# unilight/seq2seq-vc

Hardware: AMD Instinct MI355X
Metric: mel-frames/sec (train) (higher is better)
Workload: dtype bf16; 1 GPU; VTN egs/arctic/vc1 (vtn.v1.yaml) training step: fwd+Seq2SeqLoss+bwd+clip+Adam+WarmupLR; batch_per_gpu=32, global_batch=32, T_src=256, T_tgt=256, mel_dim=80, parallelism=dp1, split_backward=False, hip_graph=True, backward_stages=1

## Files before the change

include/s2svc_hip.h:

```cpp
#ifndef S2SVC_HIP_H
#define S2SVC_HIP_H
#include <stdint.h>
#ifdef __cplusplus
extern "C" {
#endif

const char* s2svc_last_error(void);
int s2svc_abi_version(void);
int s2svc_launch_floor(int workgroups, int threads, void* sink_1024_words, void* stream);

int s2svc_event_create(void** out );
int s2svc_event_destroy(void* ev);
int s2svc_event_record(void* ev, void* stream);
int s2svc_stream_wait_event(void* stream, void* ev);

enum { S2SVC_LAYOUT_KC = 0,
       S2SVC_LAYOUT_RC = 1 };
enum { S2SVC_OP_DENSE = 0,
       S2SVC_OP_CONV1D = 1,
       S2SVC_OP_CONV2D_S2 = 2,
       S2SVC_OP_TCONV2D_S2 = 3 };

typedef struct {
  const void* ptr;
  int64_t ld;
  int32_t layout;
  int32_t mode;
  int32_t C;
  int32_t T;
  int32_t pad;
  int32_t T1, F1, T2, F2;
  int64_t bs0, bs1;
  int32_t zero_padded;
  int32_t reserved_;
} s2svc_operand;

typedef struct {
  s2svc_operand A, B;
  void* C;
  int64_t ldc, cbs0, cbs1;
  int32_t c_dtype;
  const float* bias;
  const void* res;
  int64_t ldr, rbs0, rbs1;
  int32_t M, N, K;
  int32_t nb0, nb1;
  int32_t act;
  float alpha;
  int32_t dtype;
  int32_t accumulate;
  int32_t splitk;
  float* ws;
  float* a_rowsum;
  float* a_rowsum_ws;
  int32_t a_rowsum_accumulate;
  int32_t tile_hint;
  const void* emask;
  int64_t ldm;
  float drop_p;
  int32_t emask_mode;
  const uint64_t* seed_base;
  uint64_t seed_off;
  int32_t c_map;
  int32_t cm_T1, cm_F1, cm_Tc, cm_Fc, cm_pt, cm_pf;
  int32_t reserved3_;
  void* c_pre;
} s2svc_gemm_desc;

int s2svc_gemm(const s2svc_gemm_desc* desc , void* stream);
const char* s2svc_gemm_last_route(void);

int s2svc_tconv2d_weights(int O, int C, const float* w, void* out_bf16, void* stream);

int s2svc_gemm_grouped_ok(const s2svc_gemm_desc* desc );
int s2svc_gemm_grouped(const s2svc_gemm_desc* descs , int n, int tile, void* stream);
int s2svc_gemm_grouped_batched(const s2svc_gemm_desc* descs , int n, void* stream);
int s2svc_gemm_wgrad_ok(const s2svc_gemm_desc* desc );
int64_t s2svc_gemm_wgrad_ws_floats(const s2svc_gemm_desc* descs , int n);
int s2svc_gemm_wgrad_grouped(const s2svc_gemm_desc* descs , int n, float* ws, void* stream);
int s2svc_gemm_wgrad_grouped_bg(const s2svc_gemm_desc* descs , int n, float* ws, void* stream, int wgs_cap);
int s2svc_gemm_set_w8(int on, int kt_chunk);

int s2svc_gemm_set_8ph(int mode);

int s2svc_layernorm_fwd(int dtype, int rows, int D, const void* x, const void* res, float drop_p, float hscale,
                        const uint64_t* seed_base, uint64_t seed_off, const float* gamma, const float* beta, float eps,
                        void* y, void* s_out, float* mean, float* rstd, void* stream);
int s2svc_layernorm_bwd(int dtype, int rows, int D, const void* dy, const void* s, const float* mean, const float* rstd,
                        const float* gamma, const void* ds_extra, float drop_p, float hscale, const uint64_t* seed_base,
                        uint64_t seed_off, void* ds, void* dh, void* stream);
int s2svc_colreduce(int dtype, int rows, int D, int mode, const void* dy, const void* x, const float* mean,
                    const float* rstd, float scale, float* out_sum, float* out_dot, int accumulate, float* ws,
                    int ws_chunks, int Tn, const int32_t* vlens , void* stream);
typedef struct {
  const void* dy;
  const void* x;
  const float* mean;
  const float* rstd;
  float* out_sum;
  float* out_dot;
  float* ws;
  int32_t dtype, rows, D, mode, accumulate, ws_chunks;
  float scale;
  int32_t reserved_;
} s2svc_colreduce_item;
int s2svc_colreduce_grouped(const s2svc_colreduce_item* items , int n, void* stream);
int s2svc_layernorm_bwd_pg_chunks(int dtype, int rows, int D, const void* dy, const void* s, const float* gamma, const void* ds_extra,
                                  const void* ds, const void* dh);
int s2svc_layernorm_bwd_pg(int dtype, int rows, int D, const void* dy, const void* s, const float* mean, const float* rstd,
                           const float* gamma, const void* ds_extra, float drop_p, float hscale, const uint64_t* seed_base,
                           uint64_t seed_off, void* ds, void* dh, float* ws, void* stream);
int s2svc_bn_finalize(int C, int n, float eps, float momentum, const float* mean, const float* var, float* rstd,
                      float* run_mean, float* run_var, int64_t* num_batches, int var_is_ex2 ,
                      int Tn, const int32_t* vlens , void* stream);
int s2svc_rstd_from_var(int C, float eps, const float* var, float* rstd, void* stream);
int s2svc_bn_stats(int dtype, int rows, int C, const void* x, float eps, float momentum, float* mean, float* rstd,
                   float* run_mean, float* run_var, int64_t* num_batches, float* ws, int ws_chunks, int Tn, const int32_t* vlens,
                   void* stream);
int s2svc_bn_apply(int dtype, int64_t rows, int C, const void* x, const float* mean, const float* rstd,
                   const float* gamma, const float* beta, int act, float drop_p, const uint64_t* seed_base,
                   uint64_t seed_off, void* y, void* pre_act, int Tn, const int32_t* vlens, void* stream);
int s2svc_bn_bwd(int dtype, int64_t rows, int C, const void* dy, const void* x, const float* mean, const float* rstd,
                 const float* gamma, const float* sum_dy, const float* sum_dy_xhat, int use_batch_stats, void* dx,
                 int Tn, const int32_t* vlens, void* stream);

int s2svc_attn_softmax_fwd(int dtype, int B, int H, int T1, int T2, int ld, const float* scores, const float* bd, int Lp,
                           int ldb, int rel_mode, float scale, const int32_t* klen, int causal, float drop_p,
                           const uint64_t* seed_base, uint64_t seed_off, void* attn, void* pdrop, void* stream);
int s2svc_attn_softmax_bwd(int dtype, int B, int H, int T1, int T2, int ld, const void* attn, const float* dp, const void* dattn,
                           float scale, float drop_p, const uint64_t* seed_base, uint64_t seed_off, void* dscores,
                           void* dbd, int Lp, int ldb, int rel_mode, void* stream);

int s2svc_act_dropout_fwd(int dtype, int64_t n, const void* x, int act, float p, const uint64_t* seed_base,
                          uint64_t seed_off, void* y, void* stream);
int s2svc_act_dropout_bwd(int dtype, int64_t n, const void* dz, const void* saved, int act, float p,
                          const uint64_t* seed_base, uint64_t seed_off, void* dx, void* stream);
int s2svc_posenc_fwd(int dtype, int64_t B, int T, int D, const void* x, float xscale, const float* alpha, const float* pe,
                     float p, const uint64_t* seed_base, uint64_t seed_off, void* y, void* stream);
int s2svc_posenc_bwd(int dtype, int64_t B, int T, int D, const void* dy, float xscale, const float* pe, float p,
                     const uint64_t* seed_base, uint64_t seed_off, void* dx, float* dalpha, float* partials, void* stream);
int s2svc_axpby(int dtype, int64_t n, float a, const void* x, float b, const void* y, void* out, void* stream);
#define S2SVC_SCALAR_TERMS_MAX 8
typedef struct {
  const float* x[S2SVC_SCALAR_TERMS_MAX];
  int32_t n[S2SVC_SCALAR_TERMS_MAX];
  float w[S2SVC_SCALAR_TERMS_MAX];
  int32_t k;
  int32_t reserved_;
} s2svc_scalar_terms;
int s2svc_weighted_sum(const s2svc_scalar_terms* terms , float* out, void* stream);
int s2svc_weighted_sum_bwd(const s2svc_scalar_terms* grads , const float* g, void* stream);
int s2svc_scalars_axpy(const s2svc_scalar_terms* terms , float beta, float* acc, void* stream);
int s2svc_fill_zero(void* p, int64_t nbytes, void* stream);
int s2svc_seed_advance(uint64_t* seed, uint64_t inc, void* stream);
int s2svc_pad_cols(int dtype, int64_t rows, int N, int ldo, const void* in, void* out, void* stream);
int s2svc_decoder_input(int out_dtype, int B, int Tin, int r, int D, int64_t ys_batch_stride, const float* ys, void* out, void* stream);
int s2svc_append_eos(int B, int T, int64_t ldx, const int64_t* xs, const int32_t* lens, int64_t eos, int64_t pad, int64_t* out, void* stream);
int s2svc_copy_rows(int dtype, int64_t rows, int D, int64_t lds, const void* src, void* out, void* stream);
int s2svc_stop_labels(int B, int T, int64_t ld_labels, const float* labels, const int32_t* lens, float* out, void* stream);
int s2svc_add_n(int dtype, int64_t n, int k, const void* x0, const void* x1, const void* x2, const void* x3, void* out, void* stream);
int s2svc_add_head_bias(int dtype, int64_t rows, int D, const void* q, const float* u, const float* v, void* qu, void* qv,
                        void* stream);
int s2svc_add_head_bias_ld(int dtype, int64_t rows, int D, const void* q, int64_t ldq, const float* u, const float* v, void* qu,
                           void* qv, void* stream);
int s2svc_add_rows(int dtype, int64_t rows, int D, const void* a, int64_t lda, const void* b, int64_t ldb, void* out, int64_t ldo,
                   void* stream);
int s2svc_glu_fwd(int dtype, int64_t rows, int C, const void* x, void* y, void* stream);
int s2svc_glu_bwd(int dtype, int64_t rows, int C, const void* x, const void* dy, void* dx, void* stream);
int s2svc_cast(int in_dtype, int out_dtype, int64_t n, const void* x, void* y, void* stream);
int s2svc_gather3(int in_dtype, int out_dtype, int n0, int n1, int n2, int64_t s0, int64_t s1, int64_t s2, int64_t off,
                  const void* in, void* out, void* stream);
typedef struct s2svc_gather3_job {
  const void* in;
  void* out;
  int64_t s0, s1, s2, off;
  int32_t n0, n1, n2;
  int32_t out_dtype;
} s2svc_gather3_job;
int s2svc_gather3_grouped(const s2svc_gather3_job* jobs , int n, void* stream);
enum { S2SVC_DERIVED_GATHER3 = 0, S2SVC_DERIVED_TCONV2D = 1 };
typedef struct s2svc_derived_job {
  const void* in;
  void* out;
  int64_t s0, s1, s2, off;
  int32_t n0, n1, n2;
  int32_t out_dtype;
  int32_t kind;
  int32_t reserved_;
} s2svc_derived_job;
int s2svc_derived_refresh(const s2svc_derived_job* jobs , int n, void* stream);
int s2svc_derived_refresh_plan(const s2svc_derived_job* jobs , int n, int32_t* path , int32_t* units );
int s2svc_permute_inner(int n, int A, int B, const float* src, float* dst, int accumulate, void* stream);
int s2svc_rowscale(int dtype, int64_t rows, int D, const void* x, const float* s, void* out, void* stream);

int s2svc_conv_in1_fwd(int dtype, int B, int Tn, int Fn, int O, const void* x, const float* w, const float* bias, void* y,
                       void* stream);
int s2svc_conv_in1_wgrad(int dtype, int B, int Tn, int Fn, int O, const void* x, const void* dy, const void* y, float* dw,
                         float* db, int accumulate, float* partial, int max_chunks, void* stream);
int s2svc_col2im_s2(int dtype, int B, int T1, int F1, int C, int T2, int F2, const void* dcols, void* dx, void* stream);
int s2svc_interp_nearest(int dtype, int B, int Tin, int Tout, int C, const void* x, void* y, const int32_t* ext_in,
                         const int32_t* ext_out, void* stream);
int s2svc_interp_nearest_bwd(int dtype, int B, int Tin, int Tout, int C, const void* dy, void* dx, const int32_t* ext_in,
                             const int32_t* ext_out, void* stream);
int s2svc_interp_nearest_rows(int dtype, int B, int Tin, int Tout, int C, const void* x, void* y, const int32_t* lens_in,
                              const int32_t* lens_out, void* stream);
int s2svc_dwconv(int dtype, int B, int Tn, int C, int ks, int dil, const void* x, const float* w, const float* bias,
                 void* y, int flip, void* stream);
int s2svc_dwconv_add(int dtype, int B, int Tn, int C, int ks, int dil, const void* x, const float* w, const float* bias,
                     const void* add, void* y, int flip, void* stream);
int s2svc_dwconv_wgrad(int dtype, int B, int Tn, int C, int ks, int dil, const void* x, const void* dy, float* dw,
                       int accumulate, float* ws, int ws_chunks, void* stream);

int s2svc_convmod_supported(int C, int ks);
int s2svc_convmod_fwd(int B, int Tn, int C, int ks, const void* y2, const float* w, const float* bias, void* z, float eps,
                      float momentum, float* mean, float* rstd, float* run_mean, float* run_var, int64_t* num_batches, float* ws,
                      const int32_t* vlens, void* stream);
int s2svc_bn_swish_apply(int64_t rows, int C, const void* z, const float* mean, const float* rstd, const float* gamma,
                         const float* beta, void* out, int Tn, const int32_t* vlens, void* stream);
int s2svc_convmod_bwd(int B, int Tn, int C, int ks, const void* da, const void* z, const void* y2, const float* w, const float* mean,
                      const float* rstd, const float* gamma, const float* beta, void* dy2, float* sdy, float* sdyx,
                      float* dgamma_acc, float* dbeta_acc, float* ws_stats, float* ws_w, const int32_t* vlens, void* stream);
int s2svc_convmod_wgrad_final(int C, int ks, int chunks, const float* ws_w, float* dw, float* db, int accumulate, void* stream);

int s2svc_convmod_infer_supported(int C, int ks);
int s2svc_convmod_infer(int dtype, int B, int Tn, int C, int ks, const void* y2, const float* w, const float* bias, const float* run_mean,
                        const float* run_var, const float* gamma, const float* beta, float eps, void* out, const int32_t* vlens,
                        void* stream);

int s2svc_bn_stats_vec(int rows, int C, const void* x, float eps, float momentum, float* mean, float* rstd, float* run_mean,
                       float* run_var, int64_t* num_batches, float* ws, int Tn, const int32_t* vlens, void* stream);
int s2svc_bn_act_apply_vec(int rows, int C, const void* x, const float* mean, const float* rstd, const float* gamma, const float* beta,
                           int act, float drop_p, const uint64_t* seed_base, uint64_t seed_off, void* y, void* pre_act, int Tn,
                           const int32_t* vlens, void* stream);
int s2svc_bn_act_bwd_vec(int rows, int C, const void* dz, const void* saved, const void* x, const float* mean, const float* rstd,
                         const float* gamma, int act, float drop_p, const uint64_t* seed_base, uint64_t seed_off, void* dx, float* sdy,
                         float* sdyx, float* dgamma_acc, float* dbeta_acc, float* ws, int Tn, const int32_t* vlens, void* stream);

int s2svc_pairwise_l2_logsoftmax(int dtype, int B, int Tf, int Tx, int A, const void* feats, const void* text,
                                 const int32_t* text_lens, float* logp, float* dist, void* stream);
int s2svc_pairwise_l2_bwd_g(int dtype, int B, int Tf, int Tx, const float* logp, const float* dist, const float* dlogp,
                            const int32_t* text_lens, void* G, float* rowsum, void* stream);
int64_t s2svc_mas_ws_bytes(int B, int Tf, int Tx);
int s2svc_mas(int B, int Tf, int Tx, const float* log_p_attn, const int32_t* text_lens, const int32_t* feat_lens,
              int32_t* path, float* ds, float* binmean, void* ws, void* stream);
int s2svc_mas_binloss_bwd(int B, int Tf, int Tx, const int32_t* path, const int32_t* feat_lens, const float* gout,
                          float* dlogp, void* stream);
int s2svc_gauss_upsample_probs(int dtype, int B, int Tf, int Tx, const float* ds, const int32_t* text_lens,
                               const int32_t* feat_lens, float delta, void* P, void* stream);

int s2svc_length_regulate_index(int B, int Tx, int Tout, const int32_t* ds, int32_t* start, int32_t* idx, int32_t* total,
                                void* stream);
int s2svc_length_regulate_fwd(int dtype, int B, int Tx, int Tout, int D, const void* x, const int32_t* idx, float pad_value,
                              void* y, void* stream);
int s2svc_durations_finalize(int dtype_i64, int B, int Tx, const void* d, const int32_t* text_lens, float dmax, void* d_outs, float* ds,
                             int32_t* total, void* stream);
int s2svc_length_regulate_bwd(int dtype, int B, int Tx, int Tout, int D, const void* dy, const int32_t* start, const int32_t* ds,
                              void* dx, void* stream);
int s2svc_attn_durations(int NH, int Tf, int Tx, const float* att, int64_t* durations, float* focus_rate, int32_t* head,
                         void* stream);

int s2svc_seq_loss_fwd(int dtype, int B, int Tm, int D, const void* after, const void* before, const void* logits,
                       const float* ys, const float* labels, const int32_t* olens, float pos_weight, float* partial,
                       float* out, void* stream);
int s2svc_seq_loss_bwd(int dtype, int B, int Tm, int D, const void* after, const void* before, const void* logits,
                       const float* ys, const float* labels, const int32_t* olens, float pos_weight, const float* stats,
                       const float* g_l1, const float* g_bce, void* d_after, void* d_before, void* d_logits, void* stream);
int s2svc_guided_attn_loss_fwd(int dtype, int B, int H, int To, int Ti, const void* att, const int32_t* ilens,
                               const int32_t* olens, float sigma, float alpha, float* partial, float* out, void* stream);
int s2svc_guided_attn_loss_bwd(int dtype, int B, int H, int To, int Ti, const int32_t* ilens, const int32_t* olens,
                               float sigma, float alpha, const float* stats, const float* gout, void* datt, void* stream);
int s2svc_duration_loss_fwd(int B, int T, const float* d_outs, const float* ds, const int32_t* lens, float offset, int mean,
                            float* stats, float* out, void* stream);
int s2svc_duration_loss_bwd(int B, int T, const float* d_outs, const float* ds, const int32_t* lens, float offset, int mean,
                            const float* stats, const float* g, float* dd, void* stream);
int64_t s2svc_forward_sum_ws_bytes(int B, int Tf, int Tx);
int s2svc_forward_sum(int B, int Tf, int Tx, const float* log_p_attn, const float* prior, const int32_t* text_lens,
                      const int32_t* feat_lens, float log_blank, void* ws, float* loss_b, float* grad, void* stream);
int s2svc_betabinom_prior(int B, int Tf, int Tx, const int32_t* text_lens, const int32_t* feat_lens, float* prior,
                          void* stream);

int s2svc_attn_fused_supported(int dtype, int T1, int T2, int dk);
int s2svc_attn_fused_fwd(int B, int H, int T1, int T2, int dk, const void* q, int64_t ldq, int64_t qbs, const void* k, int64_t ldk,
                         int64_t kbs, const void* v, int64_t ldv, int64_t vbs, const int32_t* klen, int causal, float scale,
                         float drop_p, const uint64_t* seed_base, uint64_t seed_off, void* attn, int ld, void* out, int64_t ldo,
                         int64_t obs, void* stream);
int s2svc_attn_fused_bwd(int B, int H, int T1, int T2, int dk, const void* q, int64_t ldq, int64_t qbs, const void* k, int64_t ldk,
                         int64_t kbs, const void* v, int64_t ldv, int64_t vbs, const void* dout, int64_t ldo, int64_t obs,
                         const void* attn, const void* dattn, int ld, float scale, float drop_p, const uint64_t* seed_base,
                         uint64_t seed_off, void* dq, int64_t lddq, int64_t dqbs, void* dk_out, int64_t lddk, int64_t dkbs, void* dv,
                         int64_t lddv, int64_t dvbs, void* stream);

int s2svc_relattn_supported(int dtype, int T, int dk, int rel_mode);
int s2svc_relattn_fwd(int B, int H, int T, int dk, const void* q, int64_t ldq, int64_t qbs, const void* k, int64_t ldk, int64_t kbs,
                      const void* pos, int64_t ldp, int L, const float* u, const float* v, const int32_t* klen, float scale,
                      float drop_p, const uint64_t* seed_base, uint64_t seed_off, void* attn, void* pdrop, int ld, void* qu, void* qv,
                      void* stream);

int s2svc_attn_map_supported(int dtype, int T1, int T2, int dk);
int s2svc_attn_map_product_supported(int dk);
int s2svc_attn_map_fwd(int B, int H, int T1, int T2, int dk, const void* q, int64_t ldq, int64_t qbs, const void* k, int64_t ldk,
                       int64_t kbs, const int32_t* klen, int causal, float scale, float drop_p, const uint64_t* seed_base,
                       uint64_t seed_off, void* attn, void* pdrop, int ld, const void* v, int64_t ldv, int64_t vbs, void* ctx,
                       int64_t ldc, int64_t cbs, void* stream);
int s2svc_attn_map_bwd(int B, int H, int T1, int T2, int dk, const void* dctx, int64_t ldo, int64_t obs, const void* v, int64_t ldv,
                       int64_t vbs, const void* attn, const void* dattn, float scale, float drop_p, const uint64_t* seed_base,
                       uint64_t seed_off, void* ds, int ld, void* dbd, int ldb, const void* k, int64_t ldk, int64_t kbs, void* dq,
                       int64_t lddq, int64_t dqbs, void* stream);

int s2svc_embedding_fwd(int dtype, int64_t n, int D, int V, const int64_t* idx, const float* w, void* y, void* stream);
int s2svc_embedding_bwd(int dtype, int64_t n, int D, int V, const int64_t* idx, const void* dy, int64_t padding_idx,
                        float* dw, int accumulate, void* stream);

int s2svc_mask_rows(int dtype, int B, int T, int C, const void* x, const int32_t* lens, void* y, void* stream);
int s2svc_expand_fwd(int dtype, int B, int T, int C, const float* a, const float* w, const float* bias, const void* g,
                     const int32_t* lens, void* y, void* stream);
int s2svc_expand_bwd(int dtype, int B, int T, int C, const void* dy, const float* w, const int32_t* lens, void* dg, float* da,
                     void* stream);
int s2svc_ln_act_fwd(int dtype, int rows, int D, int T, const void* x, const float* gamma, const float* beta, float eps, int act,
                     const void* res, const int32_t* lens, float drop_p, const uint64_t* seed_base, uint64_t seed_off, void* y,
                     float* mean, float* rstd, void* stream);
int s2svc_dw_ln_act_fwd(int B, int T, int D, int ks, int dil, const float* x, const float* dw_w, const float* dw_b,
                        const float* gamma, const float* beta, float eps, int act, float* u, float* y, float* mean, float* rstd,
                        void* stream);
int s2svc_ln_act_bwd(int dtype, int rows, int D, int T, const void* dy, const void* x, const float* mean, const float* rstd,
                     const float* gamma, const float* beta, int act, const int32_t* lens, float drop_p,
                     const uint64_t* seed_base, uint64_t seed_off, void* du, void* dx, void* dres, void* stream);

int s2svc_rq_spline_fwd(int B, int T, int bins, const float* x, const float* h, float hscale, float bound, const int32_t* lens,
                        int inverse, float* out, float* lad, int lad_accumulate, void* stream);
int s2svc_rq_spline_bwd(int B, int T, int bins, const float* x, const float* h, float hscale, float bound, const int32_t* lens,
                        const float* g_out, const float* g_lad, float* dx, float* dh, void* stream);
int s2svc_sdp_head_fwd(int B, int T, const float* noise, const int32_t* lens, const float* m, const float* logs, float* z0,
                       float* z1, void* stream);
int s2svc_sdp_head_bwd(int B, int T, const float* noise, const int32_t* lens, const float* logs, const float* dz0,
                       const float* dz1, float* part, void* stream);
int s2svc_sdp_mid_fwd(int B, int T, const float* zu, const float* z1, const float* w, const int32_t* lens, const float* m,
                      const float* logs, float* y0, float* y1, float* lz, void* stream);
int s2svc_sdp_mid_bwd(int B, int T, const float* zu, const float* z1, const float* w, const int32_t* lens, const float* logs,
                      const float* dy0, const float* dy1, const float* dlz, float* dzu, float* dz1, float* part, void* stream);
int s2svc_sdp_tail_fwd(int B, int T, const float* noise, const int32_t* lens, const float* zu, const float* lz,
                       const float* lad_q, const float* lad_p, const float* af, const float* bf, const float* logs_q,
                       const float* logs_p, float* out, int normalize , void* stream);
int s2svc_sdp_tail_bwd(int B, int T, const float* g, const int32_t* lens, const float* zu, const float* af, const float* bf,
                       float* d_af, float* d_bf, float* d_lz, float* d_zu, float* neg_g, float* part, int normalize, void* stream);
int s2svc_sdp_inverse_out(int B, int T, const float* a, const int32_t* lens, const float* m, const float* logs, float* dur,
                          void* stream);

int s2svc_decode_posenc(int dtype, int B, int D, const void* x, float xscale, const float* alpha, const float* pe,
                        const int32_t* pos, void* y, void* stream);
int s2svc_decode_attn(int dtype, int B, int H, int dk, const void* q, int64_t ldq, void* kcache, void* vcache,
                      int64_t ldt, int64_t cbs, const void* knew, const void* vnew, int64_t ldn, const int32_t* pos,
                      const int32_t* klen, int Tk, float scale, void* ctx, int64_t ldo, float* att, int64_t att_bs,
                      int64_t att_hs, int64_t att_ps, void* stream);
int s2svc_decode_emit(int dtype, int B, int r, int odim, const void* feat, const void* logit, float threshold,
                      const int32_t* minlen, const int32_t* maxlen, const int32_t* pos, float* outs, int64_t outs_bs,
                      float* probs, int64_t probs_bs, void* prev, int32_t* stop_at, void* stream);
int s2svc_decode_advance(int32_t* pos, uint64_t* seed_base, uint64_t seed_stride, void* stream);
int s2svc_decode_ln_linear_supported(int dtype, int M, int K);
int s2svc_decode_ln_linear(const s2svc_gemm_desc* desc , const float* gamma, const float* beta, float eps, void* y_out,
                           int64_t ldy, void* stream);
int s2svc_decode_emit_advance(int dtype, int B, int r, int odim, const void* feat, const void* logit, int64_t ldf, float threshold,
                              const int32_t* minlen, const int32_t* maxlen, int32_t* pos, float* outs, int64_t outs_bs, float* probs,
                              int64_t probs_bs, void* prev, int32_t* stop_at, uint64_t* seed_base, uint64_t seed_stride,
                              uint32_t* ticket, const float* pe, const float* alpha, int D, int pe_rows, void* pe_next, void* stream);

int s2svc_adam_step(int64_t n, float* params, const float* grads, float* exp_avg, float* exp_avg_sq, void* bf16_shadow,
                    float beta1, float beta2, float eps, float max_norm, float base_lr, float warmup_steps,
                    double* partial, float* state, void* stream);

int s2svc_transpose_tiles(int64_t ntiles, const int64_t* tiles, const void* src, void* dst, void* stream);

int s2svc_reflect_pad(int64_t n, int pad, const float* x, float* y, void* stream);
int s2svc_magnitude(int64_t frames, int nb, const float* z, float* spc, void* stream);
int s2svc_log_clamp(int64_t n, int D, const float* x, float eps, float inv_log_base, const float* mean,
                    const float* inv_scale, float* y, void* stream);

int s2svc_reflect_pad_batch(int B, int64_t Nmax, int pad, int64_t ld, const float* x, const int32_t* nlen, float* y, void* stream);
int s2svc_stft_logmel_fft_supported(int n_fft, int nmel, int melw_n);
int s2svc_stft_logmel_fft(int B, int64_t Nmax, int Tmax, int n_fft, int hop, int nmel, const float* x, const int32_t* nlen,
                          const int32_t* frames, const float* tables, const int32_t* mel_lo, const int32_t* mel_hi, const int32_t* mel_off, int melw_n, int mel_maxw,
                          float eps, float inv_log_base, const float* mean, const float* inv_scale, float* out, void* stream);

int s2svc_stft_logmel_fft8(int B, int64_t Nmax, int Tmax, int hop, int nmel, const float* x, const int32_t* nlen, const int32_t* frames,
                           const float* tables, const int32_t* seg_lo, const int32_t* seg_len, const float* wud, float eps,
                           float inv_log_base, const float* mean, const float* inv_scale, float* out, void* stream);

int s2svc_mel_log_batch(int B, int Tmax, int nb, int nmel, const float* z, const int32_t* frames, const float* melb,
                        const int32_t* lo, const int32_t* hi, float eps, float inv_log_base, const float* mean,
                        const float* inv_scale, float* out, void* stream);
int s2svc_ragged_to_padded(int B, int Tmax, int D, const float* ragged, const int64_t* offsets, const float* mean,
                           const float* inv_scale, float* out, float* labels, void* stream);

int s2svc_hifigan_cin_padded(int C);
int s2svc_hifigan_conv1d(int dtype, int B, int T, int Cin, int Cout, int k, int dil, const void* x, const void* w_op, const float* bias,
                         float slope, const void* res, int accumulate, float scale, int act_tanh, void* out, const int32_t* vlens,
                         int vmul, void* stream);
int s2svc_hifigan_tconv1d(int dtype, int B, int Tin, int Cin, int Cout, int k, int u, const void* x, const void* w_op, const float* bias,
                          float slope, void* out, const int32_t* vlens, int vmul, void* stream);
int s2svc_hifigan_conv_out(int dtype, int B, int T, int C, int k, const void* x, const float* w, const float* bias, float slope,
                           int act_tanh, float* y, float* y_pre, const int32_t* vlens, int vmul, void* stream);
int s2svc_hifigan_input(int in_dtype, int out_dtype, int B, int T, int C, const void* x, int64_t sb, int64_t st, int64_t sc,
                        const float* a, const float* b, void* out, const int32_t* vlens, void* stream);
int s2svc_hifigan_fold(int mode, int D0, int D1, int k, int u, const float* g, const float* v, float* w32, int op_dtype, void* w_op,
                       void* stream);

int s2svc_gl_supported(int n_fft);
int s2svc_gl_prepare(int B, int Tmax, int nb, int D, int nmel, int hop, const float* x, const float* scale, const float* mean,
                     const float* pinv_t, float eps, const float* u, uint64_t seed, const int32_t* lens, float* S, float* X,
                     float* Rprev, int32_t* nsamp, void* stream);
int s2svc_gl_synth(int B, int Tmax, int n_fft, const float* X, const int32_t* lens, const float* tables, float* frames, void* stream);
int s2svc_gl_analyse(int B, int Tmax, int n_fft, int hop, int reflect, const float* frames, const float* S, const int32_t* lens,
                     const float* tables, float coef, int have_prev, float* X, float* Rprev, void* stream);
int s2svc_gl_ola(int B, int Tmax, int n_fft, int hop, const float* frames, const int32_t* lens, const float* tables, float* y,
                 void* stream);

int64_t s2svc_useg_ws_bytes(int B, int Tmax, int K);
int s2svc_useg_spans(int B, int Tmax, int K, const float* log_probs, const int32_t* lens, void* ws, void* stream);
int s2svc_useg_search(int B, int Tmax, double gamma, const int32_t* lens, const void* ws, const int32_t* labels, int32_t* codes,
                      int32_t* boundaries, int32_t* nseg, float* alpha, int32_t* P, int32_t* clusters, int32_t* cboundaries,
                      int32_t* ncl, void* stream);
int s2svc_useg_stretch(int dtype, int B, int N, int C, const void* x, int64_t sb, int64_t st, int64_t sc, const int32_t* seg,
                       const int32_t* nsegs, int Smax, int Nmax, float scale, float* out, void* stream);

#ifdef __cplusplus
}
#endif
#endif
```

seq2seq_vc_amd/_lib.py:

```python
import ctypes
import os
import subprocess
import sys
from concurrent.futures import ThreadPoolExecutor

_HERE = os.path.dirname(os.path.abspath(__file__))
CSRC = os.path.join(_HERE, "csrc")
LIB_PATH = os.environ.get("S2SVC_LIB") or os.path.join(CSRC, "libs2svc_hip.so")
HIPCC = os.environ.get("HIPCC", "/opt/rocm/bin/hipcc")
ARCH = "gfx950"


def sources():
    return sorted(f for f in os.listdir(CSRC) if f.endswith(".hip"))


DEBUG_EXEC_LIB_PATH = os.path.join(CSRC, "libs2svc_hip_dbgexec.so")


def build_library(force=False, verbose=True, debug_exec=False):
    lib_path = DEBUG_EXEC_LIB_PATH if debug_exec else LIB_PATH
    if not debug_exec and os.environ.get("S2SVC_LIB"):
        lib_path = os.path.join(CSRC, "libs2svc_hip.so")
    srcs = [os.path.join(CSRC, f) for f in sources()]
    deps = srcs + [os.path.join(CSRC, "common.h"), os.path.join(CSRC, "gemm_common.h"),
                   os.path.join(_HERE, "..", "include", "s2svc_hip.h")]
    if not force and os.path.exists(lib_path):
        newest = max(os.path.getmtime(p) for p in deps)
        if os.path.getmtime(lib_path) >= newest:
            return lib_path
    objdir = os.path.join(CSRC, "build", "dbgexec") if debug_exec else os.path.join(CSRC, "build")
    os.makedirs(objdir, exist_ok=True)

    def compile_one(src):
        obj = os.path.join(objdir, os.path.basename(src)[:-4] + ".o")
        hdr_time = max(os.path.getmtime(p) for p in deps[len(srcs):])
        if (not force and os.path.exists(obj) and os.path.getmtime(obj) >= os.path.getmtime(src)
                and os.path.getmtime(obj) >= hdr_time):
            return obj
        cmd = [HIPCC, f"--offload-arch={ARCH}", "-O3", "-std=c++17", "-fPIC", "-Wno-unused-result", "-fno-slp-vectorize",
               "-fno-vectorize", "-c", src, "-o", obj]
        if debug_exec:
            cmd.insert(2, "-DS2SVC_DEBUG_EXEC")
        if verbose:
            print("[s2svc build]", " ".join(cmd), file=sys.stderr)
        subprocess.run(cmd, check=True)
        return obj

    with ThreadPoolExecutor(max_workers=min(8, len(srcs))) as ex:
        objs = list(ex.map(compile_one, srcs))
    cmd = [HIPCC, f"--offload-arch={ARCH}", "-shared", "-fPIC", "-o", lib_path] + objs
    if verbose:
        print("[s2svc build]", " ".join(cmd), file=sys.stderr)
    subprocess.run(cmd, check=True)
    return lib_path


TORCH_OPS_LIB_PATH = os.path.join(CSRC, "libs2svc_torch_ops.so")


def build_torch_ops(force=False, verbose=True):
    import torch
    from torch.utils import cpp_extension as E
    src = os.path.join(CSRC, "torch_ops.cpp")
    deps = [src, os.path.join(_HERE, "..", "include", "s2svc_hip.h")]
    if not force and os.path.exists(TORCH_OPS_LIB_PATH) and os.path.getmtime(TORCH_OPS_LIB_PATH) >= max(os.path.getmtime(p) for p in deps):
        return TORCH_OPS_LIB_PATH
    tlib = E.library_paths()[0]
    cmd = ["g++", "-O2", "-std=c++17", "-fPIC", "-shared", "-D__HIP_PLATFORM_AMD__=1", "-DUSE_ROCM=1",
           f"-D_GLIBCXX_USE_CXX11_ABI={int(torch._C._GLIBCXX_USE_CXX11_ABI)}"]
    cmd += [f"-I{p}" for p in E.include_paths()] + ["-I/opt/rocm/include", src, "-o", TORCH_OPS_LIB_PATH,
                                                    f"-L{tlib}", "-ltorch", "-ltorch_cpu", "-lc10", "-lc10_hip", "-ltorch_hip",
                                                    f"-L{CSRC}", "-ls2svc_hip", "-Wl,-rpath,$ORIGIN", f"-Wl,-rpath,{tlib}"]
    if verbose:
        print("[s2svc build]", " ".join(cmd), file=sys.stderr)
    subprocess.run(cmd, check=True)
    return TORCH_OPS_LIB_PATH


c_i32, c_i64, c_f32, c_u64, c_vp = ctypes.c_int32, ctypes.c_int64, ctypes.c_float, ctypes.c_uint64, ctypes.c_void_p


class Operand(ctypes.Structure):
    _fields_ = [("ptr", c_vp), ("ld", c_i64), ("layout", c_i32), ("mode", c_i32), ("C", c_i32), ("T", c_i32),
                ("pad", c_i32), ("T1", c_i32), ("F1", c_i32), ("T2", c_i32), ("F2", c_i32), ("bs0", c_i64),
                ("bs1", c_i64), ("zero_padded", c_i32), ("reserved_", c_i32)]


class GemmDesc(ctypes.Structure):
    _fields_ = [("A", Operand), ("B", Operand), ("C", c_vp), ("ldc", c_i64), ("cbs0", c_i64), ("cbs1", c_i64),
                ("c_dtype", c_i32), ("bias", c_vp), ("res", c_vp), ("ldr", c_i64), ("rbs0", c_i64), ("rbs1", c_i64),
                ("M", c_i32), ("N", c_i32), ("K", c_i32), ("nb0", c_i32), ("nb1", c_i32), ("act", c_i32),
                ("alpha", c_f32), ("dtype", c_i32), ("accumulate", c_i32), ("splitk", c_i32), ("ws", c_vp),
                ("a_rowsum", c_vp), ("a_rowsum_ws", c_vp), ("a_rowsum_accumulate", c_i32), ("tile_hint", c_i32),
                ("emask", c_vp), ("ldm", c_i64), ("drop_p", c_f32), ("emask_mode", c_i32), ("seed_base", c_vp),
                ("seed_off", c_u64), ("c_map", c_i32), ("cm_T1", c_i32), ("cm_F1", c_i32), ("cm_Tc", c_i32), ("cm_Fc", c_i32),
                ("cm_pt", c_i32), ("cm_pf", c_i32), ("reserved3_", c_i32), ("c_pre", c_vp)]


class ScalarTerms(ctypes.Structure):
    _fields_ = [("x", c_vp * 8), ("n", c_i32 * 8), ("w", c_f32 * 8), ("k", c_i32), ("reserved_", c_i32)]


class Gather3Job(ctypes.Structure):
    _fields_ = [("in_", c_vp), ("out", c_vp), ("s0", c_i64), ("s1", c_i64), ("s2", c_i64), ("off", c_i64), ("n0", c_i32),
                ("n1", c_i32), ("n2", c_i32), ("out_dtype", c_i32)]


class DerivedJob(ctypes.Structure):
    _fields_ = [("in_", c_vp), ("out", c_vp), ("s0", c_i64), ("s1", c_i64), ("s2", c_i64), ("off", c_i64), ("n0", c_i32),
                ("n1", c_i32), ("n2", c_i32), ("out_dtype", c_i32), ("kind", c_i32), ("reserved_", c_i32)]


class ColreduceItem(ctypes.Structure):
    _fields_ = [("dy", c_vp), ("x", c_vp), ("mean", c_vp), ("rstd", c_vp), ("out_sum", c_vp), ("out_dot", c_vp), ("ws", c_vp),
                ("dtype", c_i32), ("rows", c_i32), ("D", c_i32), ("mode", c_i32), ("accumulate", c_i32), ("ws_chunks", c_i32),
                ("scale", c_f32), ("reserved_", c_i32)]


_SIGS = {
    "s2svc_gemm": [ctypes.POINTER(GemmDesc), c_vp],
    "s2svc_gemm_grouped_ok": [c_vp],
    "s2svc_tconv2d_weights": [c_i32, c_i32, c_vp, c_vp, c_vp],
    "s2svc_gemm_grouped": [c_vp, c_i32, c_i32, c_vp],
    "s2svc_gemm_grouped_batched": [c_vp, c_i32, c_vp],
    "s2svc_gemm_wgrad_ok": [c_vp],
    "s2svc_gemm_wgrad_grouped": [c_vp, c_i32, c_vp, c_vp],
    "s2svc_gemm_wgrad_grouped_bg": [c_vp, c_i32, c_vp, c_vp, c_i32],
    "s2svc_gemm_set_w8": [c_i32, c_i32],
    "s2svc_gemm_set_8ph": [c_i32],
    "s2svc_launch_floor": [c_i32, c_i32, c_vp, c_vp],
    "s2svc_event_create": [c_vp],
    "s2svc_event_destroy": [c_vp],
    "s2svc_event_record": [c_vp, c_vp],
    "s2svc_stream_wait_event": [c_vp, c_vp],
    "s2svc_decode_ln_linear_supported": [c_i32, c_i32, c_i32],
    "s2svc_decode_ln_linear": [ctypes.POINTER(GemmDesc), c_vp, c_vp, c_f32, c_vp, c_i64, c_vp],
    "s2svc_length_regulate_index": [c_i32, c_i32, c_i32, c_vp, c_vp, c_vp, c_vp, c_vp],
    "s2svc_length_regulate_fwd": [c_i32, c_i32, c_i32, c_i32, c_i32, c_vp, c_vp, c_f32, c_vp, c_vp],
    "s2svc_length_regulate_bwd": [c_i32, c_i32, c_i32, c_i32, c_i32, c_vp, c_vp, c_vp, c_vp, c_vp],
    "s2svc_attn_durations": [c_i32, c_i32, c_i32, c_vp, c_vp, c_vp, c_vp, c_vp],
    "s2svc_durations_finalize": [c_i32, c_i32, c_i32, c_vp, c_vp, c_f32, c_vp, c_vp, c_vp, c_vp],
    "s2svc_layernorm_fwd": [c_i32, c_i32, c_i32, c_vp, c_vp, c_f32, c_f32, c_vp, c_u64, c_vp, c_vp, c_f32, c_vp, c_vp, c_vp, c_vp, c_vp],
    "s2svc_layernorm_bwd": [c_i32, c_i32, c_i32, c_vp, c_vp, c_vp, c_vp, c_vp, c_vp, c_f32, c_f32, c_vp, c_u64, c_vp, c_vp, c_vp],
    "s2svc_layernorm_bwd_pg_chunks": [c_i32, c_i32, c_i32, c_vp, c_vp, c_vp, c_vp, c_vp, c_vp],
    "s2svc_layernorm_bwd_pg": [c_i32, c_i32, c_i32, c_vp, c_vp, c_vp, c_vp, c_vp, c_vp, c_f32, c_f32, c_vp, c_u64, c_vp, c_vp, c_vp, c_vp],
    "s2svc_colreduce_grouped": [c_vp, c_i32, c_vp],
    "s2svc_colreduce": [c_i32, c_i32, c_i32, c_i32, c_vp, c_vp, c_vp, c_vp, c_f32, c_vp, c_vp, c_i32, c_vp, c_i32, c_i32, c_vp, c_vp],
    "s2svc_bn_finalize": [c_i32, c_i32, c_f32, c_f32, c_vp, c_vp, c_vp, c_vp, c_vp, c_vp, c_i32, c_i32, c_vp, c_vp],
    "s2svc_rstd_from_var": [c_i32, c_f32, c_vp, c_vp, c_vp],
    "s2svc_bn_apply": [c_i32, c_i64, c_i32, c_vp, c_vp, c_vp, c_vp, c_vp, c_i32, c_f32, c_vp, c_u64, c_vp, c_vp, c_i32, c_vp, c_vp],
    "s2svc_bn_bwd": [c_i32, c_i64, c_i32, c_vp, c_vp, c_vp, c_vp, c_vp, c_vp, c_vp, c_i32, c_vp, c_i32, c_vp, c_vp],
    "s2svc_bn_stats": [c_i32, c_i32, c_i32, c_vp, c_f32, c_f32, c_vp, c_vp, c_vp, c_vp, c_vp, c_vp, c_i32, c_i32, c_vp, c_vp],
    "s2svc_attn_softmax_fwd": [c_i32, c_i32, c_i32, c_i32, c_i32, c_i32, c_vp, c_vp, c_i32, c_i32, c_i32, c_f32, c_vp, c_i32, c_f32,
                               c_vp, c_u64, c_vp, c_vp, c_vp],
    "s2svc_attn_softmax_bwd": [c_i32, c_i32, c_i32, c_i32, c_i32, c_i32, c_vp, c_vp, c_vp, c_f32, c_f32, c_vp, c_u64, c_vp, c_vp, c_i32,
                               c_i32, c_i32, c_vp],
    "s2svc_act_dropout_fwd": [c_i32, c_i64, c_vp, c_i32, c_f32, c_vp, c_u64, c_vp, c_vp],
    "s2svc_act_dropout_bwd": [c_i32, c_i64, c_vp, c_vp, c_i32, c_f32, c_vp, c_u64, c_vp, c_vp],
    "s2svc_posenc_fwd": [c_i32, c_i64, c_i32, c_i32, c_vp, c_f32, c_vp, c_vp, c_f32, c_vp, c_u64, c_vp, c_vp],
    "s2svc_posenc_bwd": [c_i32, c_i64, c_i32, c_i32, c_vp, c_f32, c_vp, c_f32, c_vp, c_u64, c_vp, c_vp, c_vp, c_vp],
    "s2svc_axpby": [c_i32, c_i64, c_f32, c_vp, c_f32, c_vp, c_vp, c_vp],
    "s2svc_add_n": [c_i32, c_i64, c_i32, c_vp, c_vp, c_vp, c_vp, c_vp, c_vp],
    "s2svc_weighted_sum": [ctypes.POINTER(ScalarTerms), c_vp, c_vp],
    "s2svc_weighted_sum_bwd": [ctypes.POINTER(ScalarTerms), c_vp, c_vp],
    "s2svc_scalars_axpy": [ctypes.POINTER(ScalarTerms), c_f32, c_vp, c_vp],
    "s2svc_fill_zero": [c_vp, c_i64, c_vp],
    "s2svc_seed_advance": [c_vp, c_u64, c_vp],
    "s2svc_pad_cols": [c_i32, c_i64, c_i32, c_i32, c_vp, c_vp, c_vp],
    "s2svc_decoder_input": [c_i32, c_i32, c_i32, c_i32, c_i32, c_i64, c_vp, c_vp, c_vp],
    "s2svc_stop_labels": [c_i32, c_i32, c_i64, c_vp, c_vp, c_vp, c_vp],
    "s2svc_append_eos": [c_i32, c_i32, c_i64, c_vp, c_vp, c_i64, c_i64, c_vp, c_vp],
    "s2svc_copy_rows": [c_i32, c_i64, c_i32, c_i64, c_vp, c_vp, c_vp],
    "s2svc_add_head_bias": [c_i32, c_i64, c_i32, c_vp, c_vp, c_vp, c_vp, c_vp, c_vp],
    "s2svc_add_head_bias_ld": [c_i32, c_i64, c_i32, c_vp, c_i64, c_vp, c_vp, c_vp, c_vp, c_vp],
    "s2svc_add_rows": [c_i32, c_i64, c_i32, c_vp, c_i64, c_vp, c_i64, c_vp, c_i64, c_vp],
    "s2svc_glu_fwd": [c_i32, c_i64, c_i32, c_vp, c_vp, c_vp],
    "s2svc_glu_bwd": [c_i32, c_i64, c_i32, c_vp, c_vp, c_vp, c_vp],
    "s2svc_cast": [c_i32, c_i32, c_i64, c_vp, c_vp, c_vp],
    "s2svc_gather3_grouped": [c_vp, c_i32, c_vp],
    "s2svc_derived_refresh": [c_vp, c_i32, c_vp],
    "s2svc_derived_refresh_plan": [c_vp, c_i32, c_vp, c_vp],
    "s2svc_permute_inner": [c_i32, c_i32, c_i32, c_vp, c_vp, c_i32, c_vp],
    "s2svc_gather3": [c_i32, c_i32, c_i32, c_i32, c_i32, c_i64, c_i64, c_i64, c_i64, c_vp, c_vp, c_vp],
    "s2svc_mas": [c_i32, c_i32, c_i32, c_vp, c_vp, c_vp, c_vp, c_vp, c_vp, c_vp, c_vp],
    "s2svc_mas_binloss_bwd": [c_i32, c_i32, c_i32, c_vp, c_vp, c_vp, c_vp, c_vp],
    "s2svc_seq_loss_fwd": [c_i32, c_i32, c_i32, c_i32, c_vp, c_vp, c_vp, c_vp, c_vp, c_vp, c_f32, c_vp, c_vp, c_vp],
    "s2svc_seq_loss_bwd": [c_i32, c_i32, c_i32, c_i32, c_vp, c_vp, c_vp, c_vp, c_vp, c_vp, c_f32, c_vp, c_vp, c_vp, c_vp,
                           c_vp, c_vp, c_vp],
    "s2svc_guided_attn_loss_fwd": [c_i32, c_i32, c_i32, c_i32, c_i32, c_vp, c_vp, c_vp, c_f32, c_f32, c_vp, c_vp, c_vp],
    "s2svc_guided_attn_loss_bwd": [c_i32, c_i32, c_i32, c_i32, c_i32, c_vp, c_vp, c_f32, c_f32, c_vp, c_vp, c_vp, c_vp],
    "s2svc_adam_step": [c_i64, c_vp, c_vp, c_vp, c_vp, c_vp, c_f32, c_f32, c_f32, c_f32, c_f32, c_f32, c_vp, c_vp, c_vp],
    "s2svc_transpose_tiles": [c_i64, c_vp, c_vp, c_vp, c_vp],
    "s2svc_col2im_s2": [c_i32, c_i32, c_i32, c_i32, c_i32, c_i32, c_i32, c_vp, c_vp, c_vp],
    "s2svc_interp_nearest": [c_i32, c_i32, c_i32, c_i32, c_i32, c_vp, c_vp, c_vp, c_vp, c_vp],
    "s2svc_interp_nearest_bwd": [c_i32, c_i32, c_i32, c_i32, c_i32, c_vp, c_vp, c_vp, c_vp, c_vp],
    "s2svc_interp_nearest_rows": [c_i32, c_i32, c_i32, c_i32, c_i32, c_vp, c_vp, c_vp, c_vp, c_vp],
    "s2svc_dwconv": [c_i32, c_i32, c_i32, c_i32, c_i32, c_i32, c_vp, c_vp, c_vp, c_vp, c_i32, c_vp],
    "s2svc_dwconv_add": [c_i32, c_i32, c_i32, c_i32, c_i32, c_i32, c_vp, c_vp, c_vp, c_vp, c_vp, c_i32, c_vp],
    "s2svc_dwconv_wgrad": [c_i32, c_i32, c_i32, c_i32, c_i32, c_i32, c_vp, c_vp, c_vp, c_i32, c_vp, c_i32, c_vp],
    "s2svc_convmod_supported": [c_i32, c_i32],
    "s2svc_convmod_fwd": [c_i32, c_i32, c_i32, c_i32, c_vp, c_vp, c_vp, c_vp, c_f32, c_f32, c_vp, c_vp, c_vp, c_vp, c_vp, c_vp, c_vp, c_vp],
    "s2svc_bn_swish_apply": [c_i64, c_i32, c_vp, c_vp, c_vp, c_vp, c_vp, c_vp, c_i32, c_vp, c_vp],
    "s2svc_convmod_bwd": [c_i32, c_i32, c_i32, c_i32, c_vp, c_vp, c_vp, c_vp, c_vp, c_vp, c_vp, c_vp, c_vp, c_vp, c_vp, c_vp, c_vp, c_vp,
                          c_vp, c_vp, c_vp],
    "s2svc_convmod_wgrad_final": [c_i32, c_i32, c_i32, c_vp, c_vp, c_vp, c_i32, c_vp],
    "s2svc_convmod_infer_supported": [c_i32, c_i32],
    "s2svc_convmod_infer": [c_i32, c_i32, c_i32, c_i32, c_i32, c_vp, c_vp, c_vp, c_vp, c_vp, c_vp, c_vp, c_f32, c_vp, c_vp, c_vp],
    "s2svc_bn_stats_vec": [c_i32, c_i32, c_vp, c_f32, c_f32, c_vp, c_vp, c_vp, c_vp, c_vp, c_vp, c_i32, c_vp, c_vp],
    "s2svc_bn_act_apply_vec": [c_i32, c_i32, c_vp, c_vp, c_vp, c_vp, c_vp, c_i32, c_f32, c_vp, c_u64, c_vp, c_vp, c_i32, c_vp, c_vp],
    "s2svc_bn_act_bwd_vec": [c_i32, c_i32, c_vp, c_vp, c_vp, c_vp, c_vp, c_vp, c_i32, c_f32, c_vp, c_u64, c_vp, c_vp, c_vp, c_vp, c_vp, c_vp,
                             c_i32, c_vp, c_vp],
    "s2svc_pairwise_l2_logsoftmax": [c_i32, c_i32, c_i32, c_i32, c_i32, c_vp, c_vp, c_vp, c_vp, c_vp, c_vp],
    "s2svc_pairwise_l2_bwd_g": [c_i32, c_i32, c_i32, c_i32, c_vp, c_vp, c_vp, c_vp, c_vp, c_vp, c_vp],
    "s2svc_rowscale": [c_i32, c_i64, c_i32, c_vp, c_vp, c_vp, c_vp],
    "s2svc_gauss_upsample_probs": [c_i32, c_i32, c_i32, c_i32, c_vp, c_vp, c_vp, c_f32, c_vp, c_vp],
    "s2svc_forward_sum": [c_i32, c_i32, c_i32, c_vp, c_vp, c_vp, c_vp, c_f32, c_vp, c_vp, c_vp, c_vp],
    "s2svc_betabinom_prior": [c_i32, c_i32, c_i32, c_vp, c_vp, c_vp, c_vp],
    "s2svc_conv_in1_fwd": [c_i32, c_i32, c_i32, c_i32, c_i32, c_vp, c_vp, c_vp, c_vp, c_vp],
    "s2svc_conv_in1_wgrad": [c_i32, c_i32, c_i32, c_i32, c_i32, c_vp, c_vp, c_vp, c_vp, c_vp, c_i32, c_vp, c_i32, c_vp],
    "s2svc_attn_fused_supported": [c_i32, c_i32, c_i32, c_i32],
    "s2svc_attn_fused_fwd": [c_i32, c_i32, c_i32, c_i32, c_i32, c_vp, c_i64, c_i64, c_vp, c_i64, c_i64, c_vp, c_i64, c_i64, c_vp, c_i32,
                             c_f32, c_f32, c_vp, c_u64, c_vp, c_i32, c_vp, c_i64, c_i64, c_vp],
    "s2svc_attn_fused_bwd": [c_i32, c_i32, c_i32, c_i32, c_i32, c_vp, c_i64, c_i64, c_vp, c_i64, c_i64, c_vp, c_i64, c_i64, c_vp, c_i64,
                             c_i64, c_vp, c_vp, c_i32, c_f32, c_f32, c_vp, c_u64, c_vp, c_i64, c_i64, c_vp, c_i64, c_i64, c_vp, c_i64,
                             c_i64, c_vp],
    "s2svc_relattn_supported": [c_i32, c_i32, c_i32, c_i32],
    "s2svc_relattn_fwd": [c_i32, c_i32, c_i32, c_i32, c_vp, c_i64, c_i64, c_vp, c_i64, c_i64, c_vp, c_i64, c_i32, c_vp, c_vp, c_vp, c_f32,
                          c_f32, c_vp, c_u64, c_vp, c_vp, c_i32, c_vp, c_vp, c_vp],
    "s2svc_attn_map_supported": [c_i32, c_i32, c_i32, c_i32],
    "s2svc_attn_map_product_supported": [c_i32],
    "s2svc_attn_map_fwd": [c_i32, c_i32, c_i32, c_i32, c_i32, c_vp, c_i64, c_i64, c_vp, c_i64, c_i64, c_vp, c_i32, c_f32, c_f32, c_vp, c_u64,
                           c_vp, c_vp, c_i32, c_vp, c_i64, c_i64, c_vp, c_i64, c_i64, c_vp],
    "s2svc_attn_map_bwd": [c_i32, c_i32, c_i32, c_i32, c_i32, c_vp, c_i64, c_i64, c_vp, c_i64, c_i64, c_vp, c_vp, c_f32, c_f32, c_vp, c_u64,
                           c_vp, c_i32, c_vp, c_i32, c_vp, c_i64, c_i64, c_vp, c_i64, c_i64, c_vp],
    "s2svc_duration_loss_fwd": [c_i32, c_i32, c_vp, c_vp, c_vp, c_f32, c_i32, c_vp, c_vp, c_vp],
    "s2svc_duration_loss_bwd": [c_i32, c_i32, c_vp, c_vp, c_vp, c_f32, c_i32, c_vp, c_vp, c_vp, c_vp],
    "s2svc_embedding_fwd": [c_i32, c_i64, c_i32, c_i32, c_vp, c_vp, c_vp, c_vp],
    "s2svc_embedding_bwd": [c_i32, c_i64, c_i32, c_i32, c_vp, c_vp, c_i64, c_vp, c_i32, c_vp],
    "s2svc_mask_rows": [c_i32, c_i32, c_i32, c_i32, c_vp, c_vp, c_vp, c_vp],
    "s2svc_expand_fwd": [c_i32, c_i32, c_i32, c_i32, c_vp, c_vp, c_vp, c_vp, c_vp, c_vp, c_vp],
    "s2svc_expand_bwd": [c_i32, c_i32, c_i32, c_i32, c_vp, c_vp, c_vp, c_vp, c_vp, c_vp],
    "s2svc_ln_act_fwd": [c_i32, c_i32, c_i32, c_i32, c_vp, c_vp, c_vp, c_f32, c_i32, c_vp, c_vp, c_f32, c_vp, c_u64, c_vp, c_vp,
                         c_vp, c_vp],
    "s2svc_dw_ln_act_fwd": [c_i32, c_i32, c_i32, c_i32, c_i32, c_vp, c_vp, c_vp, c_vp, c_vp, c_f32, c_i32, c_vp, c_vp, c_vp, c_vp, c_vp],
    "s2svc_ln_act_bwd": [c_i32, c_i32, c_i32, c_i32, c_vp, c_vp, c_vp, c_vp, c_vp, c_vp, c_i32, c_vp, c_f32, c_vp, c_u64, c_vp,
                         c_vp, c_vp, c_vp],
    "s2svc_rq_spline_fwd": [c_i32, c_i32, c_i32, c_vp, c_vp, c_f32, c_f32, c_vp, c_i32, c_vp, c_vp, c_i32, c_vp],
    "s2svc_rq_spline_bwd": [c_i32, c_i32, c_i32, c_vp, c_vp, c_f32, c_f32, c_vp, c_vp, c_vp, c_vp, c_vp, c_vp],
    "s2svc_sdp_head_fwd": [c_i32, c_i32, c_vp, c_vp, c_vp, c_vp, c_vp, c_vp, c_vp],
    "s2svc_sdp_head_bwd": [c_i32, c_i32, c_vp, c_vp, c_vp, c_vp, c_vp, c_vp, c_vp],
    "s2svc_sdp_mid_fwd": [c_i32, c_i32, c_vp, c_vp, c_vp, c_vp, c_vp, c_vp, c_vp, c_vp, c_vp, c_vp],
    "s2svc_sdp_mid_bwd": [c_i32, c_i32, c_vp, c_vp, c_vp, c_vp, c_vp, c_vp, c_vp, c_vp, c_vp, c_vp, c_vp, c_vp],
    "s2svc_sdp_tail_fwd": [c_i32, c_i32, c_vp, c_vp, c_vp, c_vp, c_vp, c_vp, c_vp, c_vp, c_vp, c_vp, c_vp, c_i32, c_vp],
    "s2svc_sdp_tail_bwd": [c_i32, c_i32, c_vp, c_vp, c_vp, c_vp, c_vp, c_vp, c_vp, c_vp, c_vp, c_vp, c_vp, c_i32, c_vp],
    "s2svc_sdp_inverse_out": [c_i32, c_i32, c_vp, c_vp, c_vp, c_vp, c_vp, c_vp],
    "s2svc_decode_posenc": [c_i32, c_i32, c_i32, c_vp, c_f32, c_vp, c_vp, c_vp, c_vp, c_vp],
    "s2svc_decode_attn": [c_i32, c_i32, c_i32, c_i32, c_vp, c_i64, c_vp, c_vp, c_i64, c_i64, c_vp, c_vp, c_i64, c_vp, c_vp, c_i32,
                          c_f32, c_vp, c_i64, c_vp, c_i64, c_i64, c_i64, c_vp],
    "s2svc_decode_emit": [c_i32, c_i32, c_i32, c_i32, c_vp, c_vp, c_f32, c_vp, c_vp, c_vp, c_vp, c_i64, c_vp, c_i64, c_vp, c_vp,
                          c_vp],
    "s2svc_decode_advance": [c_vp, c_vp, c_u64, c_vp],
    "s2svc_decode_emit_advance": [c_i32, c_i32, c_i32, c_i32, c_vp, c_vp, c_i64, c_f32, c_vp, c_vp, c_vp, c_vp, c_i64, c_vp, c_i64, c_vp,
                                  c_vp, c_vp, c_u64, c_vp, c_vp, c_vp, c_i32, c_i32, c_vp, c_vp],
    "s2svc_reflect_pad": [c_i64, c_i32, c_vp, c_vp, c_vp],
    "s2svc_magnitude": [c_i64, c_i32, c_vp, c_vp, c_vp],
    "s2svc_log_clamp": [c_i64, c_i32, c_vp, c_f32, c_f32, c_vp, c_vp, c_vp, c_vp],
    "s2svc_reflect_pad_batch": [c_i32, c_i64, c_i32, c_i64, c_vp, c_vp, c_vp, c_vp],
    "s2svc_mel_log_batch": [c_i32, c_i32, c_i32, c_i32, c_vp, c_vp, c_vp, c_vp, c_vp, c_f32, c_f32, c_vp, c_vp, c_vp, c_vp],
    "s2svc_stft_logmel_fft_supported": [c_i32, c_i32, c_i32],
    "s2svc_stft_logmel_fft8": [c_i32, c_i64, c_i32, c_i32, c_i32, c_vp, c_vp, c_vp, c_vp, c_vp, c_vp, c_vp, c_f32, c_f32, c_vp, c_vp, c_vp,
                               c_vp],
    "s2svc_stft_logmel_fft": [c_i32, c_i64, c_i32, c_i32, c_i32, c_i32, c_vp, c_vp, c_vp, c_vp, c_vp, c_vp, c_vp, c_i32,
                              c_i32, c_f32, c_f32, c_vp, c_vp, c_vp, c_vp],
    "s2svc_ragged_to_padded": [c_i32, c_i32, c_i32, c_vp, c_vp, c_vp, c_vp, c_vp, c_vp, c_vp],
    "s2svc_hifigan_cin_padded": [c_i32],
    "s2svc_hifigan_conv1d": [c_i32, c_i32, c_i32, c_i32, c_i32, c_i32, c_i32, c_vp, c_vp, c_vp, c_f32, c_vp, c_i32, c_f32, c_i32, c_vp,
                             c_vp, c_i32, c_vp],
    "s2svc_hifigan_tconv1d": [c_i32, c_i32, c_i32, c_i32, c_i32, c_i32, c_i32, c_vp, c_vp, c_vp, c_f32, c_vp, c_vp, c_i32, c_vp],
    "s2svc_hifigan_conv_out": [c_i32, c_i32, c_i32, c_i32, c_i32, c_vp, c_vp, c_vp, c_f32, c_i32, c_vp, c_vp, c_vp, c_i32, c_vp],
    "s2svc_hifigan_input": [c_i32, c_i32, c_i32, c_i32, c_i32, c_vp, c_i64, c_i64, c_i64, c_vp, c_vp, c_vp, c_vp, c_vp],
    "s2svc_hifigan_fold": [c_i32, c_i32, c_i32, c_i32, c_i32, c_vp, c_vp, c_vp, c_i32, c_vp, c_vp],
    "s2svc_gl_supported": [c_i32],
    "s2svc_gl_prepare": [c_i32, c_i32, c_i32, c_i32, c_i32, c_i32, c_vp, c_vp, c_vp, c_vp, c_f32, c_vp, c_u64, c_vp, c_vp, c_vp, c_vp, c_vp,
                         c_vp],
    "s2svc_gl_synth": [c_i32, c_i32, c_i32, c_vp, c_vp, c_vp, c_vp, c_vp],
    "s2svc_gl_analyse": [c_i32, c_i32, c_i32, c_i32, c_i32, c_vp, c_vp, c_vp, c_vp, c_f32, c_i32, c_vp, c_vp, c_vp],
    "s2svc_gl_ola": [c_i32, c_i32, c_i32, c_i32, c_vp, c_vp, c_vp, c_vp, c_vp],
    "s2svc_useg_spans": [c_i32, c_i32, c_i32, c_vp, c_vp, c_vp, c_vp],
    "s2svc_useg_search": [c_i32, c_i32, ctypes.c_double, c_vp, c_vp, c_vp, c_vp, c_vp, c_vp, c_vp, c_vp, c_vp, c_vp, c_vp, c_vp],
    "s2svc_useg_stretch": [c_i32, c_i32, c_i32, c_i32, c_vp, c_i64, c_i64, c_i64, c_vp, c_vp, c_i32, c_i32, c_f32, c_vp, c_vp],
}
_RET64 = {"s2svc_gemm_wgrad_ws_floats": [c_vp, c_i32], "s2svc_mas_ws_bytes": [c_i32, c_i32, c_i32], "s2svc_forward_sum_ws_bytes": [c_i32, c_i32, c_i32],
          "s2svc_useg_ws_bytes": [c_i32, c_i32, c_i32]}

_lib = None


def exported_symbols():
    return sorted(list(_SIGS) + list(_RET64) + ["s2svc_last_error", "s2svc_abi_version", "s2svc_gemm_last_route"])


def lib():
    global _lib
    if _lib is not None:
        return _lib
    import torch
    if not os.path.exists(LIB_PATH):
        raise RuntimeError(
            f"{LIB_PATH} not found: the seq2seq-vc HIP kernels are not built. Run "
            "`python -c 'import __graft_entry__ as g; g.build()'` (needs hipcc, no GPU). "
            "There is no CPU fallback for the product path.")
    L = ctypes.CDLL(LIB_PATH)
    for name, args in _SIGS.items():
        fn = getattr(L, name)
        fn.argtypes = args
        fn.restype = ctypes.c_int
    for name, args in _RET64.items():
        fn = getattr(L, name)
        fn.argtypes = args
        fn.restype = ctypes.c_int64
    L.s2svc_last_error.restype = ctypes.c_char_p
    L.s2svc_abi_version.restype = ctypes.c_int
    L.s2svc_gemm_last_route.restype = ctypes.c_char_p
    _lib = L
    return L


def check(rc, what):
    if rc != 0:
        msg = lib().s2svc_last_error().decode("utf-8", "replace")
        raise RuntimeError(f"{what} failed (rc={rc}): {msg}")
```

seq2seq_vc_amd/csrc/attn_fused.hip:

```cpp
#include "common.h"
#include "../../include/s2svc_hip.h"

typedef __attribute__((ext_vector_type(8))) __bf16 bf16x8_t;
typedef __attribute__((ext_vector_type(4))) float f32x4_t;

namespace {

constexpr int TP = 72;
constexpr float NEG = -3.4028234663852886e38f;

__device__ __forceinline__ float grp16_max(float v) {
  return row16_max(v);
}
__device__ __forceinline__ float grp16_sum(float v) {
  return row16_sum(v);
}
__device__ __forceinline__ bf16x8_t zero8() { return (bf16x8_t){0, 0, 0, 0, 0, 0, 0, 0}; }
typedef __attribute__((ext_vector_type(4))) uint32_t u32x4_t;
__device__ __forceinline__ uint32_t comp4(const u32x4_t& v, int r) { return r == 0 ? v[0] : r == 1 ? v[1] : r == 2 ? v[2] : v[3]; }
__device__ __forceinline__ float comp(const f32x4_t& v, int r) { return r == 0 ? v[0] : r == 1 ? v[1] : r == 2 ? v[2] : v[3]; }

template <int DK>
__device__ __forceinline__ void load_rows(const bf16_t* g, int64_t ld, int R, uint4 (&r)[DK / 32]) {
  constexpr int ppr = DK / 8;
#pragma unroll
  for (int i = 0; i < DK / 32; ++i) {
    const int p = threadIdx.x + 256 * i;
    const int row = p / ppr, c = p - row * ppr;
    r[i] = make_uint4(0, 0, 0, 0);
    if (row < R) r[i] = *reinterpret_cast<const uint4*>(g + (int64_t)row * ld + c * 8);
  }
}
template <int DK>
__device__ __forceinline__ void load_rows_t(const bf16_t* g, int64_t ld, int R, uint4 (&r)[DK / 32]) {
#pragma unroll
  for (int i = 0; i < DK / 32; ++i) {
    const int p = threadIdx.x + 256 * i;
    const int row = p & 63, c = p >> 6;
    r[i] = make_uint4(0, 0, 0, 0);
    if (row < R) r[i] = *reinterpret_cast<const uint4*>(g + (int64_t)row * ld + c * 8);
  }
}
template <int DK>
__device__ __forceinline__ void put_rows(const uint4 (&r)[DK / 32], bf16_t* lds) {
  constexpr int ppr = DK / 8;
#pragma unroll
  for (int i = 0; i < DK / 32; ++i) {
    const int p = threadIdx.x + 256 * i;
    const int row = p / ppr, c = p - row * ppr;
    *reinterpret_cast<uint4*>(lds + row * (DK + 8) + c * 8) = r[i];
  }
}
template <int DK>
__device__ __forceinline__ void put_rows_t(const uint4 (&r)[DK / 32], bf16_t* lds) {
#pragma unroll
  for (int i = 0; i < DK / 32; ++i) {
    const int p = threadIdx.x + 256 * i;
    const int row = p & 63, c = p >> 6;
    const uint32_t w[4] = {r[i].x, r[i].y, r[i].z, r[i].w};
#pragma unroll
    for (int e = 0; e < 4; ++e) {
      lds[(c * 8 + 2 * e) * TP + row] = (bf16_t)(w[e] & 0xffffu);
      lds[(c * 8 + 2 * e + 1) * TP + row] = (bf16_t)(w[e] >> 16);
    }
  }
}

template <int DK>
__device__ __forceinline__ void store_tile_rows(const f32x4_t (&acc)[DK / 16], bf16_t* stage, bf16_t* dst, int64_t ld, int rows_valid,
                                                bool vec_ok) {
  constexpr int KP = DK + 8;
  const int lane = threadIdx.x & 63, lr = lane & 15, lg = lane >> 4;
  if (!vec_ok) {
#pragma unroll
    for (int dn = 0; dn < DK / 16; ++dn)
#pragma unroll
      for (int r = 0; r < 4; ++r)
        if (lg * 4 + r < rows_valid) dst[(int64_t)(lg * 4 + r) * ld + dn * 16 + lr] = f2bf(acc[dn][r]);
    return;
  }
#pragma unroll
  for (int dn = 0; dn < DK / 16; ++dn)
#pragma unroll
    for (int r = 0; r < 4; ++r) stage[(lg * 4 + r) * KP + dn * 16 + lr] = f2bf(acc[dn][r]);
  constexpr int VPR = DK / 8;
#pragma unroll
  for (int v = lane; v < 16 * VPR; v += 64) {
    const int row = v / VPR, c8 = v - row * VPR;
    if (row < rows_valid)
      *reinterpret_cast<uint4*>(dst + (int64_t)row * ld + c8 * 8) = *reinterpret_cast<const uint4*>(stage + row * KP + c8 * 8);
  }
}

template <int DK>
__global__ __launch_bounds__(256) void attn_fused_fwd_kernel(int H, int T1, int T2, const bf16_t* __restrict__ q, int64_t ldq, int64_t qbs,
                                                             const bf16_t* __restrict__ k, int64_t ldk, int64_t kbs,
                                                             const bf16_t* __restrict__ v, int64_t ldv, int64_t vbs,
                                                             const int32_t* __restrict__ klen, int causal, float scale, float p,
                                                             const uint64_t* seed_base, uint64_t seed_off, bf16_t* __restrict__ attn,
                                                             int ld, bf16_t* __restrict__ out, int64_t ldo, int64_t obs) {
  constexpr int KP = DK + 8;
  __shared__ __attribute__((aligned(16))) bf16_t Ks[64 * KP];
  __shared__ __attribute__((aligned(16))) bf16_t Vt[DK * TP];
  __shared__ __attribute__((aligned(16))) bf16_t Pw[4][16 * TP];
  const int b = blockIdx.x / H, h = blockIdx.x % H;
  const int lane = threadIdx.x & 63, wave = threadIdx.x >> 6, lr = lane & 15, lg = lane >> 4;
  const uint64_t seed = (seed_base ? *seed_base : 0ull) + seed_off;
  const float inv_keep = p > 0.f ? 1.f / (1.f - p) : 1.f;
  const int kl = klen ? (klen[b] < T2 ? klen[b] : T2) : T2;
  uint4 rk[DK / 32], rv[DK / 32];
  load_rows<DK>(k + (int64_t)b * kbs + h * DK, ldk, T2, rk);
  load_rows_t<DK>(v + (int64_t)b * vbs + h * DK, ldv, T2, rv);
  const int qi = wave * 16 + lr;
  bf16x8_t qa[DK / 32];
#pragma unroll
  for (int ks = 0; ks < DK / 32; ++ks)
    qa[ks] = qi < T1 ? *reinterpret_cast<const bf16x8_t*>(q + (int64_t)b * qbs + (int64_t)qi * ldq + h * DK + ks * 32 + lg * 8) : zero8();
  put_rows<DK>(rk, Ks);
  put_rows_t<DK>(rv, Vt);
  __syncthreads();
  f32x4_t s[4];
#pragma unroll
  for (int jn = 0; jn < 4; ++jn) {
    s[jn] = (f32x4_t){0.f, 0.f, 0.f, 0.f};
#pragma unroll
    for (int ks = 0; ks < DK / 32; ++ks) {
      const bf16x8_t kb = *reinterpret_cast<const bf16x8_t*>(Ks + (jn * 16 + lr) * KP + ks * 32 + lg * 8);
      s[jn] = __builtin_amdgcn_mfma_f32_16x16x32_bf16(qa[ks], kb, s[jn], 0, 0, 0);
    }
  }
  bf16_t* pw = Pw[wave];
#pragma unroll 1
  for (int r = 0; r < 4; ++r) {
    const int i = wave * 16 + lg * 4 + r;
    float val[4];
    float mx = NEG;
#pragma unroll
    for (int jn = 0; jn < 4; ++jn) {
      const int j = jn * 16 + lr;
      const bool ok = j < kl && (!causal || j <= i);
      val[jn] = ok ? comp(s[jn], r) * scale : NEG;
      mx = fmaxf(mx, val[jn]);
    }
    mx = grp16_max(mx);
    float sum = 0.f, ex[4];
#pragma unroll
    for (int jn = 0; jn < 4; ++jn) {
      ex[jn] = expf(val[jn] - mx);
      sum += ex[jn];
    }
    sum = grp16_sum(sum);
    const float inv = 1.f / sum;
    const int64_t arow = ((int64_t)(b * H + h) * T1 + i) * ld;
#pragma unroll
    for (int jn = 0; jn < 4; ++jn) {
      const int j = jn * 16 + lr;
      const bool ok = j < kl && (!causal || j <= i);
      const float pr = ok ? ex[jn] * inv : 0.f;
      const bf16_t pb = f2bf(pr);
      if (i < T1 && j < ld) attn[arow + j] = pb;
      float pd = bf2f(pb);
      if (p > 0.f) pd *= dropout_scale(seed, (uint64_t)(arow + j), p, inv_keep);
      pw[(lg * 4 + r) * TP + j] = f2bf(pd);
    }
  }
  f32x4_t o[DK / 16];
#pragma unroll
  for (int dn = 0; dn < DK / 16; ++dn) o[dn] = (f32x4_t){0.f, 0.f, 0.f, 0.f};
#pragma unroll
  for (int ks = 0; ks < 2; ++ks) {
    const bf16x8_t pa = *reinterpret_cast<const bf16x8_t*>(pw + lr * TP + ks * 32 + lg * 8);
#pragma unroll
    for (int dn = 0; dn < DK / 16; ++dn) {
      const bf16x8_t vb = *reinterpret_cast<const bf16x8_t*>(Vt + (dn * 16 + lr) * TP + ks * 32 + lg * 8);
      o[dn] = __builtin_amdgcn_mfma_f32_16x16x32_bf16(pa, vb, o[dn], 0, 0, 0);
    }
  }
  asm volatile("s_waitcnt lgkmcnt(0)\n\ts_barrier" ::: "memory");
  {
    bf16_t* base = out + (int64_t)b * obs + (int64_t)(wave * 16) * ldo + h * DK;
    const bool vec_ok = (ldo % 8 == 0) && (obs % 8 == 0) && (((uintptr_t)out) % 16 == 0);
    store_tile_rows<DK>(o, Ks + wave * 16 * KP, base, ldo, T1 - wave * 16, vec_ok);
  }
}

template <int DK>
__global__ __launch_bounds__(256) void attn_fused_bwd_kernel(int H, int T1, int T2, const bf16_t* __restrict__ q, int64_t ldq, int64_t qbs,
                                                             const bf16_t* __restrict__ k, int64_t ldk, int64_t kbs,
                                                             const bf16_t* __restrict__ v, int64_t ldv, int64_t vbs,
                                                             const bf16_t* __restrict__ dout, int64_t ldo, int64_t obs,
                                                             const bf16_t* __restrict__ attn, const bf16_t* __restrict__ dattn, int ld,
                                                             float scale, float p, const uint64_t* seed_base, uint64_t seed_off,
                                                             bf16_t* __restrict__ dq, int64_t lddq, int64_t dqbs,
                                                             bf16_t* __restrict__ dkk, int64_t lddk, int64_t dkbs,
                                                             bf16_t* __restrict__ dv, int64_t lddv, int64_t dvbs) {
  constexpr int KP = DK + 8;
  __shared__ __attribute__((aligned(16))) bf16_t Vs[64 * KP];
  __shared__ __attribute__((aligned(16))) bf16_t Kt[DK * TP];
  __shared__ __attribute__((aligned(16))) bf16_t Qt[DK * TP];
  __shared__ __attribute__((aligned(16))) bf16_t dOt[DK * TP];
  __shared__ __attribute__((aligned(16))) bf16_t dSt[64 * TP];
  __shared__ __attribute__((aligned(16))) bf16_t Pt[64 * TP];
  __shared__ __attribute__((aligned(16))) bf16_t dSw[4][16 * TP];
  const int b = blockIdx.x / H, h = blockIdx.x % H;
  const int lane = threadIdx.x & 63, wave = threadIdx.x >> 6, lr = lane & 15, lg = lane >> 4;
  const uint64_t seed = (seed_base ? *seed_base : 0ull) + seed_off;
  const float inv_keep = p > 0.f ? 1.f / (1.f - p) : 1.f;
  uint4 rv[DK / 32], rk[DK / 32], rq[DK / 32], rdo[DK / 32];
  load_rows<DK>(v + (int64_t)b * vbs + h * DK, ldv, T2, rv);
  load_rows_t<DK>(k + (int64_t)b * kbs + h * DK, ldk, T2, rk);
  load_rows_t<DK>(q + (int64_t)b * qbs + h * DK, ldq, T1, rq);
  load_rows_t<DK>(dout + (int64_t)b * obs + h * DK, ldo, T1, rdo);
  const int qi = wave * 16 + lr;
  bf16x8_t da[DK / 32];
#pragma unroll
  for (int ks = 0; ks < DK / 32; ++ks)
    da[ks] = qi < T1 ? *reinterpret_cast<const bf16x8_t*>(dout + (int64_t)b * obs + (int64_t)qi * ldo + h * DK + ks * 32 + lg * 8) : zero8();
  u32x4_t praw[4], graw[4];
#pragma unroll
  for (int r = 0; r < 4; ++r) {
    const int i = wave * 16 + lg * 4 + r;
    const int64_t arow = ((int64_t)(b * H + h) * T1 + i) * ld;
#pragma unroll
    for (int jn = 0; jn < 4; ++jn) {
      const int j = jn * 16 + lr;
      const bool in = i < T1 && j < T2;
      praw[jn][r] = in ? attn[arow + j] : 0u;
      graw[jn][r] = (dattn && in) ? dattn[arow + j] : 0u;
    }
  }
  put_rows<DK>(rv, Vs);
  put_rows_t<DK>(rk, Kt);
  put_rows_t<DK>(rq, Qt);
  put_rows_t<DK>(rdo, dOt);
  __syncthreads();
  f32x4_t dp[4];
#pragma unroll
  for (int jn = 0; jn < 4; ++jn) {
    dp[jn] = (f32x4_t){0.f, 0.f, 0.f, 0.f};
#pragma unroll
    for (int ks = 0; ks < DK / 32; ++ks) {
      const bf16x8_t vb = *reinterpret_cast<const bf16x8_t*>(Vs + (jn * 16 + lr) * KP + ks * 32 + lg * 8);
      dp[jn] = __builtin_amdgcn_mfma_f32_16x16x32_bf16(da[ks], vb, dp[jn], 0, 0, 0);
    }
  }
  bf16_t* dsw = dSw[wave];
#pragma unroll 1
  for (int r = 0; r < 4; ++r) {
    const int il = lg * 4 + r, i = wave * 16 + il;
    const int64_t arow = ((int64_t)(b * H + h) * T1 + i) * ld;
    float pv[4], t[4], m[4];
    float dot = 0.f;
#pragma unroll
    for (int jn = 0; jn < 4; ++jn) {
      const int j = jn * 16 + lr;
      const bool in = i < T1 && j < T2;
      pv[jn] = bf2f((bf16_t)(comp4(praw[jn], r)));
      m[jn] = (p > 0.f && in) ? dropout_scale(seed, (uint64_t)(arow + j), p, inv_keep) : 1.f;
      t[jn] = comp(dp[jn], r) * m[jn] + bf2f((bf16_t)(comp4(graw[jn], r)));
      dot += pv[jn] * t[jn];
    }
    dot = grp16_sum(dot);
#pragma unroll
    for (int jn = 0; jn < 4; ++jn) {
      const int j = jn * 16 + lr;
      const bf16_t ds = f2bf(pv[jn] * (t[jn] - dot) * scale);
      const bf16_t pd = f2bf(pv[jn] * m[jn]);
      dsw[il * TP + j] = ds;
      dSt[j * TP + i] = ds;
      Pt[j * TP + i] = pd;
    }
  }
  __syncthreads();
#pragma unroll 1
  for (int which = 0; which < 3; ++which) {
    const bf16_t* At = which == 0 ? dsw : (which == 1 ? dSt : Pt) + wave * 16 * TP;
    const bf16_t* Bt = which == 0 ? Kt : which == 1 ? Qt : dOt;
    f32x4_t acc[DK / 16];
#pragma unroll
    for (int dn = 0; dn < DK / 16; ++dn) acc[dn] = (f32x4_t){0.f, 0.f, 0.f, 0.f};
#pragma unroll
    for (int ks = 0; ks < 2; ++ks) {
      const bf16x8_t a = *reinterpret_cast<const bf16x8_t*>(At + lr * TP + ks * 32 + lg * 8);
#pragma unroll
      for (int dn = 0; dn < DK / 16; ++dn) {
        const bf16x8_t bb = *reinterpret_cast<const bf16x8_t*>(Bt + (dn * 16 + lr) * TP + ks * 32 + lg * 8);
        acc[dn] = __builtin_amdgcn_mfma_f32_16x16x32_bf16(a, bb, acc[dn], 0, 0, 0);
      }
    }
    bf16_t* dst = which == 0 ? dq + (int64_t)b * dqbs : which == 1 ? dkk + (int64_t)b * dkbs : dv + (int64_t)b * dvbs;
    const int64_t ldd = which == 0 ? lddq : which == 1 ? lddk : lddv, dbs = which == 0 ? dqbs : which == 1 ? dkbs : dvbs;
    store_tile_rows<DK>(acc, Vs + wave * 16 * KP, dst + (int64_t)(wave * 16) * ldd + h * DK, ldd, (which == 0 ? T1 : T2) - wave * 16,
                        (ldd % 8 == 0) && (dbs % 8 == 0) && (((uintptr_t)dst) % 16 == 0));
  }
}

}

extern "C" int s2svc_attn_fused_supported(int dtype, int T1, int T2, int dk) {
  return dtype == S2S_BF16 && T1 >= 1 && T1 <= 64 && T2 >= 1 && T2 <= 64 && (dk == 32 || dk == 64 || dk == 96 || dk == 128);
}

extern "C" int s2svc_attn_fused_fwd(int B, int H, int T1, int T2, int dk, const void* q, int64_t ldq, int64_t qbs, const void* k,
                                    int64_t ldk, int64_t kbs, const void* v, int64_t ldv, int64_t vbs, const int32_t* klen, int causal,
                                    float scale, float drop_p, const uint64_t* seed_base, uint64_t seed_off, void* attn, int ld,
                                    void* out, int64_t ldo, int64_t obs, void* stream) {
  S2S_REQUIRE(s2svc_attn_fused_supported(S2S_BF16, T1, T2, dk), "attn_fused_fwd: unsupported shape (bf16, T <= 64, d_k in {32,64,96,128})");
  S2S_REQUIRE(ld >= T2 && ld <= 64, "attn_fused_fwd: the map's row pitch ld must be in [T2, 64]");
  S2S_REQUIRE(ldq % 8 == 0 && ldk % 8 == 0 && ldv % 8 == 0 && qbs % 8 == 0 && kbs % 8 == 0 && vbs % 8 == 0,
              "attn_fused_fwd: strides must be multiples of 8 elements");
  S2S_REQUIRE(((uintptr_t)q) % 16 == 0 && ((uintptr_t)k) % 16 == 0 && ((uintptr_t)v) % 16 == 0, "attn_fused_fwd: 16-byte aligned q/k/v");
  if (B == 0) return 0;
  hipStream_t st = (hipStream_t)stream;
#define S2S_AF_FWD(DK)                                                                                                        \
  hipLaunchKernelGGL((attn_fused_fwd_kernel<DK>), dim3(B * H), dim3(256), 0, st, H, T1, T2, (const bf16_t*)q, ldq, qbs,        \
                     (const bf16_t*)k, ldk, kbs, (const bf16_t*)v, ldv, vbs, klen, causal, scale, drop_p, seed_base, seed_off, \
                     (bf16_t*)attn, ld, (bf16_t*)out, ldo, obs)
  if (dk == 32) S2S_AF_FWD(32); else if (dk == 64) S2S_AF_FWD(64); else if (dk == 96) S2S_AF_FWD(96); else S2S_AF_FWD(128);
#undef S2S_AF_FWD
  S2S_CHECK_LAUNCH("attn_fused_fwd_kernel");
  return 0;
}

extern "C" int s2svc_attn_fused_bwd(int B, int H, int T1, int T2, int dk, const void* q, int64_t ldq, int64_t qbs, const void* k,
                                    int64_t ldk, int64_t kbs, const void* v, int64_t ldv, int64_t vbs, const void* dout, int64_t ldo,
                                    int64_t obs, const void* attn, const void* dattn, int ld, float scale, float drop_p,
                                    const uint64_t* seed_base, uint64_t seed_off, void* dq, int64_t lddq, int64_t dqbs, void* dk_out,
                                    int64_t lddk, int64_t dkbs, void* dv, int64_t lddv, int64_t dvbs, void* stream) {
  S2S_REQUIRE(s2svc_attn_fused_supported(S2S_BF16, T1, T2, dk), "attn_fused_bwd: unsupported shape (bf16, T <= 64, d_k in {32,64,96,128})");
  S2S_REQUIRE(ld >= T2, "attn_fused_bwd: the map's row pitch ld must be >= T2");
  S2S_REQUIRE(ldq % 8 == 0 && ldk % 8 == 0 && ldv % 8 == 0 && ldo % 8 == 0 && qbs % 8 == 0 && kbs % 8 == 0 && vbs % 8 == 0 &&
              obs % 8 == 0, "attn_fused_bwd: strides must be multiples of 8 elements");
  S2S_REQUIRE(((uintptr_t)q) % 16 == 0 && ((uintptr_t)k) % 16 == 0 && ((uintptr_t)v) % 16 == 0 && ((uintptr_t)dout) % 16 == 0,
              "attn_fused_bwd: 16-byte aligned q/k/v/dout");
  if (B == 0) return 0;
  hipStream_t st = (hipStream_t)stream;
#define S2S_AF_BWD(DK)                                                                                                          \
  hipLaunchKernelGGL((attn_fused_bwd_kernel<DK>), dim3(B * H), dim3(256), 0, st, H, T1, T2, (const bf16_t*)q, ldq, qbs,          \
                     (const bf16_t*)k, ldk, kbs, (const bf16_t*)v, ldv, vbs, (const bf16_t*)dout, ldo, obs, (const bf16_t*)attn, \
                     (const bf16_t*)dattn, ld, scale, drop_p, seed_base, seed_off, (bf16_t*)dq, lddq, dqbs, (bf16_t*)dk_out, lddk,  \
                     dkbs, (bf16_t*)dv, lddv, dvbs)
  if (dk == 32) S2S_AF_BWD(32); else if (dk == 64) S2S_AF_BWD(64); else if (dk == 96) S2S_AF_BWD(96); else S2S_AF_BWD(128);
#undef S2S_AF_BWD
  S2S_CHECK_LAUNCH("attn_fused_bwd_kernel");
  return 0;
}
```

seq2seq_vc_amd/modules.py:

```python
import math
import os

import torch
from torch import nn

from .ops import functional as Fn
from .ops import kernels as K

_LENS_CACHE = {}
_BANK = None


class LensBank:

    def __init__(self, device, max_slots=96):
        self.device = torch.device(device)
        self.max_slots = max_slots
        self.B = None
        self.buf = None
        self.entries = []
        self.roots = {}
        self.closed = False

    def root(self, name, source, values, cap):
        lens = Lens.__new__(Lens)
        lens._init_banked(self, values, cap, ("root", name))
        self.roots[id(source)] = (source, lens)
        return lens

    def _slot(self, lens, source):
        if self.closed:
            raise RuntimeError("LensBank: a Lens was created after the capture of this step finished")
        k = len(self.entries)
        B = len(lens.host)
        if self.buf is None:
            self.B = B
            self.buf = torch.zeros((self.max_slots, B), dtype=torch.int32, device=self.device)
        if B != self.B or k >= self.max_slots:
            raise RuntimeError(f"LensBank: {B} lengths in a bank of batch size {self.B}, or more than {self.max_slots} slots")
        self.entries.append((lens, source))
        if not (self.device.type == "cuda" and torch.cuda.is_current_stream_capturing()):
            self.buf.data[k].copy_(torch.tensor(lens.host, dtype=torch.int32))
        return self.buf[k]

    def upload(self):
        n = len(self.entries)
        if n:
            stage = torch.tensor([lens.host for lens, _ in self.entries], dtype=torch.int32)
            if self.device.type == "cuda":
                stage = stage.pin_memory()
            self.buf.data[:n].copy_(stage, non_blocking=True)

    def refresh(self, root_values):
        for k, (lens, source) in enumerate(self.entries):
            if source[0] == "root":
                vals = tuple(int(v) for v in root_values[source[1]])
                if max(vals) > lens.cap:
                    raise ValueError(f"LensBank: length {max(vals)} of '{source[1]}' exceeds the padded length {lens.cap} of this graph")
                ext = max(vals)
            else:
                vals, ext = _derive(source, len(lens.host))
            lens.host, lens.ext = vals, ext
        self.upload()


def _derive(source, B):
    parent = source[1]
    if source[0] == "crop":
        return (parent.ext,) * B, parent.ext
    _, _, fn, ext_fn, with_ext = source
    vals = tuple(fn(v, parent.ext) for v in parent.host) if with_ext else tuple(fn(v) for v in parent.host)
    return vals, (ext_fn if ext_fn is not None else fn)(parent.ext)


class lens_bank:

    def __init__(self, bank):
        self.bank = bank

    def __enter__(self):
        global _BANK
        self.prev, _BANK = _BANK, self.bank
        return self.bank

    def __exit__(self, *exc):
        global _BANK
        _BANK = self.prev


def tag_lens(tensor, lens):
    if _BANK is not None and isinstance(tensor, torch.Tensor):
        tensor._s2s_lens = lens
    return tensor


class Lens:

    def __init__(self, values, device, _source=None, _cap=None, _ext=None):
        if _BANK is not None:
            if _source is None:
                raise RuntimeError("Lens: lengths without provenance inside a captured training step (register them with "
                                   "LensBank.root, derive them with Lens.map / Lens.clamp, or tag host tensors with tag_lens)")
            self._init_banked(_BANK, values, _cap, _source, _ext)
            return
        self.host = tuple(int(v) for v in values)
        self.device = torch.device(device)
        self.cap = None
        self.ext = None
        self.rows = False
        key = (self.host, self.device.type, self.device.index)
        t = _LENS_CACHE.get(key)
        if t is None:
            if len(_LENS_CACHE) > 4096:
                _LENS_CACHE.clear()
            t = torch.tensor(self.host, dtype=torch.int32, device=self.device)
            _LENS_CACHE[key] = t
        self.dev = t

    def _init_banked(self, bank, values, cap, source, ext=None):
        self.host = tuple(int(v) for v in values)
        self.device = bank.device
        self.cap = int(cap)
        self.ext = int(max(self.host) if ext is None else ext)
        self._crop = None
        self.rows = False
        self.dev = bank._slot(self, source)

    @staticmethod
    def of(lens, device):
        if lens is None or isinstance(lens, Lens):
            return lens
        if _BANK is not None:
            tagged = getattr(lens, "_s2s_lens", None)
            if tagged is not None:
                return tagged
            reg = _BANK.roots.get(id(lens))
            if reg is not None and reg[0] is lens:
                return reg[1]
            raise RuntimeError("Lens.of: these lengths were not registered with the LensBank of the captured step")
        if isinstance(lens, torch.Tensor):
            lens = lens.tolist()
        return Lens(lens, device)

    def map(self, fn, ext_fn=None, with_ext=False):
        if self.cap is not None:
            vals, ext = _derive(("map", self, fn, ext_fn, with_ext), len(self.host))
            return Lens(vals, self.device, _source=("map", self, fn, ext_fn, with_ext), _cap=(ext_fn if ext_fn is not None else fn)(self.cap),
                        _ext=ext)
        out = Lens([fn(v, self.max()) for v in self.host] if with_ext else [fn(v) for v in self.host], self.device)
        out.rows = self.rows
        return out

    def per_row(self):
        assert self.cap is None, "per-row lengths are an inference feature: no LensBank"
        out = Lens(self.host, self.device)
        out.rows = True
        return out

    def crop(self):
        if self.cap is None:
            return None
        if self._crop is None:
            self._crop = Lens((self.ext,) * len(self.host), self.device, _source=("crop", self), _cap=self.cap, _ext=self.ext)
        return self._crop

    def max(self):
        return self.cap if self.cap is not None else max(self.host)

    def clamp(self, hi):
        return self.map(lambda v, _hi=hi: min(v, _hi))


def crop_dev(lens):
    if lens is None:
        return None
    if lens.cap is None:
        return lens.dev if lens.rows else None
    return lens.crop().dev


def rows_dev(lens):
    return lens.dev if lens is not None and lens.cap is None and lens.rows else None


def _sin_table(n, d, reverse=False):
    pos = torch.arange(n - 1, -1, -1.0, dtype=torch.float32) if reverse else torch.arange(0, n, dtype=torch.float32)
    div = torch.exp(torch.arange(0, d, 2, dtype=torch.float32) * -(math.log(10000.0) / d))
    pe = torch.zeros(n, d)
    pe[:, 0::2] = torch.sin(pos[:, None] * div)
    pe[:, 1::2] = torch.cos(pos[:, None] * div)
    return pe


class PositionalEncoding(nn.Module):

    def __init__(self, d_model, dropout_rate, max_len=5000, reverse=False):
        super().__init__()
        self.d_model, self.reverse, self.max_len = d_model, reverse, max_len
        self.xscale = math.sqrt(d_model)
        self.dropout_rate = dropout_rate
        self._pe = None

    def table(self, T, device):
        if self._pe is None or self._pe.shape[0] < T or self._pe.device != device:
            self._pe = _sin_table(max(self.max_len, T), self.d_model, self.reverse).to(device)
        return self._pe

    def forward(self, x):
        p = self.dropout_rate if self.training else 0.0
        return Fn.posenc(x, self.table(x.shape[1], x.device), None, self.xscale, p)


class ScaledPositionalEncoding(PositionalEncoding):

    def __init__(self, d_model, dropout_rate, max_len=5000):
        super().__init__(d_model, dropout_rate, max_len)
        self.alpha = nn.Parameter(torch.tensor(1.0))

    def reset_parameters(self):
        self.alpha.data = torch.tensor(1.0)

    def forward(self, x):
        p = self.dropout_rate if self.training else 0.0
        return Fn.posenc(x, self.table(x.shape[1], x.device), self.alpha, 1.0, p)


class RelPositionalEncoding(nn.Module):

    def __init__(self, d_model, dropout_rate, max_len=5000):
        super().__init__()
        self.d_model, self.dropout_rate = d_model, dropout_rate
        self.xscale = math.sqrt(d_model)
        self._cache = {}

    def pos_emb(self, T, device, dtype):
        key = (T, str(device), dtype)
        if key not in self._cache:
            if len(self._cache) > 64:
                self._cache.clear()
            plus = torch.flip(_sin_table(T, self.d_model), [0])
            pos = torch.arange(0, T, dtype=torch.float32)[:, None]
            div = torch.exp(torch.arange(0, self.d_model, 2, dtype=torch.float32) * -(math.log(10000.0) / self.d_model))
            minus = torch.zeros(T, self.d_model)
            minus[:, 0::2], minus[:, 1::2] = torch.sin(-pos * div), torch.cos(-pos * div)
            self._cache[key] = torch.cat([plus, minus[1:]], dim=0)[None].to(device).to(dtype).contiguous()
        return self._cache[key]

    def forward(self, x):
        p = self.dropout_rate if self.training else 0.0
        pe = self.pos_emb(x.shape[1], x.device, x.dtype)
        return Fn.posenc(x, None, None, self.xscale, p), Fn.dropout(pe, p)


class LegacyRelPositionalEncoding(PositionalEncoding):

    def __init__(self, d_model, dropout_rate, max_len=5000):
        super().__init__(d_model, dropout_rate, max_len, reverse=True)

    def forward(self, x):
        if _BANK is not None:
            raise NotImplementedError('config["hip_graph"]: legacy relative positional encoding is not supported in captured steps '
                                      "(no recipe uses it); run this model with hip_graph off")
        p = self.dropout_rate if self.training else 0.0
        pe = K.cast(self.table(x.shape[1], x.device)[: x.shape[1]][None].contiguous(), x.dtype)
        return Fn.posenc(x, None, None, self.xscale, p), Fn.dropout(pe, p)


class MultiHeadedAttention(nn.Module):
    def __init__(self, n_head, n_feat, dropout_rate):
        super().__init__()
        assert n_feat % n_head == 0
        self.d_k, self.h = n_feat // n_head, n_head
        self.linear_q = nn.Linear(n_feat, n_feat)
        self.linear_k = nn.Linear(n_feat, n_feat)
        self.linear_v = nn.Linear(n_feat, n_feat)
        self.linear_out = nn.Linear(n_feat, n_feat)
        self.attn = None
        self.dropout_rate = dropout_rate

    def _p(self):
        return self.dropout_rate if self.training else 0.0

    def forward(self, query, key, value, klens=None, causal=False, kv=None, passthrough=False):
        kl = None if klens is None else klens.dev
        f = getattr(self, "_fused", None)
        qp = None
        if kv is not None:
            q = Fn.linear(query, f["w_q"], f["b_q"], passthrough=passthrough)
            if passthrough:
                q, qp = q
            ctx, self.attn = Fn.attention_packed_kv(q, kv, kl, causal, self.h, self._p())
        elif f is not None and key is value and (query is not key or "w_qkv" in f):
            if query is key:
                qkv = Fn.linear(query, f["w_qkv"], f["b_qkv"], passthrough=passthrough)
                if passthrough:
                    qkv, qp = qkv
                ctx, self.attn = Fn.attention_packed_qkv(qkv, kl, causal, self.h, self._p())
            else:
                q = Fn.linear(query, f["w_q"], f["b_q"], passthrough=passthrough)
                if passthrough:
                    q, qp = q
                kv = Fn.linear(key, f["w_kv"], f["b_kv"])
                ctx, self.attn = Fn.attention_packed_kv(q, kv, kl, causal, self.h, self._p())
        else:
            q = Fn.linear(query, self.linear_q.weight, self.linear_q.bias)
            k = Fn.linear(key, self.linear_k.weight, self.linear_k.bias)
            v = Fn.linear(value, self.linear_v.weight, self.linear_v.bias)
            ctx, self.attn = Fn.attention_core(q, k, v, kl, causal, self.h, self._p())
            qp = query
        out = Fn.linear(ctx, self.linear_out.weight, self.linear_out.bias)
        return (out, qp) if passthrough else out


class RelPositionMultiHeadedAttention(MultiHeadedAttention):

    legacy = False

    def __init__(self, n_head, n_feat, dropout_rate, zero_triu=False):
        super().__init__(n_head, n_feat, dropout_rate)
        if zero_triu:
            raise NotImplementedError("zero_triu is not supported")
        self.zero_triu = zero_triu
        self.linear_pos = nn.Linear(n_feat, n_feat, bias=False)
        self.pos_bias_u = nn.Parameter(torch.Tensor(self.h, self.d_k))
        self.pos_bias_v = nn.Parameter(torch.Tensor(self.h, self.d_k))
        nn.init.xavier_uniform_(self.pos_bias_u)
        nn.init.xavier_uniform_(self.pos_bias_v)

    def forward(self, query, key, value, pos_emb, klens=None):
        f = getattr(self, "_fused", None)
        if f is not None and "w_qkv" in f and query is key and key is value:
            qkv = Fn.linear(query, f["w_qkv"], f["b_qkv"])
            pos = Fn.linear(pos_emb, self.linear_pos.weight, None)
            ctx, self.attn = Fn.rel_attention_packed(qkv, pos, self.pos_bias_u, self.pos_bias_v,
                                                     None if klens is None else klens.dev, self.h, self._p(),
                                                     2 if self.legacy else 1)
            return Fn.linear(ctx, self.linear_out.weight, self.linear_out.bias)
        q = Fn.linear(query, self.linear_q.weight, self.linear_q.bias)
        k = Fn.linear(key, self.linear_k.weight, self.linear_k.bias)
        v = Fn.linear(value, self.linear_v.weight, self.linear_v.bias)
        pos = Fn.linear(pos_emb, self.linear_pos.weight, None)
        qu, qv = Fn.add_head_bias(q, self.pos_bias_u, self.pos_bias_v)
        ctx, self.attn = Fn.rel_attention_core(qu, qv, k, v, pos, None if klens is None else klens.dev, self.h, self._p(),
                                               2 if self.legacy else 1)
        return Fn.linear(ctx, self.linear_out.weight, self.linear_out.bias)


class LegacyRelPositionMultiHeadedAttention(RelPositionMultiHeadedAttention):
    legacy = True


class PositionwiseFeedForward(nn.Module):

    def __init__(self, idim, hidden_units, dropout_rate, activation="relu"):
        super().__init__()
        self.w_1 = nn.Linear(idim, hidden_units)
        self.w_2 = nn.Linear(hidden_units, idim)
        self.dropout_rate = dropout_rate
        self.activation = activation

    def forward(self, x, passthrough=False):
        p = self.dropout_rate if self.training else 0.0
        if self.activation in ("relu", "swish"):
            return Fn.ffn_act(x, self.w_1.weight, self.w_1.bias, self.w_2.weight, self.w_2.bias, self.activation, p, passthrough)
        xp = None
        if passthrough:
            h, xp = Fn.linear(x, self.w_1.weight, self.w_1.bias, passthrough=True)
        else:
            h = Fn.linear(x, self.w_1.weight, self.w_1.bias)
        y = Fn.linear(Fn.act_dropout(h, self.activation, p), self.w_2.weight, self.w_2.bias)
        return (y, xp) if passthrough else y


class MultiLayeredConv1d(nn.Module):

    def __init__(self, in_chans, hidden_chans, kernel_size, dropout_rate):
        super().__init__()
        self.w_1 = nn.Conv1d(in_chans, hidden_chans, kernel_size, stride=1, padding=(kernel_size - 1) // 2)
        self.w_2 = nn.Conv1d(hidden_chans, in_chans, kernel_size, stride=1, padding=(kernel_size - 1) // 2)
        self.dropout_rate = dropout_rate

    def forward(self, x, lens=None):
        p = self.dropout_rate if self.training else 0.0
        vl = crop_dev(lens)
        h = Fn.dropout(Fn.conv1d(x, self.w_1.weight, self.w_1.bias, act="relu", vlens=vl), p)
        return Fn.conv1d(h, self.w_2.weight, self.w_2.bias, vlens=vl)


class LayerNorm(nn.LayerNorm):

    def __init__(self, nout, dim=-1, eps=1e-12):
        super().__init__(nout, eps=eps)
        self.dim = dim

    def forward(self, x):
        return Fn.layer_norm(x, self.weight, self.bias, self.eps)


def _sub_pass(sub, x, *args, **kw):
    if (type(sub) in (MultiHeadedAttention, PositionwiseFeedForward) and torch.is_grad_enabled() and x.requires_grad):
        return sub(x, *args, passthrough=True, **kw)
    return sub(x, *args, **kw), x


def _res_norm(norm, res, h, p, hscale=1.0):
    return Fn.add_dropout_layer_norm(res, h, norm.weight, norm.bias, norm.eps, p, hscale)


class EncoderLayer(nn.Module):
    def __init__(self, size, self_attn, feed_forward, dropout_rate, normalize_before=True, concat_after=False,
                 stochastic_depth_rate=0.0):
        super().__init__()
        if concat_after or stochastic_depth_rate > 0:
            raise NotImplementedError("concat_after / stochastic depth are not used by any recipe")
        self.self_attn, self.feed_forward = self_attn, feed_forward
        self.norm1, self.norm2 = LayerNorm(size), LayerNorm(size)
        self.dropout_rate = dropout_rate
        self.size, self.normalize_before = size, normalize_before

    def forward(self, x, klens, normed=None):
        p = self.dropout_rate if self.training else 0.0
        if self.normalize_before:
            if normed is None:
                y, x = Fn.layer_norm(x, self.norm1.weight, self.norm1.bias, self.norm1.eps, passthrough=True)
            else:
                y = normed
            a = self.self_attn(y, y, y, klens)
            y2, x = _res_norm(self.norm2, x, a, p)
            f = self.feed_forward(y2, klens) if isinstance(self.feed_forward, MultiLayeredConv1d) else self.feed_forward(y2)
            return x, f
        a, xr = _sub_pass(self.self_attn, x, x, x, klens)
        x, _ = _res_norm(self.norm1, xr, a, p)
        if isinstance(self.feed_forward, MultiLayeredConv1d):
            f, xr = self.feed_forward(x, klens), x
        else:
            f, xr = _sub_pass(self.feed_forward, x)
        x, _ = _res_norm(self.norm2, xr, f, p)
        return x, None


class DecoderLayer(nn.Module):
    def __init__(self, size, self_attn, src_attn, feed_forward, dropout_rate, normalize_before=True, concat_after=False):
        super().__init__()
        if concat_after:
            raise NotImplementedError("concat_after is not used by any recipe")
        self.size = size
        self.self_attn, self.src_attn, self.feed_forward = self_attn, src_attn, feed_forward
        self.norm1, self.norm2, self.norm3 = LayerNorm(size), LayerNorm(size), LayerNorm(size)
        self.dropout_rate = dropout_rate
        self.normalize_before = normalize_before

    def self_block(self, x, tgt_lens, normed=None, causal=True):
        p = self.dropout_rate if self.training else 0.0
        if self.normalize_before:
            if normed is None:
                y, x = Fn.layer_norm(x, self.norm1.weight, self.norm1.bias, self.norm1.eps, passthrough=True)
            else:
                y = normed
            a = self.self_attn(y, y, y, tgt_lens, causal=causal)
            return _res_norm(self.norm2, x, a, p)
        a, xr = _sub_pass(self.self_attn, x, x, x, tgt_lens, causal=causal)
        x, _ = _res_norm(self.norm1, xr, a, p)
        return x, x

    def forward(self, x, tgt_lens, memory, mem_lens, normed=None, causal=True, kv=None, head=None):
        p = self.dropout_rate if self.training else 0.0
        if self.normalize_before:
            y, x = self.self_block(x, tgt_lens, normed, causal) if head is None else head
            a = self.src_attn(y, memory, memory, mem_lens, kv=kv)
            y, x = _res_norm(self.norm3, x, a, p)
            return x, self.feed_forward(y)
        x = self.self_block(x, tgt_lens, None, causal)[0] if head is None else head[0]
        a, xr = _sub_pass(self.src_attn, x, memory, memory, mem_lens, kv=kv)
        x, _ = _res_norm(self.norm2, xr, a, p)
        f, xr = _sub_pass(self.feed_forward, x)
        x, _ = _res_norm(self.norm3, xr, f, p)
        return x, None


def run_stack(layers, x, after_norm, pre_ln, dropout_rate, training, *args, per_layer=None, **kw):
    p = dropout_rate if training else 0.0
    pending = None
    cut_name = kw.pop("cut_name", None)
    for li, layer in enumerate(layers):
        kwl = dict(kw, **per_layer[li]) if per_layer is not None else kw
        if cut_name is not None and li > 0:
            x, pending = Fn.cut_point((x, pending), f"{cut_name}.{li}")
        if pre_ln and pending is not None:
            normed, x = _res_norm(layer.norm1, x, pending, p)
            x, pending = layer(x, *args, normed=normed, **kwl)
        else:
            x, pending = layer(x, *args, **kwl)
    if pre_ln:
        if pending is not None:
            y, x = _res_norm(after_norm, x, pending, p)
            return y
        return after_norm(x)
    return x


class Conv2dSubsampling(nn.Module):
    def __init__(self, idim, odim, dropout_rate, pos_enc=None, use_pos_enc=True):
        super().__init__()
        self.conv = nn.Sequential(nn.Conv2d(1, odim, 3, 2), nn.ReLU(), nn.Conv2d(odim, odim, 3, 2), nn.ReLU())
        self.f2 = ((idim - 1) // 2 - 1) // 2
        if use_pos_enc:
            self.out = nn.Sequential(nn.Linear(odim * self.f2, odim),
                                     pos_enc if pos_enc is not None else PositionalEncoding(odim, dropout_rate))
        else:
            self.out = nn.Linear(odim * self.f2, odim)
        self.odim, self.use_pos_enc = odim, use_pos_enc

    def __getitem__(self, key):
        if key != -1:
            raise NotImplementedError("Support only `-1` (for `reset_parameters`).")
        return self.out[key]

    @staticmethod
    def out_lens(lens, t_out, exact=False):
        if lens is None:
            return None
        sub = lambda T: ((T - 1) // 2 - 1) // 2
        if exact:
            return lens.map(lambda v: min(sub(v), t_out), ext_fn=sub)
        if lens.cap is not None:
            assert sub(lens.cap) == t_out
            return lens.map(lambda v, e: min((v + 3) // 4, sub(e)), ext_fn=sub, with_ext=True)
        return lens.map(lambda v: min((v + 3) // 4, t_out))

    def forward(self, x, lens, exact_lens=False):
        B, T, idim = x.shape
        c0, c2 = self.conv[0], self.conv[2]
        if c0.weight.shape[0] % 8 == 0:
            y = Fn.conv_in1_relu(x, c0.weight, c0.bias, grad_premasked=True)
            first_relu = True
        else:
            y = Fn.conv2d_s2_relu(x.reshape(B, T, idim, 1), c0.weight, c0.bias)
            first_relu = False
        y = Fn.conv2d_s2_relu(y, c2.weight, c2.bias, grad_premasked=True, input_is_relu=first_relu)
        _, T2, F2, C = y.shape
        lin = self.out[0] if self.use_pos_enc else self.out
        y = Fn.linear_fc_permuted(y.reshape(B * T2, F2 * C), lin.weight, lin.bias, C, F2, input_is_relu=True).view(B, T2, self.odim)
        if self.use_pos_enc:
            y = self.out[1](y)
        return y, self.out_lens(lens, T2, exact_lens)


class Prenet(nn.Module):

    def __init__(self, idim, n_layers=2, n_units=256, dropout_rate=0.5):
        super().__init__()
        self.dropout_rate = dropout_rate
        self.prenet = nn.ModuleList()
        for layer in range(n_layers):
            self.prenet += [nn.Sequential(nn.Linear(idim if layer == 0 else n_units, n_units), nn.ReLU())]

    def forward(self, x):
        for blk in self.prenet:
            x = Fn.dropout(Fn.linear(x, blk[0].weight, blk[0].bias, act="relu"), self.dropout_rate)
        return x


class Postnet(nn.Module):

    def __init__(self, idim, odim, n_layers=5, n_chans=512, n_filts=5, dropout_rate=0.5, use_batch_norm=True):
        super().__init__()
        self.postnet = nn.ModuleList()
        for layer in range(n_layers):
            ichans = odim if layer == 0 else n_chans
            ochans = odim if layer == n_layers - 1 else n_chans
            mods = [nn.Conv1d(ichans, ochans, n_filts, stride=1, padding=(n_filts - 1) // 2, bias=False)]
            if use_batch_norm:
                mods.append(nn.BatchNorm1d(ochans))
            if layer != n_layers - 1:
                mods.append(nn.Tanh())
            mods.append(nn.Dropout(dropout_rate))
            self.postnet += [nn.Sequential(*mods)]
        self.dropout_rate, self.use_batch_norm = dropout_rate, use_batch_norm

    def forward(self, xs, lens=None):
        n = len(self.postnet)
        p = self.dropout_rate if self.training else 0.0
        vl = crop_dev(lens)
        for i, blk in enumerate(self.postnet):
            act = "tanh" if i != n - 1 else None
            xs = Fn.conv1d(xs, blk[0].weight, None, vlens=vl if (i == 0 or not self.use_batch_norm or not self.training) else None)
            if self.use_batch_norm:
                bn = blk[1]
                xs = Fn.batch_norm_act(xs, bn.weight, bn.bias, bn.running_mean, bn.running_var, bn.num_batches_tracked,
                                       self.training, act, p, bn.eps, bn.momentum, vlens=vl if self.training else None)
            else:
                xs = Fn.act_dropout(xs, act, p)
        return xs


class MultiSequential(nn.Sequential):
    """Holder with the reference's container name; stacks are driven by run_stack()."""


class TransformerEncoder(nn.Module):
    def __init__(self, idim, attention_dim=256, attention_heads=4, linear_units=2048, num_blocks=6, dropout_rate=0.1,
                 positional_dropout_rate=0.1, attention_dropout_rate=0.0, input_layer="conv2d",
                 pos_enc_class=PositionalEncoding, normalize_before=True, concat_after=False,
                 positionwise_layer_type="linear", positionwise_conv_kernel_size=1, padding_idx=-1):
        super().__init__()
        if input_layer == "conv2d":
            self.embed = Conv2dSubsampling(idim, attention_dim, dropout_rate)
        elif input_layer == "conv2d-scaled-pos-enc":
            self.embed = Conv2dSubsampling(idim, attention_dim, dropout_rate, pos_enc_class(attention_dim, positional_dropout_rate))
        elif isinstance(input_layer, nn.Module):
            self.embed = nn.Sequential(input_layer, pos_enc_class(attention_dim, positional_dropout_rate))
        else:
            raise ValueError("unsupported input_layer: " + str(input_layer))
# ... 78 lines not shown
```

seq2seq_vc_amd/ops/functional.py:

```python
import math
import os

import torch
from torch.autograd import Function

from . import kernels as K
from . import kernels_attn as KAT

_STATE = {"dtype": torch.float32}


def set_compute_dtype(dtype):
    if dtype not in (torch.float32, torch.bfloat16):
        raise ValueError("compute dtype must be float32 or bfloat16")
    _STATE["dtype"] = dtype


def compute_dtype():
    return _STATE["dtype"]


def to_compute(x):
    return K.cast(x.contiguous(), _STATE["dtype"])

# ... 61 lines not shown
            return x
        if name in self.points:
            raise RuntimeError(f"gradient cut '{name}' was reached twice in one forward pass")
        inner = tuple(t.detach().requires_grad_(True) if (t is not None and t.requires_grad) else t for t in xs)
        self.points[name] = (xs, inner)
        return inner if isinstance(x, tuple) else inner[0]

    def resume(self, name):
        outer, inner = self.points.get(name, (None, None))
        if outer is None:
            return
        pairs = [(o, i.grad) for o, i in zip(outer, inner) if o is not None and o.requires_grad and i is not o and i.grad is not None]
        if pairs:
            torch.autograd.backward([o for o, _ in pairs], [g for _, g in pairs], retain_graph=False)

    def clear(self):
        self.points.clear()


_CUTS = {"active": None}


class grad_cuts:
    def __init__(self, cuts):
        self.cuts = cuts

    def __enter__(self):
        self.prev, _CUTS["active"] = _CUTS["active"], self.cuts
        if self.cuts is not None:
            self.cuts.clear()
        return self.cuts

    def __exit__(self, *exc):
        _CUTS["active"] = self.prev
        return False


def cut_point(x, name):
    c = _CUTS["active"]
    return x if c is None else c.cut(x, name)


class _Side:
    enabled = False
    streams = []
    idx = 0
    pending = []
    queue = []
    origins = []
    inline = False
    inline_q = {}
    batch = 16
    grouped = []
    grouped_cr = []
    on_flush = None


def _taken_streams():
    h = {st.cuda_stream for st in _Side.streams}
    if _Branch.stream is not None:
        h.add(_Branch.stream.cuda_stream)
    if torch.cuda.is_available():
        h.add(torch.cuda.current_stream().cuda_stream)
    return h


def distinct_stream(taken=None):
    taken = _taken_streams() if taken is None else set(taken)
    for _ in range(96):
        st = torch.cuda.Stream()
        if st.cuda_stream not in taken:
            return st
    raise RuntimeError("no distinct stream left in torch's stream pool")


def enable_side_streams(n=4, inline_batches=False, batch=None):
    K.set_wgrad_cap(64 if n > 0 else 0)
    _Side.enabled = n > 0
    _Side.inline = (n == 0) and inline_batches
    _Side.batch = int(batch) if batch else (64 if _Side.inline else 16)
    old, others = _Side.streams, _taken_streams() - {st.cuda_stream for st in _Side.streams}
    if n > 0 and len(old) == n and len({st.cuda_stream for st in old}) == n and not ({st.cuda_stream for st in old} & others):
        pass
    else:
        _Side.streams = []
        for _ in range(n):
            _Side.streams.append(distinct_stream())
    _Side.idx = 0


def _side_run(fn, keep=(), solo=False):
    if solo and _Side.enabled and not _Side.inline:
        held, held_o = _Side.queue, _Side.origins
        _Side.queue, _Side.origins = [fn], [torch.cuda.current_stream()]
        _Side.pending.append(keep)
        _side_flush()
        _Side.queue, _Side.origins = held, held_o
        return
    if _Side.inline:
        cur = torch.cuda.current_stream()
        q = _Side.inline_q.setdefault(cur.cuda_stream, (cur, []))[1]
        q.append(fn)
        _Side.pending.append(keep)
        if len(q) >= _Side.batch:
            _inline_flush(cur.cuda_stream)
        return
    if not _Side.enabled:
        fn()
        return
    _Side.queue.append(fn)
    _Side.origins.append(torch.cuda.current_stream())
    _Side.pending.append(keep)
    if len(_Side.queue) >= _Side.batch:
        _side_flush()


def _run_batch(closures):
    with K.record_grouped(_Side.grouped), K.record_colreduce(_Side.grouped_cr):
        for fn in closures:
            fn()
    if _Side.grouped:
        K.flush_grouped(_Side.grouped)
    if _Side.grouped_cr:
        K.flush_colreduce(_Side.grouped_cr)


def _inline_flush(key):
    st, q = _Side.inline_q.pop(key)
    with torch.cuda.stream(st):
        _run_batch(q)
        if _Side.on_flush is not None:
            _Side.on_flush()
    return st


def _side_flush():
    if _Side.inline:
        return
    if not _Side.queue:
        return
    k = _Side.idx % len(_Side.streams)
    st = _Side.streams[k]
    cur = torch.cuda.current_stream().cuda_stream
    if st.cuda_stream == cur or (_Branch.stream is not None and st.cuda_stream == _Branch.stream.cuda_stream):
        st = _Side.streams[k] = distinct_stream()
    _Side.idx += 1
    seen = set()
    for origin in _Side.origins + [torch.cuda.current_stream()]:
        if origin.cuda_stream not in seen:
            seen.add(origin.cuda_stream)
            st.wait_stream(origin)
    _Side.origins = []
    with torch.cuda.stream(st):
        _run_batch(_Side.queue)
        if _Side.on_flush is not None:
            _Side.on_flush()
    _Side.queue = []


_NO_BRANCH = os.environ.get("S2SVC_NO_BRANCH", "0") == "1"


class _Branch:
    stream = None
    active = False
    dirty = False


def branch_run(fn, uses=()):
    if not torch.cuda.is_available() or _NO_BRANCH:
        return fn()
    main = torch.cuda.current_stream()
    if _Branch.stream is None or _Branch.stream.cuda_stream == main.cuda_stream:
        _Branch.stream = distinct_stream()
    _Branch.stream.wait_stream(main)
    for t in uses:
        if isinstance(t, torch.Tensor) and t.is_cuda:
            t.record_stream(_Branch.stream)
    with torch.cuda.stream(_Branch.stream):
        out = fn()
    _Branch.active = True
    _Branch.dirty = True
    return out


def branch_join(*results):
    if _Branch.active:
        main = torch.cuda.current_stream()
        main.wait_stream(_Branch.stream)
        for t in results:
            if isinstance(t, torch.Tensor) and t.is_cuda:
                t.record_stream(main)
        _Branch.active = False


def branch_backward(loss, fork_event, retain_graph=False, scale=1.0):
    if _Branch.stream is None or _NO_BRANCH:
        root_backward(loss, scale, retain_graph)
        return
    _Branch.stream.wait_event(fork_event)
    _Branch.dirty = True
    with torch.cuda.stream(_Branch.stream):
        root_backward(loss, scale, retain_graph)


def branch_resume(cuts, name, fork_event):
    if _Branch.stream is None or _NO_BRANCH:
        cuts.resume(name)
        return
    _Branch.stream.wait_event(fork_event)
    _Branch.dirty = True
    with torch.cuda.stream(_Branch.stream):
        cuts.resume(name)


def branch_wait():
    if _Branch.stream is not None and not _NO_BRANCH:
        torch.cuda.current_stream().wait_stream(_Branch.stream)


def side_join():
    if _Side.inline:
        main = torch.cuda.current_stream()
        for key in list(_Side.inline_q):
            st = _inline_flush(key)
            if st.cuda_stream != main.cuda_stream:
                main.wait_stream(st)
    if _Side.enabled:
        cap = K.get_wgrad_cap()
        K.set_wgrad_cap(0)
        try:
            _side_flush()
        finally:
            K.set_wgrad_cap(cap)
        main = torch.cuda.current_stream()
        for st in _Side.streams:
            main.wait_stream(st)
    _join_branch_stream()
    K.audit_reset()
    _Side.pending.clear()
    _Side.idx = 0


def _join_branch_stream():
    if _Branch.stream is not None and _Branch.dirty:
        torch.cuda.current_stream().wait_stream(_Branch.stream)
    _Branch.dirty = False


def _slotted(*params):
    return all(p is None or getattr(p, "_s2s_grad", None) is not None for p in params)


def _bias_sink(bias, n):
    if bias is None or not bias.requires_grad:
        return None, False, None
    slot = getattr(bias, "_s2s_grad", None)
    if slot is not None:
        return slot.view(-1), True, None
    buf = torch.empty(n, dtype=torch.float32, device=bias.device)
    return buf, False, buf.view(bias.shape)


def _reduce_to(p_sum, p_dot, mode, dy, x=None, mean=None, rstd=None):
    s_slot = getattr(p_sum, "_s2s_grad", None)
    d_slot = getattr(p_dot, "_s2s_grad", None) if p_dot is not None else None
    if s_slot is not None and (p_dot is None or d_slot is not None):
        K.colreduce(mode, dy, x, mean, rstd, want_dot=p_dot is not None, out_sum=s_slot.view(-1),
                    out_dot=None if d_slot is None else d_slot.view(-1), accumulate=True)
        return None, None
    s, d = K.colreduce(mode, dy, x, mean, rstd, want_dot=p_dot is not None)
    return s.view(p_sum.shape), (None if d is None else d.view(p_dot.shape))




class _Linear(Function):

    @staticmethod
    def forward(ctx, x, weight, bias, act, passthrough=False):
        dtype = x.dtype
        x2 = _c(x).view(-1, x.shape[-1])
        M, Kd = x2.shape
        N = weight.shape[0]
        w = _wcast(weight, dtype)
        y = torch.empty((M, N), dtype=dtype, device=x.device)
        K.gemm(K.operand(x2, Kd), K.operand(w, Kd), M, N, Kd, y, in_dtype=dtype, bias=bias, act=act)
        ctx.act = act
        ctx.has_bias = bias is not None
        ctx.params = (weight, bias)
        ctx.save_for_backward(x2, w, y if act else None)
        ctx.xshape = x.shape
        if passthrough:
            ctx.set_materialize_grads(False)
            return y.view(*x.shape[:-1], N), x.view_as(x)
        return y.view(*x.shape[:-1], N)

    @staticmethod
    def backward(ctx, dy, g_pass=None):
        if dy is None:
            return g_pass, None, None, None, None
        x2, w, y = ctx.saved_tensors
        weight, bias = ctx.params
        M, Kd = x2.shape
        N = w.shape[0]
        dtype = x2.dtype
        dy2 = _c(dy).view(M, N)
        if ctx.act:
            dy2 = K.act_dropout_bwd(dy2, y, act=ctx.act)
        ldy, zp, dy_rows = N, False, dy2
        if dtype == torch.float32 and N % 4 and dy2.is_cuda:
            ldy, zp = (N + 3) // 4 * 4, True
            dy2 = K.pad_cols(dy2, ldy)
        dx = None
        if ctx.needs_input_grad[0]:
            dx = torch.empty((M, Kd), dtype=dtype, device=dy.device)
            res = _c(g_pass).view(M, Kd).to(dtype) if g_pass is not None else None
            K.gemm(K.operand(dy2, ldy, zero_padded=zp), _dgrad_operand(weight, w, N, Kd, dtype), M, Kd, N, dx, in_dtype=dtype, res=res)
            dx = dx.view(ctx.xshape)
        dw = db = None
        if weight.requires_grad:
            tile, sk = K.plan_gemm(N, Kd, M, dtype=dtype)
            rs, racc, db = _bias_sink(bias, N)

            def wr(out, acc):
                K.gemm(K.operand(dy2, ldy, layout=K.RC, zero_padded=zp), K.operand(x2, Kd, layout=K.RC), N, Kd, M, out, in_dtype=dtype,
                       splitk=sk, tile=tile, accumulate=acc, a_rowsum=rs, a_rowsum_accumulate=racc)
            if _slotted(weight, bias if ctx.has_bias else None):
                _side_run(lambda: _emit_wgrad(weight, (N, Kd), wr), keep=(dy2, x2))
            else:
                dw = _emit_wgrad(weight, (N, Kd), wr)
                if dw is not None:
                    dw = dw.view(weight.shape)
        elif ctx.has_bias and bias.requires_grad:
            db, _ = _reduce_to(bias, None, 0, dy_rows)
        return dx, dw, db, None, None


def linear(x, weight, bias=None, act=None, passthrough=False):
    return _Linear.apply(x, weight, bias, act, passthrough)


class _FFNRelu(Function):

    @staticmethod
    def forward(ctx, x, w1, b1, w2, b2, p, passthrough=False, act="relu"):
        dtype = x.dtype
        x2 = _c(x).view(-1, x.shape[-1])
        M, Kd = x2.shape
        Hd, N = w1.shape[0], w2.shape[0]
        w1c, w2c = _wcast(w1, dtype), _wcast(w2, dtype)
        seed = K.new_seed(x.device) if p > 0.0 else (None, 0)
        h = torch.empty((M, Hd), dtype=dtype, device=x.device)
        u = torch.empty((M, Hd), dtype=dtype, device=x.device) if act != "relu" else None
        K.gemm(K.operand(x2, Kd), K.operand(w1c, Kd), M, Hd, Kd, h, in_dtype=dtype, bias=b1, act=act, drop_p=p, seed=seed, pre_out=u)
        y = torch.empty((M, N), dtype=dtype, device=x.device)
        K.gemm(K.operand(h, Hd), K.operand(w2c, Hd), M, N, Hd, y, in_dtype=dtype, bias=b2)
        ctx.params = (w1, b1, w2, b2)
        ctx.meta = (p, seed, x.shape)
        ctx.save_for_backward(x2, h, w1c, w2c, u)
        if passthrough:
            ctx.set_materialize_grads(False)
            return y.view(*x.shape[:-1], N), x.view_as(x)
        return y.view(*x.shape[:-1], N)

    @staticmethod
    def backward(ctx, dy, g_pass=None):
        if dy is None:
            return g_pass, None, None, None, None, None, None, None
        x2, h, w1c, w2c, u = ctx.saved_tensors
        w1, b1, w2, b2 = ctx.params
        p, seed, xshape = ctx.meta
        M, Kd = x2.shape
        Hd, N = w1c.shape[0], w2c.shape[0]
        dtype = x2.dtype
        dy2 = _c(dy).view(M, N)
        du = torch.empty((M, Hd), dtype=dtype, device=dy.device)
        K.gemm(K.operand(dy2, N), _dgrad_operand(w2, w2c, N, Hd, dtype), M, Hd, N, du, in_dtype=dtype, emask=h if u is None else u,
               emask_mode=0 if u is None else 1, drop_p=p, seed=seed)
        dx = None
        if ctx.needs_input_grad[0]:
            dx = torch.empty((M, Kd), dtype=dtype, device=dy.device)
            res = _c(g_pass).view(M, Kd).to(dtype) if g_pass is not None else None
            K.gemm(K.operand(du, Hd), _dgrad_operand(w1, w1c, Hd, Kd, dtype), M, Kd, Hd, dx, in_dtype=dtype, res=res)
            dx = dx.view(xshape)

        def wgrad(weight, bias, g, a, n_out, n_in):
            tile, sk = K.plan_gemm(n_out, n_in, M, dtype=dtype)
            rs, racc, db = _bias_sink(bias, n_out)

            def wr(out, acc):
                K.gemm(K.operand(g, n_out, layout=K.RC), K.operand(a, n_in, layout=K.RC), n_out, n_in, M, out, in_dtype=dtype,
                       splitk=sk, tile=tile, accumulate=acc, a_rowsum=rs, a_rowsum_accumulate=racc)
            if _slotted(weight, bias):
                _side_run(lambda: _emit_wgrad(weight, (n_out, n_in), wr), keep=(g, a))
                return None, None
            dw = _emit_wgrad(weight, (n_out, n_in), wr)
            return (dw.view(weight.shape) if dw is not None else None), db
        dw2, db2 = wgrad(w2, b2, dy2, h, N, Hd) if w2.requires_grad else (None, None)
        dw1, db1 = wgrad(w1, b1, du, x2, Hd, Kd) if w1.requires_grad else (None, None)
        return dx, dw1, db1, dw2, db2, None, None, None


def ffn_relu(x, w1, b1, w2, b2, p=0.0, passthrough=False):
    return _FFNRelu.apply(x, w1, b1, w2, b2, p, passthrough, "relu")


def ffn_act(x, w1, b1, w2, b2, act, p=0.0, passthrough=False):
    return _FFNRelu.apply(x, w1, b1, w2, b2, p, passthrough, act)


class _Embedding(Function):

    @staticmethod
    def forward(ctx, idx, weight, padding_idx):
        idx = idx.contiguous()
        ctx.weight, ctx.padding_idx = weight, padding_idx
        ctx.save_for_backward(idx)
        return K.embedding_fwd(idx, weight.detach(), compute_dtype())

    @staticmethod
    def backward(ctx, dy):
        (idx,) = ctx.saved_tensors
        weight = ctx.weight
        dw = None
        if weight.requires_grad:
            dw = _emit_wgrad(weight, tuple(weight.shape),
                             lambda out, acc: K.embedding_bwd(idx, _c(dy), weight.shape[0], ctx.padding_idx, out=out, accumulate=acc))
        return None, dw, None


def embedding(idx, weight, padding_idx=None):
    return _Embedding.apply(idx, weight, padding_idx)


class _AddLayerNorm(Function):
    @staticmethod
    def forward(ctx, h, res, gamma, beta, eps, p, hscale):
        seed = K.new_seed(h.device) if p > 0.0 else (None, 0)
        h = _c(h)
        res = _c(res) if res is not None else None
        y, s, mean, rstd = K.layernorm_fwd(h, gamma, beta, eps, res=res, p=p, seed=seed, hscale=hscale)
        ctx.meta = (eps, p, seed, hscale, res is not None)
        ctx.params = (gamma, beta)
        ctx.save_for_backward(s if res is not None else h, mean, rstd)
        ctx.set_materialize_grads(False)
        if res is None:
            return y
        return y, s

    @staticmethod
    def backward(ctx, dy, ds_direct=None):
        s, mean, rstd = ctx.saved_tensors
        gamma, beta = ctx.params
        eps, p, seed, hscale, fused = ctx.meta
        dy = _c(dy) if dy is not None else torch.zeros_like(s)
        extra = _c(ds_direct) if (fused and ds_direct is not None) else None
        slotted = gamma.requires_grad and _slotted(gamma, beta)
        ds, dh, part = K.layernorm_bwd(dy, s, mean, rstd, gamma, ds_extra=extra, p=p, seed=seed,
                                       want_dh=fused and (p > 0.0 or hscale != 1.0), hscale=hscale, want_partials=True, partials_ok=slotted)
        dgamma = dbeta = None
        if gamma.requires_grad:
            if part is not None:
                ws, chunks = part
                b_slot, g_slot = beta._s2s_grad.view(-1), gamma._s2s_grad.view(-1)
                _side_run(lambda: K.colreduce_partials(ws, chunks, s.shape[-1], b_slot, g_slot), keep=(ws,))
            elif _slotted(gamma, beta):
                _side_run(lambda: _reduce_to(beta, gamma, 1, dy, s, mean, rstd), keep=(dy, s, mean, rstd))
            else:
                dbeta, dgamma = _reduce_to(beta, gamma, 1, dy, s, mean, rstd)
        if fused:
            return (dh if dh is not None else ds), ds, dgamma, dbeta, None, None, None
        return ds, None, dgamma, dbeta, None, None, None


class _LayerNormPass(Function):

    @staticmethod
    def forward(ctx, x, gamma, beta, eps):
        x = _c(x)
        y, _, mean, rstd = K.layernorm_fwd(x, gamma, beta, eps)
        ctx.params = (gamma, beta)
        ctx.save_for_backward(x, mean, rstd)
        ctx.set_materialize_grads(False)
        return y, x.view_as(x)

    @staticmethod
    def backward(ctx, dy, dx_pass=None):
        x, mean, rstd = ctx.saved_tensors
        gamma, beta = ctx.params
        if dy is None:
            return dx_pass, None, None, None
        dy = _c(dy)
        slotted = gamma.requires_grad and _slotted(gamma, beta)
        ds, _, part = K.layernorm_bwd(dy, x, mean, rstd, gamma, ds_extra=_c(dx_pass) if dx_pass is not None else None,
                                      want_partials=True, partials_ok=slotted)
        dgamma = dbeta = None
        if gamma.requires_grad:
            if part is not None:
                ws, chunks = part
                b_slot, g_slot = beta._s2s_grad.view(-1), gamma._s2s_grad.view(-1)
                _side_run(lambda: K.colreduce_partials(ws, chunks, x.shape[-1], b_slot, g_slot), keep=(ws,))
            elif _slotted(gamma, beta):
                _side_run(lambda: _reduce_to(beta, gamma, 1, dy, x, mean, rstd), keep=(dy, x, mean, rstd))
            else:
                dbeta, dgamma = _reduce_to(beta, gamma, 1, dy, x, mean, rstd)
        return ds, dgamma, dbeta, None


def layer_norm(x, gamma, beta, eps=1e-12, passthrough=False):
    if passthrough and torch.is_grad_enabled() and x.requires_grad:
        return _LayerNormPass.apply(x, gamma, beta, eps)
    y = _AddLayerNorm.apply(x, None, gamma, beta, eps, 0.0, 1.0)
    return (y, x) if passthrough else y


class _FanOut(Function):

    @staticmethod
    def forward(ctx, x, n):
        ctx.set_materialize_grads(False)
        return tuple(x.view_as(x) for _ in range(n))

    @staticmethod
    def backward(ctx, *grads):
        gs = [_c(g) for g in grads if g is not None]
        if not gs:
            return None, None
        while len(gs) > 1:
            gs = [K.add_n(gs[:4])] + gs[4:]
        return gs[0], None


def fan_out(x, n):
    if n < 2 or not (torch.is_grad_enabled() and x.requires_grad):
        return (x,) * n
    return _FanOut.apply(x, n)


def add_dropout_layer_norm(res, h, gamma, beta, eps=1e-12, p=0.0, hscale=1.0):
    return _AddLayerNorm.apply(h, res, gamma, beta, eps, p, hscale)


class _AddDropout(Function):

    @staticmethod
    def forward(ctx, h, res, p, hscale):
        seed = K.new_seed(h.device) if p > 0.0 else (None, 0)
        hd = K.act_dropout_fwd(_c(h), p=p, seed=seed) if p > 0.0 else _c(h)
        ctx.meta = (p, seed, hscale)
        return K.axpby(1.0, _c(res), hscale, hd)

    @staticmethod
    def backward(ctx, ds):
        p, seed, hscale = ctx.meta
        ds = _c(ds)
        dh = ds
        if p > 0.0:
            dh = K.act_dropout_bwd(ds, ds, act=None, p=p, seed=seed)
        if hscale != 1.0:
            dh = K.axpby(hscale, dh)
        return dh, ds, None, None


def add_dropout(res, h, p=0.0, hscale=1.0):
    return _AddDropout.apply(h, res, p, hscale)


class _ActDropout(Function):
    @staticmethod
    def forward(ctx, x, act, p):
        seed = K.new_seed(x.device) if p > 0.0 else (None, 0)
        x = _c(x)
        y = K.act_dropout_fwd(x, act=act, p=p, seed=seed)
        ctx.meta = (act, p, seed)
        ctx.save_for_backward(x if act in ("swish", "gelu") else y)
        return y

    @staticmethod
    def backward(ctx, dy):
        (saved,) = ctx.saved_tensors
        act, p, seed = ctx.meta
        return K.act_dropout_bwd(_c(dy), saved, act=act, p=p, seed=seed), None, None


def act_dropout(x, act=None, p=0.0):
    if act is None and p <= 0.0:
        return x
    return _ActDropout.apply(x, act, p)


def dropout(x, p, training=True):
    return act_dropout(x, None, p if training else 0.0)


class _Glu(Function):
    @staticmethod
    def forward(ctx, x):
        x = _c(x)
        ctx.save_for_backward(x)
        return K.glu_fwd(x)

    @staticmethod
    def backward(ctx, dy):
        (x,) = ctx.saved_tensors
        return K.glu_bwd(x, _c(dy))


def glu(x):
    return _Glu.apply(x)


class _PosEnc(Function):
    @staticmethod
    def forward(ctx, x, alpha, pe, xscale, p):
        seed = K.new_seed(x.device) if p > 0.0 else (None, 0)
        x = _c(x)
        y = K.posenc_fwd(x, xscale, alpha, pe, p=p, seed=seed)
        ctx.meta = (xscale, p, seed)
        ctx.alpha = alpha
        ctx.save_for_backward(pe)
        return y

    @staticmethod
    def backward(ctx, dy):
        (pe,) = ctx.saved_tensors
        xscale, p, seed = ctx.meta
        alpha = ctx.alpha
        want = alpha is not None and alpha.requires_grad
        dx, dalpha = K.posenc_bwd(_c(dy), xscale, pe, p=p, seed=seed, want_dalpha=want)
        if want:
            dalpha = _emit_vgrad(alpha, dalpha)
        return dx, dalpha, None, None, None


def posenc(x, pe, alpha=None, xscale=1.0, p=0.0):
    return _PosEnc.apply(x, alpha, pe, xscale, p)


def _bop(t, dk, layout=K.KC, bs0=None):
    assert t.stride(-1) == 1
    return K.operand(t, t.stride(1), layout=layout, bs0=t.stride(0) if bs0 is None else bs0, bs1=dk)


def _pad8(n):
    return (n + 7) // 8 * 8


def _qk(q, k, B, H, T1, T2, dk, D, dtype, bs0_b=None):
    ld = _pad8(T2)
    scores = torch.empty((B, H, T1, ld), dtype=torch.float32, device=q.device)
    K.gemm(_bop(q, dk), _bop(k, dk, bs0=bs0_b), T1, T2, dk, scores, in_dtype=dtype, nb0=B, nb1=H, ldc=ld, cbs=(H * T1 * ld, T1 * ld))
    return scores


def _into(out, A, Bop, M, N, Kd, dk, dtype, B, H, group=None):
    K.gemm(A, Bop, M, N, Kd, out, in_dtype=dtype, nb0=B, nb1=H, ldc=out.stride(1), cbs=(out.stride(0), dk), group=group)
    return out


def _pop(pm, T1, H, layout=K.KC):
    ld = pm.shape[-1]
    return K.operand(pm, ld, layout=layout, bs0=H * T1 * ld, bs1=T1 * ld, zero_padded=True)


def _pv(pm, v, B, H, T1, T2, dk, D, dtype):
    ctxv = torch.empty((B, T1, D), dtype=dtype, device=v.device)
    return _into(ctxv, _pop(pm, T1, H), _bop(v, dk, K.RC), T1, dk, T2, dk, dtype, B, H)


def _pad_like(dattn, ref):
    if dattn is None:
        return None
    if dattn.shape[-1] == ref.shape[-1]:
        return _c(dattn)
    out = torch.zeros_like(ref)
    out[..., : dattn.shape[-1]].copy_(dattn)
    return out


def _attn_common_bwd(dctx, dattn, attn, pm, q, k, v, H, scale, p, seed, Lp=0, rel_mode=0, outs=None, ldb=None, groups=None):
    B, T1, D = q.shape
    T2 = k.shape[1]
    dk = D // H
    dtype = q.dtype
    dctx = _c(dctx) if dctx is not None else torch.zeros((B, T1, D), dtype=dtype, device=q.device)
    if outs is None:
        outs = (torch.empty((B, T1, D), dtype=dtype, device=q.device), torch.empty((B, T2, D), dtype=dtype, device=q.device),
                torch.empty((B, T2, D), dtype=dtype, device=q.device))
    dq, dkk, dv = outs
    if pm is None:
        KAT.fused_bwd(q, k, v, dctx, attn, _pad_like(dattn, attn), H, scale, p, seed, dq, dkk, dv)
        return dq, dkk, dv, None
    gkc, grc, keep = groups if groups is not None else ([], [], [])
    dq_fused = False
    rel_ok = not Lp or (rel_mode == 1 and T1 == T2 and Lp == 2 * T1 - 1 and ldb is not None and ldb % 8 == 0)
    if rel_ok and attn.is_contiguous() and KAT.map_supported(dctx, v, H):
        dq_fused = dq.stride(2) == 1 and KAT.map_product_ok(k, H)
        ds, dbd = KAT.map_bwd(dctx, v, attn, _pad_like(dattn, attn), H, scale, p, seed, ldb=ldb if Lp else 0,
                              k=k if dq_fused else None, dq=dq if dq_fused else None)
    else:
        dp = _qk(dctx, v, B, H, T1, T2, dk, D, dtype)
        ds, dbd = K.attn_softmax_bwd(attn, dp, scale, p=p, seed=seed, Lp=Lp, rel_mode=rel_mode, dattn=_pad_like(dattn, attn), T2=T2,
                                     ldb=ldb)
    _into(dv, _pop(pm, T1, H, K.RC), _bop(dctx, dk, K.RC), T2, dk, T1, dk, dtype, B, H, group=grc)
    if not dq_fused:
        _into(dq, _pop(ds, T1, H), _bop(k, dk, K.RC), T1, dk, T2, dk, dtype, B, H, group=gkc)
    _into(dkk, _pop(ds, T1, H, K.RC), _bop(q, dk, K.RC), T2, dk, T1, dk, dtype, B, H, group=grc)
    keep += [dctx, ds, dbd, pm, q, k, v]
    if groups is None:
        K.launch_group_batched(gkc)
        K.launch_group_batched(grc)
    return dq, dkk, dv, dbd


_FUSED = object()


def _split_pdrop(ctx, pdrop):
    ctx.fused = pdrop is _FUSED
    return None if ctx.fused else pdrop


def _pm(ctx, attn, pdrop):
    return None if ctx.fused else (pdrop if pdrop is not None else attn)


def _attn_fwd_views(q, k, v, klen, causal, H, p):
    B, T1, D = q.shape
    T2 = k.shape[1]
    dk = D // H
    dtype = q.dtype
    scale = 1.0 / math.sqrt(dk)
    seed = K.new_seed(q.device) if p > 0.0 else (None, 0)
    if KAT.supported(q, k, v, H):
        out, attn = KAT.fused_fwd(q, k, v, klen, causal, H, scale, p, seed)
        return out, attn, _FUSED, scale, seed
    if KAT.map_supported(q, k, H):
        attn, pdrop, out = KAT.map_fwd(q, k, klen, causal, H, scale, p, seed, v=v if KAT.map_product_ok(v, H) else None)
        if out is not None:
            return out, attn, pdrop, scale, seed
    else:
        scores = _qk(q, k, B, H, T1, T2, dk, D, dtype)
        attn, pdrop = K.attn_softmax_fwd(scores, dtype, scale, klen=klen, causal=causal, p=p, seed=seed, T2=T2)
    out = _pv(pdrop if pdrop is not None else attn, v, B, H, T1, T2, dk, D, dtype)
    return out, attn, pdrop, scale, seed


def _user_attn(attn, T2):
    return attn if attn.shape[-1] == T2 else attn[..., :T2]


class _AttnPackedQKV(Function):

    @staticmethod
    def forward(ctx, qkv, klen, causal, H, p):
        qkv = _c(qkv)
        D = qkv.shape[-1] // 3
        q, k, v = qkv[..., :D], qkv[..., D:2 * D], qkv[..., 2 * D:]
        out, attn, pdrop, scale, seed = _attn_fwd_views(q, k, v, klen, causal, H, p)
        ctx.meta = (H, scale, p, seed, D)
        ctx.save_for_backward(qkv, attn, _split_pdrop(ctx, pdrop))
        ctx.set_materialize_grads(False)
        return out, _user_attn(attn, k.shape[1])

    @staticmethod
    def backward(ctx, dctx, dattn):
        qkv, attn, pdrop = ctx.saved_tensors
        H, scale, p, seed, D = ctx.meta
        q, k, v = qkv[..., :D], qkv[..., D:2 * D], qkv[..., 2 * D:]
        dqkv = torch.empty_like(qkv)
        _attn_common_bwd(dctx, dattn, attn, _pm(ctx, attn, pdrop), q, k, v, H, scale, p, seed,
                         outs=(dqkv[..., :D], dqkv[..., D:2 * D], dqkv[..., 2 * D:]))
        return dqkv, None, None, None, None


class _AttnPackedKV(Function):

    @staticmethod
    def forward(ctx, q, kv, klen, causal, H, p):
        q = _c(q)
        D = q.shape[-1]
        in_place = kv.stride(-1) == 1 and (KAT.supported(q, kv[..., :D], kv[..., D:], H)
                                           or (KAT.map_supported(q, kv[..., :D], H) and KAT.view_ok(kv[..., D:])))
        if not in_place:
            kv = _c(kv)
        k, v = kv[..., :D], kv[..., D:]
        out, attn, pdrop, scale, seed = _attn_fwd_views(q, k, v, klen, causal, H, p)
        ctx.meta = (H, scale, p, seed, D)
        ctx.gsink = getattr(kv, "_s2s_gsink", None) if in_place else None
        ctx.save_for_backward(q, kv, attn, _split_pdrop(ctx, pdrop))
        ctx.set_materialize_grads(False)
        return out, _user_attn(attn, k.shape[1])

    @staticmethod
    def backward(ctx, dctx, dattn):
        q, kv, attn, pdrop = ctx.saved_tensors
        H, scale, p, seed, D = ctx.meta
        k, v = kv[..., :D], kv[..., D:]
        dq = torch.empty_like(q)
        if ctx.gsink is not None and dctx is not None:
            dkv = ctx.gsink[0].part(ctx.gsink[1])
        else:
            dkv = torch.empty(kv.shape, dtype=kv.dtype, device=kv.device)
        _attn_common_bwd(dctx, dattn, attn, _pm(ctx, attn, pdrop), q, k, v, H, scale, p, seed,
                         outs=(dq, dkv[..., :D], dkv[..., D:]))
        return dq, dkv, None, None, None, None


class _GradSink:
    __slots__ = ("shape", "dtype", "device", "W", "buf", "claimed")

    def __init__(self, shape, dtype, device, W):
        self.shape, self.dtype, self.device, self.W, self.buf, self.claimed = shape, dtype, device, W, None, set()

    def part(self, i):
        if i in self.claimed:
            return torch.empty(self.shape[:-1] + (self.W,), dtype=self.dtype, device=self.device)
        self.claimed.add(i)
        if self.buf is None:
            self.buf = torch.empty(self.shape, dtype=self.dtype, device=self.device)
        return self.buf[..., i * self.W:(i + 1) * self.W]

    def holds(self, grads):
        if self.buf is None:
            return False
        base, es = self.buf.data_ptr(), self.buf.element_size()
        return all(g is not None and g.data_ptr() == base + i * self.W * es and g.shape == self.buf.shape[:-1] + (self.W,)
                   and g.stride() == self.buf.stride() and g.dtype == self.dtype for i, g in enumerate(grads))


class _SplitCols(Function):

    @staticmethod
    def forward(ctx, x, n, sink):
        W = x.shape[-1] // n
        ctx.n, ctx.W, ctx.sink = n, W, sink
        ctx.meta = (x.shape, x.dtype, x.device)
        ctx.set_materialize_grads(False)
        return tuple(x[..., i * W:(i + 1) * W] for i in range(n))

    @staticmethod
    def backward(ctx, *grads):
        shape, dtype, device = ctx.meta
        if all(g is None for g in grads):
            return None, None, None
        sink = ctx.sink
        if sink is not None and sink.holds(grads):
            buf, sink.buf = sink.buf, None
            sink.claimed.clear()
            return buf, None, None
        if sink is not None:
            sink.buf = None
            sink.claimed.clear()
        blk = shape[:-1] + (ctx.W,)
        parts = [g if g is not None else torch.zeros(blk, dtype=dtype, device=device) for g in grads]
        return torch.cat(parts, dim=-1), None, None


def split_cols(x, n):
    sink = _GradSink(tuple(x.shape), x.dtype, x.device, x.shape[-1] // n) if (x.requires_grad and x.is_contiguous()) else None
    parts = _SplitCols.apply(x, n, sink)
    if sink is not None:
        for i, t in enumerate(parts):
            t._s2s_gsink = (sink, i)
    return parts


def attention_packed_qkv(qkv, klen, causal, H, p=0.0):
    return _AttnPackedQKV.apply(qkv, klen, causal, H, p)


def attention_packed_kv(q, kv, klen, causal, H, p=0.0):
    return _AttnPackedKV.apply(q, kv, klen, causal, H, p)


class _AttnCore(Function):
    @staticmethod
    def forward(ctx, q, k, v, klen, causal, H, p):
        q, k, v = _c(q), _c(k), _c(v)
        out, attn, pdrop, scale, seed = _attn_fwd_views(q, k, v, klen, causal, H, p)
        ctx.meta = (H, scale, p, seed)
        ctx.save_for_backward(q, k, v, attn, _split_pdrop(ctx, pdrop))
        ctx.set_materialize_grads(False)
        return out, _user_attn(attn, k.shape[1])

    @staticmethod
    def backward(ctx, dctx, dattn):
        q, k, v, attn, pdrop = ctx.saved_tensors
        H, scale, p, seed = ctx.meta
        pm = _pm(ctx, attn, pdrop)
        dq, dkk, dv, _ = _attn_common_bwd(dctx, dattn, attn, pm, q, k, v, H, scale, p, seed)
        return dq, dkk, dv, None, None, None, None


def attention_core(q, k, v, klen, causal, H, p=0.0):
    return _AttnCore.apply(q, k, v, klen, causal, H, p)


class _RelAttnCore(Function):

    @staticmethod
    def forward(ctx, qu, qv, k, v, pos, klen, H, p, rel_mode):
        qu, qv, k, v, pos = _c(qu), _c(qv), _c(k), _c(v), _c(pos)
        B, T, D = qu.shape
        dk = D // H
        L = pos.shape[1]
        dtype = qu.dtype
        scale = 1.0 / math.sqrt(dk)
        seed = K.new_seed(qu.device) if p > 0.0 else (None, 0)
        ac = _qk(qu, k, B, H, T, T, dk, D, dtype)
        Lq = _pad8(L)
        bd = torch.empty((B, H, T, Lq), dtype=torch.float32, device=qu.device)
        K.gemm(K.operand(qv, D, bs0=T * D, bs1=dk), K.operand(pos, D, bs0=0, bs1=dk), T, L, dk, bd, in_dtype=dtype, nb0=B, nb1=H,
               ldc=Lq, cbs=(H * T * Lq, T * Lq))
        attn, pdrop = K.attn_softmax_fwd(ac, dtype, scale, klen=klen, causal=False, bd=bd, rel_mode=rel_mode, p=p, seed=seed, T2=T,
                                         Lp=L)
        pm = pdrop if pdrop is not None else attn
        out = _pv(pm, v, B, H, T, T, dk, D, dtype)
        ctx.meta = (H, scale, p, seed, rel_mode, L)
        ctx.save_for_backward(qu, qv, k, v, pos, attn, pdrop)
        ctx.set_materialize_grads(False)
        return out, _user_attn(attn, T)

    @staticmethod
    def backward(ctx, dctx, dattn):
        qu, qv, k, v, pos, attn, pdrop = ctx.saved_tensors
        H, scale, p, seed, rel_mode, L = ctx.meta
        B, T, D = qu.shape
        dk = D // H
        dtype = qu.dtype
        pm = pdrop if pdrop is not None else attn
        Lq = _pad8(L)
        dqu, dkk, dv, dbd = _attn_common_bwd(dctx, dattn, attn, pm, qu, k, v, H, scale, p, seed, Lp=L, rel_mode=rel_mode, ldb=Lq)
        dqv = torch.empty((B, T, D), dtype=dtype, device=qu.device)
        K.gemm(K.operand(dbd, Lq, bs0=H * T * Lq, bs1=T * Lq, zero_padded=True), K.operand(pos, D, layout=K.RC, bs0=0, bs1=dk), T, dk,
               L, dqv, in_dtype=dtype, nb0=B, nb1=H, ldc=D, cbs=(T * D, dk))
        part = torch.empty((B, L, D), dtype=dtype, device=qu.device)
        K.gemm(K.operand(dbd, Lq, layout=K.RC, bs0=H * T * Lq, bs1=T * Lq, zero_padded=True),
               K.operand(qv, D, layout=K.RC, bs0=T * D, bs1=dk), L, dk, T, part, in_dtype=dtype, nb0=B, nb1=H, ldc=D, cbs=(L * D, dk))
        dpos, _ = K.colreduce(0, part.view(B, L * D))
        dpos = K.cast(dpos.view(1, L, D), dtype)
        return dqu, dqv, dkk, dv, dpos, None, None, None, None


def rel_attention_core(qu, qv, k, v, pos, klen, H, p=0.0, rel_mode=1):
    return _RelAttnCore.apply(qu, qv, k, v, pos, klen, H, p, rel_mode)


def _head_bias_grads(u, v, dqu, dqv):
    if not u.requires_grad:
        return None, None
    D = dqu.shape[-1]
    a, b = dqu.view(-1, D), dqv.view(-1, D)
    if _slotted(u, v):
        _side_run(lambda: (_reduce_to(u, None, 0, a), _reduce_to(v, None, 0, b)), keep=(a, b))
        return None, None
    su, _ = K.colreduce(0, a)
    sv, _ = K.colreduce(0, b)
    return su.view(u.shape), sv.view(v.shape)


class _RelAttnPacked(Function):

    @staticmethod
    def forward(ctx, qkv, pos, u, v, klen, H, p, rel_mode):
        qkv, pos = _c(qkv), _c(pos)
        B, T, D3 = qkv.shape
        D = D3 // 3
        dk = D // H
        L = pos.shape[1]
        dtype = qkv.dtype
        q, k, vv = qkv[..., :D], qkv[..., D:2 * D], qkv[..., 2 * D:]
        scale = 1.0 / math.sqrt(dk)
        seed = K.new_seed(qkv.device) if p > 0.0 else (None, 0)
        ctx.fused_rel = KAT.rel_supported(q, k, vv, pos, H, rel_mode)
        if ctx.fused_rel:
            attn, pdrop, qu, qv = KAT.rel_fwd(q, k, pos, u.detach().reshape(-1), v.detach().reshape(-1), klen, H, scale, p, seed)
            out = _pv(pdrop if pdrop is not None else attn, vv, B, H, T, T, dk, D, dtype)
            ctx.meta = (H, scale, p, seed, rel_mode, L, D)
            ctx.params = (u, v)
            ctx.save_for_backward(qkv, qu, qv, pos, attn, pdrop)
            ctx.set_materialize_grads(False)
            return out, _user_attn(attn, T)
        qu, qv = K.add_head_bias_view(q, u.detach().reshape(-1), v.detach().reshape(-1))
        ac = _qk(qu, k, B, H, T, T, dk, D, dtype)
        Lq = _pad8(L)
        bd = torch.empty((B, H, T, Lq), dtype=torch.float32, device=qkv.device)
        K.gemm(K.operand(qv, D, bs0=T * D, bs1=dk), K.operand(pos, D, bs0=0, bs1=dk), T, L, dk, bd, in_dtype=dtype, nb0=B, nb1=H,
               ldc=Lq, cbs=(H * T * Lq, T * Lq))
        attn, pdrop = K.attn_softmax_fwd(ac, dtype, scale, klen=klen, causal=False, bd=bd, rel_mode=rel_mode, p=p, seed=seed, T2=T,
                                         Lp=L)
        pm = pdrop if pdrop is not None else attn
        out = _pv(pm, vv, B, H, T, T, dk, D, dtype)
        ctx.meta = (H, scale, p, seed, rel_mode, L, D)
        ctx.params = (u, v)
        ctx.save_for_backward(qkv, qu, qv, pos, attn, pdrop)
        ctx.set_materialize_grads(False)
        return out, _user_attn(attn, T)

    @staticmethod
    def backward(ctx, dctx, dattn):
        qkv, qu, qv, pos, attn, pdrop = ctx.saved_tensors
        H, scale, p, seed, rel_mode, L, D = ctx.meta
        u, v = ctx.params
        B, T, _ = qu.shape
        dk = D // H
        dtype = qu.dtype
        k, vv = qkv[..., D:2 * D], qkv[..., 2 * D:]
        pm = pdrop if pdrop is not None else attn
        Lq = _pad8(L)
        dqkv = torch.empty_like(qkv)
        dqu = torch.empty((B, T, D), dtype=dtype, device=qu.device)
        gkc, grc, keep = [], [], []
        _, _, _, dbd = _attn_common_bwd(dctx, dattn, attn, pm, qu, k, vv, H, scale, p, seed, Lp=L, rel_mode=rel_mode, ldb=Lq,
                                        outs=(dqu, dqkv[..., D:2 * D], dqkv[..., 2 * D:]), groups=(gkc, grc, keep))
        dqv = torch.empty((B, T, D), dtype=dtype, device=qu.device)
        K.gemm(K.operand(dbd, Lq, bs0=H * T * Lq, bs1=T * Lq, zero_padded=True), K.operand(pos, D, layout=K.RC, bs0=0, bs1=dk), T, dk,
               L, dqv, in_dtype=dtype, nb0=B, nb1=H, ldc=D, cbs=(T * D, dk), group=gkc)
        part = torch.empty((B, L, D), dtype=dtype, device=qu.device)
        K.gemm(K.operand(dbd, Lq, layout=K.RC, bs0=H * T * Lq, bs1=T * Lq, zero_padded=True),
               K.operand(qv, D, layout=K.RC, bs0=T * D, bs1=dk), L, dk, T, part, in_dtype=dtype, nb0=B, nb1=H, ldc=D, cbs=(L * D, dk),
               group=grc)
        K.launch_group_batched(gkc)
        K.launch_group_batched(grc)
        del keep
        dpos, _ = K.colreduce(0, part.view(B, L * D))
        dpos = K.cast(dpos.view(1, L, D), dtype)
        K.add_rows(dqu, dqv, dqkv[..., :D])
        du, dv = _head_bias_grads(u, v, dqu, dqv)
        return dqkv, dpos, du, dv, None, None, None, None


def rel_attention_packed(qkv, pos, u, v, klen, H, p=0.0, rel_mode=1):
    return _RelAttnPacked.apply(qkv, pos, u, v, klen, H, p, rel_mode)


class _HeadBias(Function):

    @staticmethod
    def forward(ctx, q, u, v):
        q = _c(q)
        ctx.params = (u, v)
        return K.add_head_bias(q, u.detach().reshape(-1), v.detach().reshape(-1))

    @staticmethod
    def backward(ctx, dqu, dqv):
        u, v = ctx.params
        dqu, dqv = _c(dqu), _c(dqv)
        dq = K.axpby(1.0, dqu, 1.0, dqv)
        du, dv = _head_bias_grads(u, v, dqu, dqv)
        return dq, du, dv


def add_head_bias(q, u, v):
    return _HeadBias.apply(q, u, v)




class _Conv1d(Function):
    @staticmethod
    def forward(ctx, x, weight, bias, act):
        x = _c(x)
        B, T, Cin = x.shape
        Cout, _, ks = weight.shape
        pad = (ks - 1) // 2
        dtype = x.dtype
        wp = K.gather3_cached(weight, (Cout, ks, Cin), (Cin * ks, 1, ks), 0, dtype)
        y = torch.empty((B, T, Cout), dtype=dtype, device=x.device)
        K.gemm(K.operand(x, Cin, mode=K.CONV1D, C=Cin, T=T, pad=pad), K.operand(wp, ks * Cin), B * T, Cout, ks * Cin, y,
               in_dtype=dtype, bias=bias, act=act)
        ctx.act = act
        ctx.params = (weight, bias)
        ctx.save_for_backward(x, y if act else None)
        return y

    @staticmethod
    def backward(ctx, dy):
        x, y = ctx.saved_tensors
        weight, bias = ctx.params
        B, T, Cin = x.shape
        Cout, _, ks = weight.shape
        pad = (ks - 1) // 2
        dtype = x.dtype
        dy = _c(dy)
        if ctx.act:
            dy = K.act_dropout_bwd(dy, y, act=ctx.act)
        dx = None
        if ctx.needs_input_grad[0]:
            wd = K.gather3_cached(weight, (Cin, ks, Cout), (ks, -1, Cin * ks), ks - 1, dtype)
            dx = torch.empty((B, T, Cin), dtype=dtype, device=x.device)
            K.gemm(K.operand(dy, Cout, mode=K.CONV1D, C=Cout, T=T, pad=pad), K.operand(wd, ks * Cout), B * T, Cin, ks * Cout, dx,
                   in_dtype=dtype)
        dw = db = None
        if weight.requires_grad:
            def work():
                dwp = torch.empty((Cout, ks * Cin), dtype=torch.float32, device=x.device)
                rs, racc, dbv = _bias_sink(bias, Cout)
                tile, sk = K.plan_gemm(Cout, ks * Cin, B * T)
                K.gemm(K.operand(dy, Cout, layout=K.RC), K.operand(x, Cin, layout=K.RC, mode=K.CONV1D, C=Cin, T=T, pad=pad),
                       Cout, ks * Cin, B * T, dwp, in_dtype=dtype, splitk=sk, tile=tile, a_rowsum=rs, a_rowsum_accumulate=racc,
                       wgrad=True)
                return _emit_permuted(weight, dwp, Cout, ks, Cin), dbv
            if _slotted(weight, bias):
                _side_run(work, keep=(dy, x))
            else:
                dw, db = work()
        elif bias is not None and bias.requires_grad:
            db, _ = _reduce_to(bias, None, 0, dy.view(B * T, Cout))
        return dx, dw, db, None


class _CropRows(Function):

    @staticmethod
    def forward(ctx, x, vlens):
        from . import kernels_sdp as KS
        ctx.vlens = vlens
        return KS.mask_rows(_c(x), vlens)

    @staticmethod
    def backward(ctx, dy):
        from . import kernels_sdp as KS
        return KS.mask_rows(_c(dy), ctx.vlens), None


def crop_rows(x, vlens):
    return x if vlens is None else _CropRows.apply(x, vlens)


def conv1d(x, weight, bias=None, act=None, vlens=None):
    if vlens is not None and weight.shape[-1] > 1:
        x = crop_rows(x, vlens)
    return _Conv1d.apply(x, weight, bias, act)






class _Conv2dS2(Function):
    @staticmethod
    def forward(ctx, x, weight, bias, grad_premasked=False, input_is_relu=False):
        x = _c(x)
        ctx.grad_premasked = grad_premasked
        ctx.input_is_relu = input_is_relu
        B, T1, F1, C = x.shape
        O = weight.shape[0]
        T2, F2 = (T1 - 3) // 2 + 1, (F1 - 3) // 2 + 1
        dtype = x.dtype
        wp = K.gather3_cached(weight, (O, 9, C), (C * 9, 1, 9), 0, dtype)
        y = torch.empty((B, T2, F2, O), dtype=dtype, device=x.device)
        K.gemm(K.operand(x, C, mode=K.CONV2D_S2, C=C, T1=T1, F1=F1, T2=T2, F2=F2), K.operand(wp, 9 * C), B * T2 * F2, O, 9 * C, y,
               in_dtype=dtype, bias=bias, act="relu")
        ctx.params = (weight, bias)
        ctx.save_for_backward(x, y, wp)
        return y

    @staticmethod
    def backward(ctx, dy):
        x, y, wp = ctx.saved_tensors
        weight, bias = ctx.params
        B, T1, F1, C = x.shape
        O = weight.shape[0]
        T2, F2 = y.shape[1], y.shape[2]
        M2 = B * T2 * F2
        dtype = x.dtype
        dy = _c(dy) if ctx.grad_premasked else K.act_dropout_bwd(_c(dy), y, act="relu")
        dw = db = None
        if weight.requires_grad:
            def work():
                dwp = torch.empty((O, 9 * C), dtype=torch.float32, device=x.device)
                rs, racc, dbv = _bias_sink(bias, O)
                tile, sk = K.plan_gemm(O, 9 * C, M2)
                K.gemm(K.operand(dy, O, layout=K.RC),
                       K.operand(x, C, layout=K.RC, mode=K.CONV2D_S2, C=C, T1=T1, F1=F1, T2=T2, F2=F2), O, 9 * C, M2, dwp,
# ... 322 lines not shown
```

seq2seq_vc_amd/ops/kernels_attn.py:

```python
import os

import torch

from .. import _lib
from .kernels import _DT, ptr, stream

_DISABLED = False


def _strided_ok(t):
    return t.stride(2) == 1 and t.stride(1) % 8 == 0 and t.stride(0) % 8 == 0 and t.data_ptr() % 16 == 0


view_ok = _strided_ok


def supported(q, k, v, H):
    if _DISABLED or q.dtype != torch.bfloat16:
        return False
    dk = q.shape[-1] // H
    if not _lib.lib().s2svc_attn_fused_supported(_DT[q.dtype], q.shape[1], k.shape[1], dk):
        return False
    return _strided_ok(q) and _strided_ok(k) and _strided_ok(v)


def fused_fwd(q, k, v, klen, causal, H, scale, p, seed):
    B, T1, D = q.shape
    T2 = k.shape[1]
    dk = D // H
    ld = (T2 + 7) // 8 * 8
    attn = torch.empty((B, H, T1, ld), dtype=q.dtype, device=q.device)
    out = torch.empty((B, T1, D), dtype=q.dtype, device=q.device)
    _lib.check(_lib.lib().s2svc_attn_fused_fwd(B, H, T1, T2, dk, ptr(q), q.stride(1), q.stride(0), ptr(k), k.stride(1), k.stride(0),
                                               ptr(v), v.stride(1), v.stride(0), ptr(klen), 1 if causal else 0, scale, p, seed[0],
                                               seed[1], ptr(attn), ld, ptr(out), D, T1 * D, stream()), "attn_fused_fwd")
    return out, attn


def fused_bwd(q, k, v, dout, attn, dattn, H, scale, p, seed, dq, dk_out, dv):
    B, T1, D = q.shape
    T2 = k.shape[1]
    dk = D // H
    ld = attn.shape[-1]
    for t in (dout, dq, dk_out, dv):
        if t.stride(2) != 1:
            raise ValueError("fused attention backward: last dim of gradients must be contiguous")
    _lib.check(_lib.lib().s2svc_attn_fused_bwd(B, H, T1, T2, dk, ptr(q), q.stride(1), q.stride(0), ptr(k), k.stride(1), k.stride(0),
                                               ptr(v), v.stride(1), v.stride(0), ptr(dout), dout.stride(1), dout.stride(0), ptr(attn),
                                               ptr(dattn), ld, scale, p, seed[0], seed[1], ptr(dq), dq.stride(1), dq.stride(0),
                                               ptr(dk_out), dk_out.stride(1), dk_out.stride(0), ptr(dv), dv.stride(1), dv.stride(0),
                                               stream()), "attn_fused_bwd")


_MAP_DISABLED = os.environ.get("S2SVC_NO_ATTNMAP", "0") == "1"


def map_supported(q, k, H):
    if _MAP_DISABLED or q.dtype != torch.bfloat16:
        return False
    dk = q.shape[-1] // H
    if not _lib.lib().s2svc_attn_map_supported(_DT[q.dtype], q.shape[1], k.shape[1], dk):
        return False
    return _strided_ok(q) and _strided_ok(k)


def map_product_ok(m, H):
    return bool(_lib.lib().s2svc_attn_map_product_supported(m.shape[-1] // H)) and _strided_ok(m)


def map_fwd(q, k, klen, causal, H, scale, p, seed, v=None):
    B, T1, D = q.shape
    T2 = k.shape[1]
    dk = D // H
    ld = (T2 + 7) // 8 * 8
    attn = torch.empty((B, H, T1, ld), dtype=q.dtype, device=q.device)
    pdrop = torch.empty_like(attn) if p > 0.0 else None
    ctx = torch.empty((B, T1, D), dtype=q.dtype, device=q.device) if v is not None else None
    _lib.check(_lib.lib().s2svc_attn_map_fwd(B, H, T1, T2, dk, ptr(q), q.stride(1), q.stride(0), ptr(k), k.stride(1), k.stride(0),
                                             ptr(klen), 1 if causal else 0, scale, p, seed[0], seed[1], ptr(attn), ptr(pdrop), ld,
                                             ptr(v), v.stride(1) if v is not None else 0, v.stride(0) if v is not None else 0,
                                             ptr(ctx), D, T1 * D, stream()), "attn_map_fwd")
    return attn, pdrop, ctx


def map_bwd(dctx, v, attn, dattn, H, scale, p, seed, ldb=0, k=None, dq=None):
    B, T1, D = dctx.shape
    T2 = v.shape[1]
    ld = attn.shape[-1]
    if dattn is not None and (dattn.shape != attn.shape or not dattn.is_contiguous()):
        raise ValueError("attention map backward: dattn must have the stored map's padded layout")
    if (k is None) != (dq is None) or (dq is not None and (dq.stride(2) != 1 or dq.shape != dctx.shape)):
        raise ValueError("attention map backward: k and dq come together, dq (B,T1,D) with its last dim contiguous")
    ds = torch.empty_like(attn)
    dbd = torch.empty((B, H, T1, ldb), dtype=attn.dtype, device=attn.device) if ldb else None
    _lib.check(_lib.lib().s2svc_attn_map_bwd(B, H, T1, T2, D // H, ptr(dctx), dctx.stride(1), dctx.stride(0), ptr(v), v.stride(1), v.stride(0),
                                             ptr(attn), ptr(dattn), scale, p, seed[0], seed[1], ptr(ds), ld, ptr(dbd), ldb,
                                             ptr(k), k.stride(1) if k is not None else 0, k.stride(0) if k is not None else 0,
                                             ptr(dq), dq.stride(1) if dq is not None else 0, dq.stride(0) if dq is not None else 0,
                                             stream()), "attn_map_bwd")
    return ds, dbd




def rel_supported(q, k, v, pos, H, rel_mode):
    if os.environ.get("S2SVC_NO_RELATTN", "0") == "1" or q.dtype != torch.bfloat16:
        return False
    T, dk = q.shape[1], q.shape[-1] // H
    if not _lib.lib().s2svc_relattn_supported(_DT[q.dtype], T, dk, rel_mode) or pos.shape[1] != 2 * T - 1:
        return False
    return _strided_ok(q) and _strided_ok(k) and _strided_ok(v) and pos.is_contiguous() and pos.data_ptr() % 16 == 0


def rel_fwd(q, k, pos, u, v, klen, H, scale, p, seed):
    B, T, D = q.shape
    dk = D // H
    ld = (T + 7) // 8 * 8
    attn = torch.empty((B, H, T, ld), dtype=q.dtype, device=q.device)
    pdrop = torch.empty_like(attn) if p > 0.0 else None
    qu = torch.empty((B, T, D), dtype=q.dtype, device=q.device)
    qv = torch.empty((B, T, D), dtype=q.dtype, device=q.device)
    _lib.check(_lib.lib().s2svc_relattn_fwd(B, H, T, dk, ptr(q), q.stride(1), q.stride(0), ptr(k), k.stride(1), k.stride(0), ptr(pos),
                                            pos.stride(1), pos.shape[1], ptr(u), ptr(v), ptr(klen), scale, p, seed[0], seed[1],
                                            ptr(attn), ptr(pdrop), ld, ptr(qu), ptr(qv), stream()), "relattn_fwd")
    return attn, pdrop, qu, qv
```

Baseline: 1.697 million mel-frames/sec.

## Fuse output-projection dgrad into fused attention backward kernel

Adds an attention-block autograd path that runs the QKV/Q projection, attention and output projection together. In backward, a new kernel computes dO = dy·W_o^T per head in LDS and feeds it straight into the shared attention backward core, so the separate dctx GEMM and its global round trip are skipped. The attention backward body is moved into a reusable device function. This costs more LDS and registers per block and is limited to D ≤ 512 and short sequences. It is only used where the model calls the new block functions.

```diff
diff --git a/include/s2svc_hip.h b/include/s2svc_hip.h
--- a/include/s2svc_hip.h
+++ b/include/s2svc_hip.h
@@ -290,6 +290,13 @@
                          uint64_t seed_off, void* dq, int64_t lddq, int64_t dqbs, void* dk_out, int64_t lddk, int64_t dkbs, void* dv,
                          int64_t lddv, int64_t dvbs, void* stream);
 
+int s2svc_attn_proj_supported(int dtype, int T1, int T2, int dk, int D, int nproj);
+int s2svc_attn_proj_bwd(int B, int H, int T1, int T2, int dk, const void* q, int64_t ldq, int64_t qbs, const void* k, int64_t ldk,
+                        int64_t kbs, const void* v, int64_t ldv, int64_t vbs, const void* dy, int64_t ldy, int64_t ybs,
+                        const void* wot, int64_t ldw, const void* attn, const void* dattn, int ld, float scale, float drop_p,
+                        const uint64_t* seed_base, uint64_t seed_off, void* dq, int64_t lddq, int64_t dqbs, void* dk_out,
+                        int64_t lddk, int64_t dkbs, void* dv, int64_t lddv, int64_t dvbs, void* stream);
+
 int s2svc_relattn_supported(int dtype, int T, int dk, int rel_mode);
 int s2svc_relattn_fwd(int B, int H, int T, int dk, const void* q, int64_t ldq, int64_t qbs, const void* k, int64_t ldk, int64_t kbs,
                       const void* pos, int64_t ldp, int L, const float* u, const float* v, const int32_t* klen, float scale,
diff --git a/seq2seq_vc_amd/_lib.py b/seq2seq_vc_amd/_lib.py
--- a/seq2seq_vc_amd/_lib.py
+++ b/seq2seq_vc_amd/_lib.py
@@ -225,6 +225,10 @@
     "s2svc_attn_fused_bwd": [c_i32, c_i32, c_i32, c_i32, c_i32, c_vp, c_i64, c_i64, c_vp, c_i64, c_i64, c_vp, c_i64, c_i64, c_vp, c_i64,
                              c_i64, c_vp, c_vp, c_i32, c_f32, c_f32, c_vp, c_u64, c_vp, c_i64, c_i64, c_vp, c_i64, c_i64, c_vp, c_i64,
                              c_i64, c_vp],
+    "s2svc_attn_proj_supported": [c_i32, c_i32, c_i32, c_i32, c_i32, c_i32],
+    "s2svc_attn_proj_bwd": [c_i32, c_i32, c_i32, c_i32, c_i32, c_vp, c_i64, c_i64, c_vp, c_i64, c_i64, c_vp, c_i64, c_i64, c_vp, c_i64,
+                            c_i64, c_vp, c_i64, c_vp, c_vp, c_i32, c_f32, c_f32, c_vp, c_u64, c_vp, c_i64, c_i64, c_vp, c_i64, c_i64,
+                            c_vp, c_i64, c_i64, c_vp],
     "s2svc_relattn_supported": [c_i32, c_i32, c_i32, c_i32],
     "s2svc_relattn_fwd": [c_i32, c_i32, c_i32, c_i32, c_vp, c_i64, c_i64, c_vp, c_i64, c_i64, c_vp, c_i64, c_i32, c_vp, c_vp, c_vp, c_f32,
                           c_f32, c_vp, c_u64, c_vp, c_vp, c_i32, c_vp, c_vp, c_vp],
diff --git a/seq2seq_vc_amd/csrc/attn_fused.hip b/seq2seq_vc_amd/csrc/attn_fused.hip
--- a/seq2seq_vc_amd/csrc/attn_fused.hip
+++ b/seq2seq_vc_amd/csrc/attn_fused.hip
@@ -184,6 +184,94 @@
   }
 }
 
+__device__ __forceinline__ void load_map_rows(const bf16_t* __restrict__ attn, const bf16_t* __restrict__ dattn, int bh, int T1, int T2, int ld,
+                                              u32x4_t (&praw)[4], u32x4_t (&graw)[4]) {
+  const int lane = threadIdx.x & 63, wave = threadIdx.x >> 6, lr = lane & 15, lg = lane >> 4;
+#pragma unroll
+  for (int r = 0; r < 4; ++r) {
+    const int i = wave * 16 + lg * 4 + r;
+    const int64_t arow = ((int64_t)bh * T1 + i) * ld;
+#pragma unroll
+    for (int jn = 0; jn < 4; ++jn) {
+      const int j = jn * 16 + lr;
+      const bool in = i < T1 && j < T2;
+      praw[jn][r] = in ? attn[arow + j] : 0u;
+      graw[jn][r] = (dattn && in) ? dattn[arow + j] : 0u;
+    }
+  }
+}
+
+template <int DK>
+__device__ __forceinline__ void attn_bwd_core(int b, int h, int H, int T1, int T2, int ld, float scale, float p, uint64_t seed,
+                                              const bf16x8_t (&da)[DK / 32], const u32x4_t (&praw)[4], const u32x4_t (&graw)[4],
+                                              bf16_t* Vs, const bf16_t* Kt, const bf16_t* Qt, const bf16_t* dOt, bf16_t* dSt, bf16_t* Pt,
+                                              bf16_t* dSw, bf16_t* __restrict__ dq, int64_t lddq, int64_t dqbs,
+                                              bf16_t* __restrict__ dkk, int64_t lddk, int64_t dkbs, bf16_t* __restrict__ dv, int64_t lddv,
+                                              int64_t dvbs) {
+  constexpr int KP = DK + 8;
+  const int lane = threadIdx.x & 63, wave = threadIdx.x >> 6, lr = lane & 15, lg = lane >> 4;
+  const float inv_keep = p > 0.f ? 1.f / (1.f - p) : 1.f;
+  f32x4_t dp[4];
+#pragma unroll
+  for (int jn = 0; jn < 4; ++jn) {
+    dp[jn] = (f32x4_t){0.f, 0.f, 0.f, 0.f};
+#pragma unroll
+    for (int ks = 0; ks < DK / 32; ++ks) {
+      const bf16x8_t vb = *reinterpret_cast<const bf16x8_t*>(Vs + (jn * 16 + lr) * KP + ks * 32 + lg * 8);
+      dp[jn] = __builtin_amdgcn_mfma_f32_16x16x32_bf16(da[ks], vb, dp[jn], 0, 0, 0);
+    }
+  }
+  bf16_t* dsw = dSw + wave * 16 * TP;
+#pragma unroll 1
+  for (int r = 0; r < 4; ++r) {
+    const int il = lg * 4 + r, i = wave * 16 + il;
+    const int64_t arow = ((int64_t)(b * H + h) * T1 + i) * ld;
+    float pv[4], t[4], m[4];
+    float dot = 0.f;
+#pragma unroll
+    for (int jn = 0; jn < 4; ++jn) {
+      const int j = jn * 16 + lr;
+      const bool in = i < T1 && j < T2;
+      pv[jn] = bf2f((bf16_t)(comp4(praw[jn], r)));
+      m[jn] = (p > 0.f && in) ? dropout_scale(seed, (uint64_t)(arow + j), p, inv_keep) : 1.f;
+      t[jn] = comp(dp[jn], r) * m[jn] + bf2f((bf16_t)(comp4(graw[jn], r)));
+      dot += pv[jn] * t[jn];
+    }
+    dot = grp16_sum(dot);
+#pragma unroll
+    for (int jn = 0; jn < 4; ++jn) {
+      const int j = jn * 16 + lr;
+      const bf16_t ds = f2bf(pv[jn] * (t[jn] - dot) * scale);
+      const bf16_t pd = f2bf(pv[jn] * m[jn]);
+      dsw[il * TP + j] = ds;
+      dSt[j * TP + i] = ds;
+      Pt[j * TP + i] = pd;
+    }
+  }
+  __syncthreads();
+#pragma unroll 1
+  for (int which = 0; which < 3; ++which) {
+    const bf16_t* At = which == 0 ? dsw : (which == 1 ? dSt : Pt) + wave * 16 * TP;
+    const bf16_t* Bt = which == 0 ? Kt : which == 1 ? Qt : dOt;
+    f32x4_t acc[DK / 16];
+#pragma unroll
+    for (int dn = 0; dn < DK / 16; ++dn) acc[dn] = (f32x4_t){0.f, 0.f, 0.f, 0.f};
+#pragma unroll
+    for (int ks = 0; ks < 2; ++ks) {
+      const bf16x8_t a = *reinterpret_cast<const bf16x8_t*>(At + lr * TP + ks * 32 + lg * 8);
+#pragma unroll
+      for (int dn = 0; dn < DK / 16; ++dn) {
+        const bf16x8_t bb = *reinterpret_cast<const bf16x8_t*>(Bt + (dn * 16 + lr) * TP + ks * 32 + lg * 8);
+        acc[dn] = __builtin_amdgcn_mfma_f32_16x16x32_bf16(a, bb, acc[dn], 0, 0, 0);
+      }
+    }
+    bf16_t* dst = which == 0 ? dq + (int64_t)b * dqbs : which == 1 ? dkk + (int64_t)b * dkbs : dv + (int64_t)b * dvbs;
+    const int64_t ldd = which == 0 ? lddq : which == 1 ? lddk : lddv, dbs = which == 0 ? dqbs : which == 1 ? dkbs : dvbs;
+    store_tile_rows<DK>(acc, Vs + wave * 16 * KP, dst + (int64_t)(wave * 16) * ldd + h * DK, ldd, (which == 0 ? T1 : T2) - wave * 16,
+                        (ldd % 8 == 0) && (dbs % 8 == 0) && (((uintptr_t)dst) % 16 == 0));
+  }
+}
+
 template <int DK>
 __global__ __launch_bounds__(256) void attn_fused_bwd_kernel(int H, int T1, int T2, const bf16_t* __restrict__ q, int64_t ldq, int64_t qbs,
                                                              const bf16_t* __restrict__ k, int64_t ldk, int64_t kbs,
@@ -201,11 +289,10 @@
   __shared__ __attribute__((aligned(16))) bf16_t dOt[DK * TP];
   __shared__ __attribute__((aligned(16))) bf16_t dSt[64 * TP];
   __shared__ __attribute__((aligned(16))) bf16_t Pt[64 * TP];
-  __shared__ __attribute__((aligned(16))) bf16_t dSw[4][16 * TP];
+  __shared__ __attribute__((aligned(16))) bf16_t dSw[4 * 16 * TP];
   const int b = blockIdx.x / H, h = blockIdx.x % H;
   const int lane = threadIdx.x & 63, wave = threadIdx.x >> 6, lr = lane & 15, lg = lane >> 4;
   const uint64_t seed = (seed_base ? *seed_base : 0ull) + seed_off;
-  const float inv_keep = p > 0.f ? 1.f / (1.f - p) : 1.f;
   uint4 rv[DK / 32], rk[DK / 32], rq[DK / 32], rdo[DK / 32];
   load_rows<DK>(v + (int64_t)b * vbs + h * DK, ldv, T2, rv);
   load_rows_t<DK>(k + (int64_t)b * kbs + h * DK, ldk, T2, rk);
@@ -217,82 +304,115 @@
   for (int ks = 0; ks < DK / 32; ++ks)
     da[ks] = qi < T1 ? *reinterpret_cast<const bf16x8_t*>(dout + (int64_t)b * obs + (int64_t)qi * ldo + h * DK + ks * 32 + lg * 8) : zero8();
   u32x4_t praw[4], graw[4];
-#pragma unroll
-  for (int r = 0; r < 4; ++r) {
-    const int i = wave * 16 + lg * 4 + r;
-    const int64_t arow = ((int64_t)(b * H + h) * T1 + i) * ld;
-#pragma unroll
-    for (int jn = 0; jn < 4; ++jn) {
-      const int j = jn * 16 + lr;
-      const bool in = i < T1 && j < T2;
-      praw[jn][r] = in ? attn[arow + j] : 0u;
-      graw[jn][r] = (dattn && in) ? dattn[arow + j] : 0u;
-    }
-  }
+  load_map_rows(attn, dattn, b * H + h, T1, T2, ld, praw, graw);
   put_rows<DK>(rv, Vs);
   put_rows_t<DK>(rk, Kt);
   put_rows_t<DK>(rq, Qt);
   put_rows_t<DK>(rdo, dOt);
   __syncthreads();
-  f32x4_t dp[4];
-#pragma unroll
-  for (int jn = 0; jn < 4; ++jn) {
-    dp[jn] = (f32x4_t){0.f, 0.f, 0.f, 0.f};
-#pragma unroll
-    for (int ks = 0; ks < DK / 32; ++ks) {
-      const bf16x8_t vb = *reinterpret_cast<const bf16x8_t*>(Vs + (jn * 16 + lr) * KP + ks * 32 + lg * 8);
-      dp[jn] = __builtin_amdgcn_mfma_f32_16x16x32_bf16(da[ks], vb, dp[jn], 0, 0, 0);
-    }
-  }
-  bf16_t* dsw = dSw[wave];
-#pragma unroll 1
-  for (int r = 0; r < 4; ++r) {
-    const int il = lg * 4 + r, i = wave * 16 + il;
-    const int64_t arow = ((int64_t)(b * H + h) * T1 + i) * ld;
-    float pv[4], t[4], m[4];
-    float dot = 0.f;
-#pragma unroll
-    for (int jn = 0; jn < 4; ++jn) {
-      const int j = jn * 16 + lr;
-      const bool in = i < T1 && j < T2;
-      pv[jn] = bf2f((bf16_t)(comp4(praw[jn], r)));
-      m[jn] = (p > 0.f && in) ? dropout_scale(seed, (uint64_t)(arow + j), p, inv_keep) : 1.f;
-      t[jn] = comp(dp[jn], r) * m[jn] + bf2f((bf16_t)(comp4(graw[jn], r)));
-      dot += pv[jn] * t[jn];
-    }
-    dot = grp16_sum(dot);
-#pragma unroll
-    for (int jn = 0; jn < 4; ++jn) {
-      const int j = jn * 16 + lr;
-      const bf16_t ds = f2bf(pv[jn] * (t[jn] - dot) * scale);
-      const bf16_t pd = f2bf(pv[jn] * m[jn]);
-      dsw[il * TP + j] = ds;
-      dSt[j * TP + i] = ds;
-      Pt[j * TP + i] = pd;
-    }
-  }
+  attn_bwd_core<DK>(b, h, H, T1, T2, ld, scale, p, seed, da, praw, graw, Vs, Kt, Qt, dOt, dSt, Pt, dSw, dq, lddq, dqbs, dkk, lddk, dkbs, dv,
+                    lddv, dvbs);
+}
+
+constexpr int PROJ_MAX_D = 512;
+template <int DK, int NKC> constexpr int attn_proj_bwd_lds() {
+  constexpr int tiles = 64 * (DK + 8) + 3 * DK * TP + 2 * 64 * TP + 4 * 16 * TP, wst = NKC * DK * TP;
+  return tiles > wst ? tiles : wst;
+}
+
+template <int DK, int NKC>
+__global__ __launch_bounds__(256) void attn_proj_bwd_kernel(int H, int T1, int T2, const bf16_t* __restrict__ q, int64_t ldq, int64_t qbs,
+                                                            const bf16_t* __restrict__ k, int64_t ldk, int64_t kbs,
+                                                            const bf16_t* __restrict__ v, int64_t ldv, int64_t vbs,
+                                                            const bf16_t* __restrict__ dy, int64_t ldy, int64_t ybs,
+                                                            const bf16_t* __restrict__ wot, int64_t ldw,
+                                                            const bf16_t* __restrict__ attn, const bf16_t* __restrict__ dattn, int ld,
+                                                            float scale, float p, const uint64_t* seed_base, uint64_t seed_off,
+                                                            bf16_t* __restrict__ dq, int64_t lddq, int64_t dqbs,
+                                                            bf16_t* __restrict__ dkk, int64_t lddk, int64_t dkbs,
+                                                            bf16_t* __restrict__ dv, int64_t lddv, int64_t dvbs) {
+  constexpr int KP = DK + 8, NKS = 2 * NKC, RPC = DK / 32;
+  __shared__ __attribute__((aligned(16))) bf16_t smem[attn_proj_bwd_lds<DK, NKC>()];
+  bf16_t* Vs = smem;
+  bf16_t* Kt = Vs + 64 * KP;
+  bf16_t* Qt = Kt + DK * TP;
+  bf16_t* dOt = Qt + DK * TP;
+  bf16_t* dSt = dOt + DK * TP;
+  bf16_t* Pt = dSt + 64 * TP;
+  bf16_t* dSw = Pt + 64 * TP;
+  bf16_t* Ws = smem;
+  static_assert(64 * KP <= 2 * 64 * TP, "the waves' dO tiles fit the dS^T / Pdrop^T area");
+  const int D = H * DK;
+  const int b = blockIdx.x / H, h = blockIdx.x % H;
+  const int lane = threadIdx.x & 63, wave = threadIdx.x >> 6, lr = lane & 15, lg = lane >> 4;
+  const uint64_t seed = (seed_base ? *seed_base : 0ull) + seed_off;
+  uint4 rw[NKC][RPC];
+  const int wrow = threadIdx.x >> 3, wcol = (threadIdx.x & 7) * 8;
+  const bf16_t* wl = wot + ((int64_t)h * DK + wrow) * ldw + wcol;
+#pragma unroll
+  for (int kc = 0; kc < NKC; ++kc)
+#pragma unroll
+    for (int j = 0; j < RPC; ++j) {
+      rw[kc][j] = make_uint4(0, 0, 0, 0);
+      if (kc < NKC - 2 || kc * 64 + wcol < D) rw[kc][j] = *reinterpret_cast<const uint4*>(wl + (int64_t)(32 * j) * ldw + kc * 64);
+    }
+  const int qi = wave * 16 + lr;
+  bf16x8_t ya[NKS];
+  const bf16_t* yl = dy + (int64_t)b * ybs + (int64_t)qi * ldy + lg * 8;
+#pragma unroll
+  for (int ks = 0; ks < NKS; ++ks)
+    ya[ks] = (qi < T1 && (ks < NKS - 4 || ks * 32 < D)) ? *reinterpret_cast<const bf16x8_t*>(yl + ks * 32) : zero8();
+  uint4 rv[DK / 32], rk[DK / 32], rq[DK / 32];
+  load_rows<DK>(v + (int64_t)b * vbs + h * DK, ldv, T2, rv);
+  load_rows_t<DK>(k + (int64_t)b * kbs + h * DK, ldk, T2, rk);
+  load_rows_t<DK>(q + (int64_t)b * qbs + h * DK, ldq, T1, rq);
+  u32x4_t praw[4], graw[4];
+  load_map_rows(attn, dattn, b * H + h, T1, T2, ld, praw, graw);
+#pragma unroll
+  for (int kc = 0; kc < NKC; ++kc)
+#pragma unroll
+    for (int j = 0; j < RPC; ++j) *reinterpret_cast<uint4*>(Ws + (kc * DK + wrow + 32 * j) * TP + wcol) = rw[kc][j];
   __syncthreads();
-#pragma unroll 1
-  for (int which = 0; which < 3; ++which) {
-    const bf16_t* At = which == 0 ? dsw : (which == 1 ? dSt : Pt) + wave * 16 * TP;
-    const bf16_t* Bt = which == 0 ? Kt : which == 1 ? Qt : dOt;
-    f32x4_t acc[DK / 16];
-#pragma unroll
-    for (int dn = 0; dn < DK / 16; ++dn) acc[dn] = (f32x4_t){0.f, 0.f, 0.f, 0.f};
-#pragma unroll
-    for (int ks = 0; ks < 2; ++ks) {
-      const bf16x8_t a = *reinterpret_cast<const bf16x8_t*>(At + lr * TP + ks * 32 + lg * 8);
-#pragma unroll
-      for (int dn = 0; dn < DK / 16; ++dn) {
-        const bf16x8_t bb = *reinterpret_cast<const bf16x8_t*>(Bt + (dn * 16 + lr) * TP + ks * 32 + lg * 8);
-        acc[dn] = __builtin_amdgcn_mfma_f32_16x16x32_bf16(a, bb, acc[dn], 0, 0, 0);
-      }
-    }
-    bf16_t* dst = which == 0 ? dq + (int64_t)b * dqbs : which == 1 ? dkk + (int64_t)b * dkbs : dv + (int64_t)b * dvbs;
-    const int64_t ldd = which == 0 ? lddq : which == 1 ? lddk : lddv, dbs = which == 0 ? dqbs : which == 1 ? dkbs : dvbs;
-    store_tile_rows<DK>(acc, Vs + wave * 16 * KP, dst + (int64_t)(wave * 16) * ldd + h * DK, ldd, (which == 0 ? T1 : T2) - wave * 16,
-                        (ldd % 8 == 0) && (dbs % 8 == 0) && (((uintptr_t)dst) % 16 == 0));
-  }
+  f32x4_t o[DK / 16];
+#pragma unroll
+  for (int dn = 0; dn < DK / 16; ++dn) o[dn] = (f32x4_t){0.f, 0.f, 0.f, 0.f};
+  bf16x8_t wb[2][DK / 16];
+#pragma unroll
+  for (int dn = 0; dn < DK / 16; ++dn) wb[0][dn] = *reinterpret_cast<const bf16x8_t*>(Ws + (dn * 16 + lr) * TP + lg * 8);
+#pragma unroll
+  for (int ks = 0; ks < NKS; ++ks) {
+    __builtin_amdgcn_sched_barrier(0);
+    if (ks + 1 < NKS) {
+#pragma unroll
+      for (int dn = 0; dn < DK / 16; ++dn)
+        wb[(ks + 1) & 1][dn] =
+            *reinterpret_cast<const bf16x8_t*>(Ws + (((ks + 1) >> 1) * DK + dn * 16 + lr) * TP + ((ks + 1) & 1) * 32 + lg * 8);
+    }
+    __builtin_amdgcn_sched_barrier(0);
+#pragma unroll
+    for (int dn = 0; dn < DK / 16; ++dn) o[dn] = __builtin_amdgcn_mfma_f32_16x16x32_bf16(ya[ks], wb[ks & 1][dn], o[dn], 0, 0, 0);
+  }
+  __builtin_amdgcn_sched_barrier(0);
+  asm volatile("s_waitcnt lgkmcnt(0)\n\ts_barrier" ::: "memory");
+  put_rows<DK>(rv, Vs);
+  put_rows_t<DK>(rk, Kt);
+  put_rows_t<DK>(rq, Qt);
+  bf16_t* tile = dSt + wave * 16 * KP;
+  bf16x8_t da[DK / 32];
+#pragma unroll
+  for (int dn = 0; dn < DK / 16; ++dn) {
+    const uint32_t lo = f2bf2(o[dn][0], o[dn][1]), hi = f2bf2(o[dn][2], o[dn][3]);
+    *reinterpret_cast<uint2*>(dOt + (dn * 16 + lr) * TP + wave * 16 + lg * 4) = make_uint2(lo, hi);
+    tile[(lg * 4 + 0) * KP + dn * 16 + lr] = (bf16_t)(lo & 0xffffu);
+    tile[(lg * 4 + 1) * KP + dn * 16 + lr] = (bf16_t)(lo >> 16);
+    tile[(lg * 4 + 2) * KP + dn * 16 + lr] = (bf16_t)(hi & 0xffffu);
+    tile[(lg * 4 + 3) * KP + dn * 16 + lr] = (bf16_t)(hi >> 16);
+  }
+#pragma unroll
+  for (int ks = 0; ks < DK / 32; ++ks) da[ks] = *reinterpret_cast<const bf16x8_t*>(tile + lr * KP + ks * 32 + lg * 8);
+  __syncthreads();
+  attn_bwd_core<DK>(b, h, H, T1, T2, ld, scale, p, seed, da, praw, graw, Vs, Kt, Qt, dOt, dSt, Pt, dSw, dq, lddq, dqbs, dkk, lddk, dkbs, dv,
+                    lddv, dvbs);
 }
 
 }
@@ -345,3 +465,39 @@
   S2S_CHECK_LAUNCH("attn_fused_bwd_kernel");
   return 0;
 }
+
+extern "C" int s2svc_attn_proj_supported(int dtype, int T1, int T2, int dk, int D, int nproj) {
+  return s2svc_attn_fused_supported(dtype, T1, T2, dk) && D >= dk && D % dk == 0 && D % 32 == 0 && D <= PROJ_MAX_D && nproj == 0;
+}
+
+extern "C" int s2svc_attn_proj_bwd(int B, int H, int T1, int T2, int dk, const void* q, int64_t ldq, int64_t qbs, const void* k,
+                                   int64_t ldk, int64_t kbs, const void* v, int64_t ldv, int64_t vbs, const void* dy, int64_t ldy,
+                                   int64_t ybs, const void* wot, int64_t ldw, const void* attn, const void* dattn, int ld, float scale,
+                                   float drop_p, const uint64_t* seed_base, uint64_t seed_off, void* dq, int64_t lddq, int64_t dqbs,
+                                   void* dk_out, int64_t lddk, int64_t dkbs, void* dv, int64_t lddv, int64_t dvbs, void* stream) {
+  S2S_REQUIRE(H >= 1 && s2svc_attn_proj_supported(S2S_BF16, T1, T2, dk, H * dk, 0),
+              "attn_proj_bwd: unsupported shape (bf16, T <= 64, d_k in {32,64,96,128}, D = H d_k <= 512)");
+  S2S_REQUIRE(ld >= T2, "attn_proj_bwd: the map's row pitch ld must be >= T2");
+  S2S_REQUIRE(ldy >= (int64_t)H * dk && ldw >= (int64_t)H * dk, "attn_proj_bwd: rows of dY and W_o^T hold D elements");
+  S2S_REQUIRE(ldq % 8 == 0 && ldk % 8 == 0 && ldv % 8 == 0 && ldy % 8 == 0 && ldw % 8 == 0 && qbs % 8 == 0 && kbs % 8 == 0 &&
+              vbs % 8 == 0 && ybs % 8 == 0, "attn_proj_bwd: strides must be multiples of 8 elements");
+  S2S_REQUIRE(((uintptr_t)q) % 16 == 0 && ((uintptr_t)k) % 16 == 0 && ((uintptr_t)v) % 16 == 0 && ((uintptr_t)dy) % 16 == 0 &&
+              ((uintptr_t)wot) % 16 == 0, "attn_proj_bwd: 16-byte aligned q/k/v/dY/W_o^T");
+  if (B == 0) return 0;
+  hipStream_t st = (hipStream_t)stream;
+#define S2S_AP_BWD(DK, NKC)                                                                                                     \
+  hipLaunchKernelGGL((attn_proj_bwd_kernel<DK, NKC>), dim3(B * H), dim3(256), 0, st, H, T1, T2, (const bf16_t*)q, ldq, qbs,      \
+                     (const bf16_t*)k, ldk, kbs, (const bf16_t*)v, ldv, vbs, (const bf16_t*)dy, ldy, ybs, (const bf16_t*)wot, ldw, \
+                     (const bf16_t*)attn, (const bf16_t*)dattn, ld, scale, drop_p, seed_base, seed_off, (bf16_t*)dq, lddq, dqbs,  \
+                     (bf16_t*)dk_out, lddk, dkbs, (bf16_t*)dv, lddv, dvbs)
+#define S2S_AP_BWD_D(DK)                                                                            \
+  do {                                                                                              \
+    if (H * DK <= 128) S2S_AP_BWD(DK, 2); else if (H * DK <= 256) S2S_AP_BWD(DK, 4);                \
+    else if (H * DK <= 384) S2S_AP_BWD(DK, 6); else S2S_AP_BWD(DK, 8);                              \
+  } while (0)
+  if (dk == 32) S2S_AP_BWD_D(32); else if (dk == 64) S2S_AP_BWD_D(64); else if (dk == 96) S2S_AP_BWD_D(96); else S2S_AP_BWD_D(128);
+#undef S2S_AP_BWD_D
+#undef S2S_AP_BWD
+  S2S_CHECK_LAUNCH("attn_proj_bwd_kernel");
+  return 0;
+}
diff --git a/seq2seq_vc_amd/modules.py b/seq2seq_vc_amd/modules.py
--- a/seq2seq_vc_amd/modules.py
+++ b/seq2seq_vc_amd/modules.py
@@ -285,12 +285,23 @@
         kl = None if klens is None else klens.dev
         f = getattr(self, "_fused", None)
         qp = None
+        wo, bo = self.linear_out.weight, self.linear_out.bias
+        packed = f is not None and key is value and (query is not key or "w_qkv" in f)
+        if (kv is not None or packed) and Fn.attn_block_ok(query, (key if kv is None else kv).shape[1], kv, self.h, wo):
+            if kv is None and query is key:
+                r = Fn.attention_block_qkv(query, f["w_qkv"], f["b_qkv"], wo, bo, kl, causal, self.h, self._p(), passthrough)
+            else:
+                if kv is None:
+                    kv = Fn.linear(key, f["w_kv"], f["b_kv"])
+                r = Fn.attention_block_kv(query, f["w_q"], f["b_q"], kv, wo, bo, kl, causal, self.h, self._p(), passthrough)
+            self.attn = r[1]
+            return (r[0], r[2]) if passthrough else r[0]
         if kv is not None:
             q = Fn.linear(query, f["w_q"], f["b_q"], passthrough=passthrough)
             if passthrough:
                 q, qp = q
             ctx, self.attn = Fn.attention_packed_kv(q, kv, kl, causal, self.h, self._p())
-        elif f is not None and key is value and (query is not key or "w_qkv" in f):
+        elif packed:
             if query is key:
                 qkv = Fn.linear(query, f["w_qkv"], f["b_qkv"], passthrough=passthrough)
                 if passthrough:
@@ -308,7 +319,7 @@
             v = Fn.linear(value, self.linear_v.weight, self.linear_v.bias)
             ctx, self.attn = Fn.attention_core(q, k, v, kl, causal, self.h, self._p())
             qp = query
-        out = Fn.linear(ctx, self.linear_out.weight, self.linear_out.bias)
+        out = Fn.linear(ctx, wo, bo)
         return (out, qp) if passthrough else out
 
 
diff --git a/seq2seq_vc_amd/ops/functional.py b/seq2seq_vc_amd/ops/functional.py
--- a/seq2seq_vc_amd/ops/functional.py
+++ b/seq2seq_vc_amd/ops/functional.py
@@ -387,39 +387,43 @@
             return g_pass, None, None, None, None
         x2, w, y = ctx.saved_tensors
         weight, bias = ctx.params
-        M, Kd = x2.shape
-        N = w.shape[0]
-        dtype = x2.dtype
-        dy2 = _c(dy).view(M, N)
-        if ctx.act:
-            dy2 = K.act_dropout_bwd(dy2, y, act=ctx.act)
-        ldy, zp, dy_rows = N, False, dy2
-        if dtype == torch.float32 and N % 4 and dy2.is_cuda:
-            ldy, zp = (N + 3) // 4 * 4, True
-            dy2 = K.pad_cols(dy2, ldy)
-        dx = None
-        if ctx.needs_input_grad[0]:
-            dx = torch.empty((M, Kd), dtype=dtype, device=dy.device)
-            res = _c(g_pass).view(M, Kd).to(dtype) if g_pass is not None else None
-            K.gemm(K.operand(dy2, ldy, zero_padded=zp), _dgrad_operand(weight, w, N, Kd, dtype), M, Kd, N, dx, in_dtype=dtype, res=res)
-            dx = dx.view(ctx.xshape)
-        dw = db = None
-        if weight.requires_grad:
-            tile, sk = K.plan_gemm(N, Kd, M, dtype=dtype)
-            rs, racc, db = _bias_sink(bias, N)
-
-            def wr(out, acc):
-                K.gemm(K.operand(dy2, ldy, layout=K.RC, zero_padded=zp), K.operand(x2, Kd, layout=K.RC), N, Kd, M, out, in_dtype=dtype,
-                       splitk=sk, tile=tile, accumulate=acc, a_rowsum=rs, a_rowsum_accumulate=racc)
-            if _slotted(weight, bias if ctx.has_bias else None):
-                _side_run(lambda: _emit_wgrad(weight, (N, Kd), wr), keep=(dy2, x2))
-            else:
-                dw = _emit_wgrad(weight, (N, Kd), wr)
-                if dw is not None:
-                    dw = dw.view(weight.shape)
-        elif ctx.has_bias and bias.requires_grad:
-            db, _ = _reduce_to(bias, None, 0, dy_rows)
-        return dx, dw, db, None, None
+        dx, dw, db = _linear_bwd(x2, w, y, ctx.act, weight, bias, ctx.has_bias, dy, g_pass, ctx.needs_input_grad[0])
+        return (None if dx is None else dx.view(ctx.xshape)), dw, db, None, None
+
+
+def _linear_bwd(x2, w, y, act, weight, bias, has_bias, dy, g_pass, want_dx):
+    M, Kd = x2.shape
+    N = w.shape[0]
+    dtype = x2.dtype
+    dy2 = _c(dy).view(M, N)
+    if act:
+        dy2 = K.act_dropout_bwd(dy2, y, act=act)
+    ldy, zp, dy_rows = N, False, dy2
+    if dtype == torch.float32 and N % 4 and dy2.is_cuda:
+        ldy, zp = (N + 3) // 4 * 4, True
+        dy2 = K.pad_cols(dy2, ldy)
+    dx = None
+    if want_dx:
+        dx = torch.empty((M, Kd), dtype=dtype, device=dy.device)
+        res = _c(g_pass).view(M, Kd).to(dtype) if g_pass is not None else None
+        K.gemm(K.operand(dy2, ldy, zero_padded=zp), _dgrad_operand(weight, w, N, Kd, dtype), M, Kd, N, dx, in_dtype=dtype, res=res)
+    dw = db = None
+    if weight.requires_grad:
+        tile, sk = K.plan_gemm(N, Kd, M, dtype=dtype)
+        rs, racc, db = _bias_sink(bias, N)
+
+        def wr(out, acc):
+            K.gemm(K.operand(dy2, ldy, layout=K.RC, zero_padded=zp), K.operand(x2, Kd, layout=K.RC), N, Kd, M, out, in_dtype=dtype,
+                   splitk=sk, tile=tile, accumulate=acc, a_rowsum=rs, a_rowsum_accumulate=racc)
+        if _slotted(weight, bias if has_bias else None):
+            _side_run(lambda: _emit_wgrad(weight, (N, Kd), wr), keep=(dy2, x2))
+        else:
+            dw = _emit_wgrad(weight, (N, Kd), wr)
+            if dw is not None:
+                dw = dw.view(weight.shape)
+    elif has_bias and bias.requires_grad:
+        db, _ = _reduce_to(bias, None, 0, dy_rows)
+    return dx, dw, db
 
 
 def linear(x, weight, bias=None, act=None, passthrough=False):
@@ -958,6 +962,120 @@
 
 def attention_packed_kv(q, kv, klen, causal, H, p=0.0):
     return _AttnPackedKV.apply(q, kv, klen, causal, H, p)
+
+
+def attn_block_ok(query, T2, kv, H, w_o):
+    if not (torch.is_grad_enabled() and query.dim() == 3 and getattr(w_o, "_s2s_bf16_t", None) is not None):
+        return False
+    D = query.shape[-1]
+    if not KAT.proj_bwd_supported(query.dtype, query.shape[1], T2, D // H, D) or D % 8:
+        return False
+    return kv is None or (kv.dtype == query.dtype and kv.stride(-1) == 1 and KAT.view_ok(kv[..., :D]) and KAT.view_ok(kv[..., D:]))
+
+
+def _block_project(x, weight, bias):
+    dtype = x.dtype
+    x2 = _c(x).view(-1, x.shape[-1])
+    M, Kd = x2.shape
+    N = weight.shape[0]
+    w = _wcast(weight, dtype)
+    y = torch.empty((M, N), dtype=dtype, device=x.device)
+    K.gemm(K.operand(x2, Kd), K.operand(w, Kd), M, N, Kd, y, in_dtype=dtype, bias=bias)
+    return x2, w, y.view(*x.shape[:-1], N)
+
+
+def _block_core_bwd(ctx, dy, dattn, attn, cv, wo, q, k, v, outs):
+    H, scale, p, seed, D = ctx.meta
+    w_o, b_o = ctx.out_params
+    if dy is None:
+        _attn_common_bwd(None, dattn, attn, None, q, k, v, H, scale, p, seed, outs=outs)
+        return None, None
+    dy = _c(dy)
+    wot = getattr(w_o, "_s2s_bf16_t", None)
+    fold = (wot is not None and dy.shape[0] * dy.shape[1] > 64 and all(t.stride(-1) == 1 for t in outs)
+            and KAT.proj_bwd_ok(q, k, v, dy, wot, H))
+    dctx, dwo, dbo = _linear_bwd(cv.view(-1, D), wo, None, None, w_o, b_o, b_o is not None, dy, None, not fold)
+    if fold:
+        KAT.proj_bwd(q, k, v, dy, wot, attn, _pad_like(dattn, attn), H, scale, p, seed, *outs)
+    else:
+        _attn_common_bwd(dctx.view(cv.shape), dattn, attn, None, q, k, v, H, scale, p, seed, outs=outs)
+    return dwo, dbo
+
+
+class _AttnBlockQKV(Function):
+
+    @staticmethod
+    def forward(ctx, x, w_qkv, b_qkv, w_o, b_o, klen, causal, H, p, passthrough):
+        D = x.shape[-1]
+        x2, wi, qkv = _block_project(x, w_qkv, b_qkv)
+        q, k, v = qkv[..., :D], qkv[..., D:2 * D], qkv[..., 2 * D:]
+        cv, attn, pdrop, scale, seed = _attn_fwd_views(q, k, v, klen, causal, H, p)
+        assert pdrop is _FUSED
+        _, wo, y = _block_project(cv, w_o, b_o)
+        ctx.meta = (H, scale, p, seed, D)
+        ctx.in_params, ctx.out_params, ctx.xshape = (w_qkv, b_qkv), (w_o, b_o), x.shape
+        ctx.save_for_backward(x2, wi, qkv, attn, cv, wo)
+        ctx.set_materialize_grads(False)
+        if passthrough:
+            return y, _user_attn(attn, k.shape[1]), x.view_as(x)
+        return y, _user_attn(attn, k.shape[1])
+
+    @staticmethod
+    def backward(ctx, dy, dattn, g_pass=None):
+        if dy is None and dattn is None:
+            return (g_pass,) + (None,) * 9
+        x2, wi, qkv, attn, cv, wo = ctx.saved_tensors
+        D = ctx.meta[4]
+        dqkv = torch.empty_like(qkv)
+        dwo, dbo = _block_core_bwd(ctx, dy, dattn, attn, cv, wo, qkv[..., :D], qkv[..., D:2 * D], qkv[..., 2 * D:],
+                                   (dqkv[..., :D], dqkv[..., D:2 * D], dqkv[..., 2 * D:]))
+        w_in, b_in = ctx.in_params
+        dx, dw, db = _linear_bwd(x2, wi, None, None, w_in, b_in, b_in is not None, dqkv, g_pass, ctx.needs_input_grad[0])
+        return (None if dx is None else dx.view(ctx.xshape)), dw, db, dwo, dbo, None, None, None, None, None
+
+
+class _AttnBlockKV(Function):
+
+    @staticmethod
+    def forward(ctx, x, w_q, b_q, kv, w_o, b_o, klen, causal, H, p, passthrough):
+        D = x.shape[-1]
+        x2, wi, q = _block_project(x, w_q, b_q)
+        k, v = kv[..., :D], kv[..., D:]
+        cv, attn, pdrop, scale, seed = _attn_fwd_views(q, k, v, klen, causal, H, p)
+        assert pdrop is _FUSED
+        _, wo, y = _block_project(cv, w_o, b_o)
+        ctx.meta = (H, scale, p, seed, D)
+        ctx.in_params, ctx.out_params, ctx.xshape = (w_q, b_q), (w_o, b_o), x.shape
+        ctx.gsink = getattr(kv, "_s2s_gsink", None)
+        ctx.save_for_backward(x2, wi, q, kv, attn, cv, wo)
+        ctx.set_materialize_grads(False)
+        if passthrough:
+            return y, _user_attn(attn, k.shape[1]), x.view_as(x)
+        return y, _user_attn(attn, k.shape[1])
+
+    @staticmethod
+    def backward(ctx, dy, dattn, g_pass=None):
+        if dy is None and dattn is None:
+            return (g_pass,) + (None,) * 10
+        x2, wi, q, kv, attn, cv, wo = ctx.saved_tensors
+        D = ctx.meta[4]
+        dq = torch.empty_like(q)
+        if ctx.gsink is not None and dy is not None:
+            dkv = ctx.gsink[0].part(ctx.gsink[1])
+        else:
+            dkv = torch.empty(kv.shape, dtype=kv.dtype, device=kv.device)
+        dwo, dbo = _block_core_bwd(ctx, dy, dattn, attn, cv, wo, q, kv[..., :D], kv[..., D:], (dq, dkv[..., :D], dkv[..., D:]))
+        w_in, b_in = ctx.in_params
+        dx, dw, db = _linear_bwd(x2, wi, None, None, w_in, b_in, b_in is not None, dq, g_pass, ctx.needs_input_grad[0])
+        return (None if dx is None else dx.view(ctx.xshape)), dw, db, dkv, dwo, dbo, None, None, None, None, None
+
+
+def attention_block_qkv(x, w_qkv, b_qkv, w_o, b_o, klen, causal, H, p=0.0, passthrough=False):
+    return _AttnBlockQKV.apply(x, w_qkv, b_qkv, w_o, b_o, klen, causal, H, p, passthrough)
+
+
+def attention_block_kv(x, w_q, b_q, kv, w_o, b_o, klen, causal, H, p=0.0, passthrough=False):
+    return _AttnBlockKV.apply(x, w_q, b_q, kv, w_o, b_o, klen, causal, H, p, passthrough)
 
 
 class _AttnCore(Function):
diff --git a/seq2seq_vc_amd/ops/kernels_attn.py b/seq2seq_vc_amd/ops/kernels_attn.py
--- a/seq2seq_vc_amd/ops/kernels_attn.py
+++ b/seq2seq_vc_amd/ops/kernels_attn.py
@@ -50,6 +50,35 @@
                                                ptr(dattn), ld, scale, p, seed[0], seed[1], ptr(dq), dq.stride(1), dq.stride(0),
                                                ptr(dk_out), dk_out.stride(1), dk_out.stride(0), ptr(dv), dv.stride(1), dv.stride(0),
                                                stream()), "attn_fused_bwd")
+
+
+_PROJ_OFF = {"0": set(), "1": {"fwd", "bwd"}, "fwd": {"fwd"}, "bwd": {"bwd"}}[os.environ.get("S2SVC_NO_ATTN_PROJ", "0")]
+
+
+def proj_bwd_supported(dtype, T1, T2, dk, D):
+    if _DISABLED or "bwd" in _PROJ_OFF or dtype != torch.bfloat16:
+        return False
+    return bool(_lib.lib().s2svc_attn_proj_supported(_DT[dtype], T1, T2, dk, D, 0))
+
+
+def proj_bwd_ok(q, k, v, dy, wot, H):
+    D = q.shape[-1]
+    return (proj_bwd_supported(q.dtype, q.shape[1], k.shape[1], D // H, D) and _strided_ok(q) and _strided_ok(k) and _strided_ok(v)
+            and dy.dtype == q.dtype and _strided_ok(dy) and wot.dtype == q.dtype and tuple(wot.shape) == (D, D) and wot.stride(1) == 1
+            and wot.stride(0) % 8 == 0 and wot.data_ptr() % 16 == 0)
+
+
+def proj_bwd(q, k, v, dy, wot, attn, dattn, H, scale, p, seed, dq, dk_out, dv):
+    B, T1, D = q.shape
+    T2 = k.shape[1]
+    for t in (dy, dq, dk_out, dv):
+        if t.stride(2) != 1:
+            raise ValueError("fused attention backward: last dim of gradients must be contiguous")
+    _lib.check(_lib.lib().s2svc_attn_proj_bwd(B, H, T1, T2, D // H, ptr(q), q.stride(1), q.stride(0), ptr(k), k.stride(1), k.stride(0),
+                                              ptr(v), v.stride(1), v.stride(0), ptr(dy), dy.stride(1), dy.stride(0), ptr(wot),
+                                              wot.stride(0), ptr(attn), ptr(dattn), attn.shape[-1], scale, p, seed[0], seed[1], ptr(dq),
+                                              dq.stride(1), dq.stride(0), ptr(dk_out), dk_out.stride(1), dk_out.stride(0), ptr(dv),
+                                              dv.stride(1), dv.stride(0), stream()), "attn_proj_bwd")
 
 
 _MAP_DISABLED = os.environ.get("S2SVC_NO_ATTNMAP", "0") == "1"
```

Result: faster. 1.730 million mel-frames/sec (median of 6 runs) (+1.9%).
